# NilanEkanayake/TiTok-Video

Measured on AMD Instinct MI355X. Metric: video clips/sec encode+decode (whole node), higher is better.
Workload: dtype bf16

## Files before the change

include/titok_hip.h:

```cpp
#ifndef TITOK_HIP_H
#define TITOK_HIP_H

#include <stdint.h>

#ifdef __cplusplus
extern "C" {
#endif

#define TTV_OK 0
#define TTV_ERR_INVALID 1
#define TTV_ERR_LAUNCH 2
#define TTV_ERR_UNSUPPORTED 3

#define TTV_BF16 0
#define TTV_F32 1

#define TTV_ENCODER 0
#define TTV_DECODER 1

#define TTV_MAX_FSQ 8
#define TTV_MAX_TOKEN 64
#define TTV_MAX_CLIPS_PER_LAUNCH 64

const char* ttv_error_string(void);
// ... 100 lines not shown
                    int q_heads, int kv_heads, int head_dim, int flags, int dtype, void* stream);

int ttv_patch_gather(const void* const* clips, const int32_t* clip_desc, int clip0, int n_clips, int patch_t, int patch_h,
                     int patch_w, int channels, void* patches, int ld, int dtype, int max_patches_per_clip, void* stream);
int ttv_patch_scatter(const void* patches, int ld, const int32_t* clip_desc, int clip0, int n_clips, int patch_t, int patch_h,
                      int patch_w, int channels, void* const* clips, int dtype, int max_patches_per_clip, void* stream);

typedef struct ttv_tower_dims {
  int32_t kind;
  int32_t dtype;
  int32_t width;
  int32_t layers;
  int32_t q_heads, kv_heads, head_dim;
  int32_t inner;
  int32_t patch_t, patch_h, patch_w;
  int32_t pix_channels;
  int32_t token_size;
  float eps;
  float alpha;
} ttv_tower_dims;

typedef struct ttv_layer_weights {
  const float* pre_ln;
  const void* to_qkv;
  const void* out_proj;
  const float* ffd_norm;
  const void* w12;
  const void* w3;
  const float* attn_post_ln;
  const float* ffd_post_ln;
  const void* to_qkv_pn;
  const void* w12_pn;
  const void* mlp_pack;
  int32_t mlp_pack_qkv_rows;
  int32_t qkv_q_prescaled;
  const void* to_qkv_qs;
  const void* to_qkv_f8; const float* to_qkv_f8_scale;
  const void* w12_f8; const float* w12_f8_scale;
  const void* to_qkv_mx; const void* w12_mx;
  const void* out_proj_f8; const float* out_proj_f8_scale; const void* out_proj_mx;
  const void* w3_f8; const float* w3_f8_scale; const void* w3_mx;
} ttv_layer_weights;

typedef struct ttv_tower_weights {
  const void* proj_in_w;
  const void* proj_in_b;
  const float* mask_token;
  const float* ln_pre_t;
  const float* ln_pre_p;
  const float* ln_post;
  const void* proj_out_w;
  const void* proj_out_b;
  const ttv_layer_weights* layers;
  const void* proj_out_pn;
  int32_t f32_split3;
} ttv_tower_weights;

typedef struct ttv_batch {
  int32_t n_clips;
  int32_t total_rows;
  int32_t sum_tokens;
  int32_t sum_patches;
  int32_t max_patches_per_clip;
  int32_t n_qblocks;
  const int32_t* cu_seqlens;
  const int32_t* latent_rows;
  const int32_t* patch_rows;
  const int32_t* clip_desc;
  const int32_t* qblocks;
  const float* rope_cs;
  const int32_t* blocks64;
  const int32_t* row_seq;
  int32_t n_blocks64;
  int32_t qblocks_paired;
  int32_t qblocks_all_full;
  const int32_t* items64;
  int32_t n_items64;
  const int32_t* rope_ids;
  const float* rope_base;
  const int32_t* qblocks_latent;
  int32_t n_qblocks_latent;
  const int32_t* qblocks_patch;
  int32_t n_qblocks_patch;
} ttv_batch;

int ttv_rope_table_build(const float* base_cos, const float* base_sin, int n_ids, int n_freqs, const int32_t* clip_desc,
                         const int32_t* cu_seqlens, const int32_t* row_seq, float* rope_cs, int total_rows, void* stream);

typedef struct ttv_plan_sizes {
  int32_t n_clips, total_rows, sum_tokens, sum_patches, max_patches_per_clip, max_seqlen, n_rope_ids, n_blocks64;
  int64_t host_words;
  int64_t off_cu_seqlens, off_clip_desc, off_blocks64;
  int64_t dev_words;
  int64_t off_latent_rows, off_patch_rows, off_row_seq, off_rope_ids;
} ttv_plan_sizes;

int ttv_plan_rows_sizes(const int32_t* pixel_dims, const int32_t* token_counts, int n_clips, const int32_t* patch, ttv_plan_sizes* sizes);
int ttv_plan_rows_fill(const int32_t* pixel_dims, const int32_t* token_counts, int n_clips, const int32_t* patch, int bwd_xcd,
                       int32_t* host_segment, int64_t host_words);

int ttv_plan_rows_build(const ttv_plan_sizes* sizes, const int32_t* host_segment, int32_t* dev_segment, const float* base_cos,
                        const float* base_sin, int n_freqs, float* rope_cs, const float* rope_base, ttv_batch* batch, void* stream);

typedef struct ttv_plan_attn {
  int32_t n_qblocks, qblocks_all_full, n_qblocks_latent, n_qblocks_patch, n_qblocks_l0, reserved;
  int64_t words;
  int64_t off_qblocks, off_qblocks_latent, off_qblocks_patch, off_qblocks_l0;
} ttv_plan_attn;

int ttv_plan_attn_sizes(const int32_t* cu_seqlens, const int32_t* token_counts, int n_clips, int q_heads, int kv_heads, int split,
                        int tail_div, ttv_plan_attn* sizes);
int ttv_plan_attn_fill(const int32_t* cu_seqlens, const int32_t* token_counts, int n_clips, int q_heads, int kv_heads, int split,
                       int tail_div, int32_t* host_tables, int64_t host_words);
int ttv_plan_attn_set(const ttv_plan_attn* sizes, const int32_t* host_tables, int32_t* dev_tables, ttv_batch* batch, void* stream);

int ttv_rope_base_table(int head_dim, int nd, int n_ids, double theta, float* base_cos, float* base_sin);

int64_t ttv_tower_workspace_bytes(const ttv_tower_dims* dims, const ttv_batch* batch);

int ttv_encoder_forward(const ttv_tower_dims* dims, const ttv_tower_weights* w, const ttv_batch* batch,
                        const void* const* clips, const ttv_fsq_params* fsq, float* z, void* codes, int32_t* indices,
                        float* bounded, void* workspace, int64_t workspace_bytes, void* stream);

int ttv_decoder_forward(const ttv_tower_dims* dims, const ttv_tower_weights* w, const ttv_batch* batch, const void* codes,
                        void* const* clips_out, void* workspace, int64_t workspace_bytes, void* stream);

typedef struct ttv_dec_l0_const {
  const void* rows;
  int32_t latent_rows;
  int32_t patch_rows;
  const float* state;
  const int32_t* qblocks;
  int32_t n_qblocks;
} ttv_dec_l0_const;
int64_t ttv_dec_l0_const_bytes(const ttv_tower_dims* dims, int patch_rows);
int ttv_dec_l0_const_build(const ttv_tower_dims* dims, const ttv_tower_weights* w, const int32_t* iota, const float* rope_cs,
                           const int32_t* rope_ids, const float* rope_base, int patch_rows, void* block, int64_t block_bytes,
                           int64_t* state_offset, int64_t* flag_offset, void* stream);
int ttv_decoder_forward_const(const ttv_tower_dims* dims, const ttv_tower_weights* w, const ttv_batch* batch, const void* codes,
                              void* const* clips_out, void* workspace, int64_t workspace_bytes, const ttv_dec_l0_const* l0, void* stream);

typedef struct ttv_layer_weights_t {
  const void* to_qkv_t;
  const void* out_proj_t;
  const void* w12_t;
  const void* w3_t;
} ttv_layer_weights_t;
typedef struct ttv_tower_weights_t {
  const void* proj_in_t;
  const void* proj_out_t;
  const ttv_layer_weights_t* layers;
} ttv_tower_weights_t;
typedef struct ttv_layer_grads {
  float* pre_ln; float* to_qkv; float* out_proj; float* ffd_norm; float* w12; float* w3; float* attn_post_ln; float* ffd_post_ln;
} ttv_layer_grads;
typedef struct ttv_tower_grads {
  float* proj_in_w; float* proj_in_b; float* mask_token; float* ln_pre_t; float* ln_pre_p; float* ln_post; float* proj_out_w;
  float* proj_out_b;
  const ttv_layer_grads* layers;
  void** layer_done_events;
} ttv_tower_grads;

int64_t ttv_tower_tape_bytes(const ttv_tower_dims* dims, const ttv_batch* batch);
int64_t ttv_tower_bwd_workspace_bytes(const ttv_tower_dims* dims, const ttv_batch* batch);
#define TTV_TAPE_STORED 0
#define TTV_TAPE_RECOMPUTE 1
// ... 144 lines not shown
int ttv_fvd_preprocess(void* const* clips, const int32_t* dims, int n_clips, int dtype, int clamp, float* out, void* stream);

int ttv_i3d_features(const ttv_i3d_weights* w, const float* x, int n, float* feats, void* workspace, int64_t workspace_bytes,
                     void* stream);

int ttv_i3d_conv3d(const float* x, int N, int T, int H, int W, int Cin, int k, int stride, const float* w, const float* scale,
                   const float* shift, int Cout, int relu, float* y, int ldc, int c_off, void* stream);
int ttv_i3d_maxpool3d(const float* x, int N, int T, int H, int W, int C, int kt, int kh, int kw, int st, int sh, int sw, float* y,
                      void* stream);

#define TTV_VJEPA_WIDTH 1024
#define TTV_VJEPA_TOKENS 1568
#define TTV_VJEPA_PATCH_K 1536
typedef struct ttv_vjepa_layer {
  const float* norm1_w; const float* norm1_b;
  const void* qkv_w; const void* qkv_b;
  const void* proj_w; const void* proj_b;
  const float* norm2_w; const float* norm2_b;
  const void* fc1_w; const void* fc1_b;
  const void* fc2_w; const void* fc2_b;
} ttv_vjepa_layer;
typedef struct ttv_vjepa_weights {
  int32_t width, heads, depth;
  const void* patch_w; const void* patch_b; const float* pos_embed;
  const ttv_vjepa_layer* layers;
  const float* norm_w; const float* norm_b;
  const float* query_tokens; const void* pool_q;
  const float* pool_norm1_w; const float* pool_norm1_b;
  const void* pool_kv_w; const void* pool_kv_b;
  const void* pool_proj_w; const void* pool_proj_b;
  const float* pool_norm2_w; const float* pool_norm2_b;
  const void* pool_fc1_w; const void* pool_fc1_b;
  const void* pool_fc2_w; const void* pool_fc2_b;
} ttv_vjepa_weights;

int ttv_jedi_preprocess(void* const* clips, const int32_t* dims, int n_clips, int dtype, void* out, void* stream);
int64_t ttv_vjepa_workspace_bytes(int n);
int ttv_vjepa_features(const ttv_vjepa_weights* w, const void* x, int n, float* feats, int finetuned, void* workspace,
                       int64_t workspace_bytes, void* stream);

#define TTV_VJEPA_EPI_STORE 0
#define TTV_VJEPA_EPI_GELU 1
#define TTV_VJEPA_EPI_RESID 2
int ttv_vjepa_layernorm(const float* x, int ldx, int rows, int width, const float* w1, const float* b1, float eps1, const float* w2,
                        const float* b2, float eps2, float* y32, int ld32, void* y16, int ld16, void* stream);
int ttv_vjepa_linear(const void* x, int ldx, const void* w, int ldw, const void* bias, int M, int N, int K, int epilogue,
                     const float* resid, int ldr, int resid_rows, void* y, int ldy, void* stream);
int ttv_vjepa_pool_attention(const void* q, const void* kv, int n, int rows, void* out, void* stream);

#define TTV_KC_ATTENTION 1
#define TTV_KC_GEMM_QKV 2
#define TTV_KC_GEMM_GEGLU 3
#define TTV_KC_GEMM_RESID 4
#define TTV_KC_GEMM_STORE 5
#define TTV_KC_RMSNORM 6
#define TTV_KC_PATCH 7
#define TTV_KC_ROWS 8
int ttv_prof_begin(int kernel_class, int max_records);
enum {
  TTV_DBG_NO_STORES = 1,
  TTV_DBG_K256_NO_PANEL_DMA = 2,
  TTV_DBG_MLP_NO_WEIGHT_DMA = 2,
  TTV_DBG_K256_NO_TILE_RELOAD = 4,
  TTV_DBG_MLP_NO_GEGLU = 4,
  TTV_DBG_K256_NO_EPILOGUE_MATH = 8,
  TTV_DBG_MLP_TILES8 = 8,
  TTV_DBG_MLP_NO_P2 = 16,
  TTV_DBG_MLP_PAIRS_ONLY = 32,
  TTV_DBG_MLP_TILES4 = 64,
  TTV_DBG_GEMM_TILE160 = 128,
  TTV_DBG_GEMM_TILE128 = 256,
  TTV_DBG_GEMM_T256 = 512,
  TTV_DBG_MLP_TILES9 = 512,
  TTV_DBG_GEMM_NO_T256 = 1024,
  TTV_DBG_MX_UNFUSED_QUANT = 2048,
  TTV_DBG_SPLIT3_NO_IMAGES = 4096,
  TTV_DBG_SPLIT3_NO_DMA = 8192,
  TTV_DBG_K256_GENERAL = 16384,
  TTV_DBG_QKV256_OFF = 32768,
  TTV_DBG_QKV256_WS = 131072,
  TTV_DBG_ENC_ALL_ROWS = 524288,
  TTV_DBG_ATTN_NO_SWP = 1048576,
  TTV_DBG_DEC_ALL_BLOCKS = 2097152,
  TTV_DBG_DEC_L0_NO_CONST = 4194304
};
int ttv_debug_set(int flags);
int ttv_debug_stamps(void* device_buffer);
int ttv_prof_end(double* total_ms, int* count);

#ifdef __cplusplus
}
#endif
#endif
```

titok_video_amd/_lib.py:

```python
from __future__ import annotations

import ctypes as C
import os
import threading

import torch

from . import switches

TTV_BF16, TTV_F32 = 0, 1
TTV_ENCODER, TTV_DECODER = 0, 1
TTV_MAX_FSQ = 8
TTV_MAX_TOKEN = 64
TTV_MAX_CLIPS_PER_LAUNCH = 64
TTV_DISC_HEAD_GENERATOR, TTV_DISC_HEAD_DISCRIMINATOR = 0, 1
TTV_TAPE_STORED, TTV_TAPE_RECOMPUTE = 0, 1

DBG_NO_STORES = 1
DBG_K256_NO_PANEL_DMA = 2
DBG_MLP_NO_WEIGHT_DMA = 2
DBG_K256_NO_TILE_RELOAD = 4
DBG_MLP_NO_GEGLU = 4
DBG_K256_NO_EPILOGUE_MATH = 8
DBG_MLP_TILES8 = 8
DBG_MLP_NO_P2 = 16
DBG_MLP_PAIRS_ONLY = 32
DBG_MLP_TILES4 = 64
DBG_GEMM_TILE160 = 128
DBG_GEMM_TILE128 = 256
DBG_GEMM_T256 = 512
DBG_MLP_TILES9 = 512
DBG_GEMM_NO_T256 = 1024
DBG_MX_UNFUSED_QUANT = 2048
DBG_SPLIT3_NO_IMAGES = 4096
DBG_SPLIT3_NO_DMA = 8192
DBG_K256_GENERAL = 16384
DBG_QKV256_OFF = 32768
DBG_QKV256_WS = 131072
DBG_ENC_ALL_ROWS = 524288
DBG_ATTN_NO_SWP = 1048576
DBG_DEC_ALL_BLOCKS = 2097152
DBG_DEC_L0_NO_CONST = 4194304

_HERE = os.path.dirname(os.path.abspath(__file__))
LIB_PATH = switches.text("TTV_LIB_PATH") or os.path.join(_HERE, "libtitok_hip.so")

i32, i64, f32, vp = C.c_int32, C.c_int64, C.c_float, C.c_void_p


class FsqParams(C.Structure):
    _fields_ = [("n", i32), ("levels", i32 * TTV_MAX_FSQ), ("basis", i32 * TTV_MAX_FSQ),
                ("half_l", f32 * TTV_MAX_FSQ), ("offset", f32 * TTV_MAX_FSQ), ("shift", f32 * TTV_MAX_FSQ),
                ("half_width", f32 * TTV_MAX_FSQ)]


class TowerDims(C.Structure):
    _fields_ = [("kind", i32), ("dtype", i32), ("width", i32), ("layers", i32), ("q_heads", i32), ("kv_heads", i32),
                ("head_dim", i32), ("inner", i32), ("patch_t", i32), ("patch_h", i32), ("patch_w", i32),
                ("pix_channels", i32), ("token_size", i32), ("eps", f32), ("alpha", f32)]


class NextQkv(C.Structure):
    _fields_ = [("qkv", vp), ("ld", i32), ("rope_cs", vp), ("rows", i32), ("rope_q_end", i32), ("rope_k_begin", i32), ("rope_k_end", i32)]


class LayerWeights(C.Structure):
    _fields_ = [("pre_ln", vp), ("to_qkv", vp), ("out_proj", vp), ("ffd_norm", vp), ("w12", vp), ("w3", vp),
                ("attn_post_ln", vp), ("ffd_post_ln", vp), ("to_qkv_pn", vp), ("w12_pn", vp), ("mlp_pack", vp), ("mlp_pack_qkv_rows", i32), ("qkv_q_prescaled", i32),
                ("to_qkv_qs", vp), ("to_qkv_f8", vp), ("to_qkv_f8_scale", vp), ("w12_f8", vp), ("w12_f8_scale", vp),
                ("to_qkv_mx", vp), ("w12_mx", vp), ("out_proj_f8", vp), ("out_proj_f8_scale", vp), ("out_proj_mx", vp),
                ("w3_f8", vp), ("w3_f8_scale", vp), ("w3_mx", vp)]


class TowerWeights(C.Structure):
    _fields_ = [("proj_in_w", vp), ("proj_in_b", vp), ("mask_token", vp), ("ln_pre_t", vp), ("ln_pre_p", vp),
                ("ln_post", vp), ("proj_out_w", vp), ("proj_out_b", vp), ("layers", C.POINTER(LayerWeights)), ("proj_out_pn", vp),
                ("f32_split3", i32)]


class Batch(C.Structure):
    _fields_ = [("n_clips", i32), ("total_rows", i32), ("sum_tokens", i32), ("sum_patches", i32),
                ("max_patches_per_clip", i32), ("n_qblocks", i32), ("cu_seqlens", vp), ("latent_rows", vp),
                ("patch_rows", vp), ("clip_desc", vp), ("qblocks", vp), ("rope_cs", vp), ("blocks64", vp), ("row_seq", vp),
                ("n_blocks64", i32), ("qblocks_paired", i32), ("qblocks_all_full", i32), ("items64", vp), ("n_items64", i32),
                ("rope_ids", vp), ("rope_base", vp), ("qblocks_latent", vp), ("n_qblocks_latent", i32), ("qblocks_patch", vp),
                ("n_qblocks_patch", i32)]


class PlanSizes(C.Structure):
    _fields_ = [("n_clips", i32), ("total_rows", i32), ("sum_tokens", i32), ("sum_patches", i32), ("max_patches_per_clip", i32),
                ("max_seqlen", i32), ("n_rope_ids", i32), ("n_blocks64", i32), ("host_words", i64), ("off_cu_seqlens", i64),
                ("off_clip_desc", i64), ("off_blocks64", i64), ("dev_words", i64), ("off_latent_rows", i64), ("off_patch_rows", i64),
                ("off_row_seq", i64), ("off_rope_ids", i64)]


class PlanAttn(C.Structure):
    _fields_ = [("n_qblocks", i32), ("qblocks_all_full", i32), ("n_qblocks_latent", i32), ("n_qblocks_patch", i32), ("n_qblocks_l0", i32),
                ("reserved", i32), ("words", i64), ("off_qblocks", i64), ("off_qblocks_latent", i64), ("off_qblocks_patch", i64),
                ("off_qblocks_l0", i64)]


class DecL0Const(C.Structure):
    _fields_ = [("rows", vp), ("latent_rows", i32), ("patch_rows", i32), ("state", vp), ("qblocks", vp), ("n_qblocks", i32)]


class LayerWeightsT(C.Structure):
    _fields_ = [("to_qkv_t", vp), ("out_proj_t", vp), ("w12_t", vp), ("w3_t", vp)]


class TowerWeightsT(C.Structure):
    _fields_ = [("proj_in_t", vp), ("proj_out_t", vp), ("layers", C.POINTER(LayerWeightsT))]


class LayerGrads(C.Structure):
    _fields_ = [("pre_ln", vp), ("to_qkv", vp), ("out_proj", vp), ("ffd_norm", vp), ("w12", vp), ("w3", vp),
                ("attn_post_ln", vp), ("ffd_post_ln", vp)]


class TowerGrads(C.Structure):
    _fields_ = [("proj_in_w", vp), ("proj_in_b", vp), ("mask_token", vp), ("ln_pre_t", vp), ("ln_pre_p", vp), ("ln_post", vp),
                ("proj_out_w", vp), ("proj_out_b", vp), ("layers", C.POINTER(LayerGrads)), ("layer_done_events", C.POINTER(vp))]


TTV_OPT_SCHEDULE_NONE, TTV_OPT_SCHEDULE_COSINE = 0, 1
TTV_OPT_SKIP_NONFINITE = 1


class OptState(C.Structure):
    _fields_ = [("updates", i64), ("skipped", i64), ("schedule_index", i64), ("skip_now", i32), ("lr", f32), ("bc1", f32),
                ("bc2_sqrt", f32), ("clip_coef", f32), ("norm", f32)]


class OptSchedule(C.Structure):
    _fields_ = [("kind", i32), ("reserved", i32), ("warmup_steps", i64), ("training_steps", i64), ("base_lr", C.c_double),
                ("end_lr", C.c_double), ("num_cycles", C.c_double), ("initial_lr", C.c_double), ("first", i64), ("stride", i64)]


class LpipsWeights(C.Structure):
    _fields_ = [("w", vp * 13), ("wd", vp * 13), ("b", vp * 13), ("lin", vp * 5)]


TTV_I3D_CONVS = 58
TTV_I3D_FEATURES = 400


class I3dWeights(C.Structure):
    _fields_ = [("w", vp * TTV_I3D_CONVS), ("scale", vp * TTV_I3D_CONVS), ("shift", vp * TTV_I3D_CONVS)]


TTV_VJEPA_WIDTH = 1024
TTV_VJEPA_TOKENS = 1568
TTV_VJEPA_PATCH_K = 1536
TTV_VJEPA_EPI_STORE, TTV_VJEPA_EPI_GELU, TTV_VJEPA_EPI_RESID = 0, 1, 2


class VjepaLayer(C.Structure):
    _fields_ = [("norm1_w", vp), ("norm1_b", vp), ("qkv_w", vp), ("qkv_b", vp), ("proj_w", vp), ("proj_b", vp), ("norm2_w", vp),
                ("norm2_b", vp), ("fc1_w", vp), ("fc1_b", vp), ("fc2_w", vp), ("fc2_b", vp)]


class VjepaWeights(C.Structure):
    _fields_ = [("width", i32), ("heads", i32), ("depth", i32), ("patch_w", vp), ("patch_b", vp), ("pos_embed", vp),
                ("layers", C.POINTER(VjepaLayer)), ("norm_w", vp), ("norm_b", vp), ("query_tokens", vp), ("pool_q", vp),
                ("pool_norm1_w", vp), ("pool_norm1_b", vp), ("pool_kv_w", vp), ("pool_kv_b", vp), ("pool_proj_w", vp),
                ("pool_proj_b", vp), ("pool_norm2_w", vp), ("pool_norm2_b", vp), ("pool_fc1_w", vp), ("pool_fc1_b", vp),
                ("pool_fc2_w", vp), ("pool_fc2_b", vp)]


_lib = None
# ... 194 lines not shown
```

titok_video_amd/csrc/ttv_api.hip:

```cpp
#include <stdarg.h>
#include <stdio.h>
#include <stdlib.h>
#include <string.h>

#include "ttv_common.h"
#include "ttv_kernels.h"

static thread_local char g_err[512] = "";

void ttv_set_error(const char* fmt, ...) {
  va_list ap;
  va_start(ap, fmt);
  vsnprintf(g_err, sizeof(g_err), fmt, ap);
  va_end(ap);
}

int g_ttv_prof_class = 0;
bool ttv_sw_enc_latent_last() { static const bool v = ttv_env_flag("TTV_ENC_LATENT_LAST", true); return v; }
bool ttv_enc_latent_rows_only(const ttv_tower_dims* d, const ttv_batch* b) {
  return ttv_sw_enc_latent_last() && !(g_ttv_debug & TTV_DBG_ENC_ALL_ROWS) && d->kind == TTV_ENCODER && b->latent_rows && b->sum_tokens > 0 &&
         b->sum_tokens < b->total_rows;
}
bool ttv_sw_keel_f32sum() { static const bool v = ttv_env_flag("TTV_KEEL_F32SUM", false); return v; }
bool ttv_sw_fused_patch() { static const bool v = ttv_env_flag("TTV_FUSED_PATCH", true); return v; }
bool ttv_sw_attn_pipe() { static const bool v = ttv_env_flag("TTV_ATTN_PIPE", false); return v; }
static bool sw_dec_l0_const() { static const bool v = ttv_env_flag("TTV_DEC_L0_CONST", true); return v; }
float ttv_sw_attn_thr() { static const float v = ttv_env_float("TTV_ATTN_THR", 8.0f); return v; }
thread_local int g_ttv_debug = 0;
long long* g_ttv_stamps = nullptr;
static hipEvent_t* g_prof_start = nullptr;
static hipEvent_t* g_prof_stop = nullptr;
static int g_prof_cap = 0, g_prof_n = 0;

TtvProfScope::TtvProfScope(int cls, hipStream_t stream) : slot(-1), s(stream) {
  if (g_ttv_prof_class != 0 && cls == g_ttv_prof_class && g_prof_n < g_prof_cap) {
    slot = g_prof_n++;
    (void)hipEventRecord(g_prof_start[slot], s);
  }
}
TtvProfScope::~TtvProfScope() {
  if (slot >= 0) (void)hipEventRecord(g_prof_stop[slot], s);
}

struct TowerWs {
  char *x, *xn, *qkv, *ao, *h, *pa, *pb;
  char *xl, *aol;
  char *f8, *f8mx;
  float* y32;
  float* rstd;
  int64_t total;
};

static TowerWs carve(const ttv_tower_dims* d, const ttv_batch* b, char* base) {
  const int64_t e = dtype_bytes(d->dtype);
  const int64_t L = b->total_rows, P = b->sum_patches;
  const int64_t g = (int64_t)d->kv_heads * d->head_dim;
  const int64_t pd = patch_dim(d);
  int64_t off = 0;
  TowerWs w;
  auto take = [&](int64_t bytes) { char* p = base ? base + off : nullptr; off += align256(bytes); return p; };
  w.x = take(L * d->width * e);
  w.xn = take(L * d->width * e);
  w.qkv = take(L * (2 * d->width + 2 * g) * e);
  w.ao = take(L * d->width * e);
  w.y32 = (float*)take(L * d->width * 4);
  w.h = take(L * d->inner * e);
  w.pa = take(P * pd * e);
  w.pb = take(P * d->width * e);
  w.rstd = (float*)take(L * 4);
  w.xl = take((int64_t)b->sum_tokens * d->width * e);
  w.aol = take((int64_t)b->sum_tokens * d->width * e);
  w.f8 = w.f8mx = nullptr;
  if (d->dtype == TTV_BF16 && d->width != 256 && d->width % 128 == 0) {
    const int64_t wide = d->width > d->inner ? d->width : d->inner;
    w.f8 = take(L * wide);
    w.f8mx = take(L * (wide / 128 + 4) * 4);
  }
  w.total = off;
  return w;
}

static int check_dims(const ttv_tower_dims* d, const ttv_batch* b) {
  TTV_CHECK_ARG(d && b, "null dims/batch");
  TTV_CHECK_ARG(d->dtype == TTV_BF16 || d->dtype == TTV_F32, "bad dtype %d", d->dtype);
  TTV_CHECK_ARG(d->head_dim == 64 && d->width == d->q_heads * 64, "width must be q_heads*64");
  TTV_CHECK_ARG(d->width % 64 == 0 && d->width <= 1024, "width %d unsupported", d->width);
  TTV_CHECK_ARG(d->inner % 32 == 0, "GEGLU inner dim must be a multiple of 32");
  TTV_CHECK_ARG(d->token_size >= 1 && d->token_size <= TTV_MAX_TOKEN, "token_size out of range");
  TTV_CHECK_ARG(((int64_t)d->pix_channels * d->patch_t * d->patch_h * d->patch_w) % 8 == 0, "patch vector length must be a multiple of 8");
  TTV_CHECK_ARG(b->n_clips > 0 && b->total_rows == b->sum_tokens + b->sum_patches, "inconsistent batch");
  return TTV_OK;
}

struct LayerCtx {
  const ttv_tower_dims* d; const ttv_batch* b; const TowerWs& ws; hipStream_t s;
  int split3, s3img;
  bool gen_ok;
  int pair, all_full, pipe;
};

static int tower_attention(const LayerCtx& c, bool q_scaled, const int32_t* table, int n_table, int site) {
  const ttv_tower_dims* d = c.d;
  const int flags = TTV_ATTN_GATE | (q_scaled ? TTV_ATTN_QSCALED : 0) | (c.split3 ? TTV_ATTN_SPLIT3 : 0) |
                    (c.s3img ? (TTV_ATTN_SPLIT_OUT | TTV_ATTN_SPLIT_IN) : 0) | site;
  return ttvk_attention(c.ws.qkv, 2 * d->width + 2 * d->kv_heads * d->head_dim, c.ws.ao, d->width, c.b->cu_seqlens, table, n_table, d->q_heads,
                        d->kv_heads, d->head_dim, flags, d->dtype, c.s);
}

static int run_layer_mx(const LayerCtx& c, const ttv_layer_weights& lw, int i, bool& rstd_valid, bool& xq_valid) {
  const ttv_tower_dims* d = c.d;
  const ttv_batch* b = c.b;
  const TowerWs& ws = c.ws;
  hipStream_t s = c.s;
  const int L = b->total_rows, dm = d->width, g = d->kv_heads * d->head_dim, dt = d->dtype, nq = 2 * dm + 2 * g, I = d->inner;
  const float alpha = keel_alpha(d, i);
  static const bool fused_env = ttv_env_flag("TTV_MX_FUSED_QUANT", true);
  const bool fused_q = fused_env && !(g_ttv_debug & TTV_DBG_MX_UNFUSED_QUANT);
  if (!rstd_valid) TTV_TRY(ttvk_row_rstd(ws.x, dt, dm, ws.rstd, L, dm, d->eps, s));
  if (!xq_valid) TTV_TRY(ttvk_quant_mx_fp8(ws.x, dt, dm, ws.f8, dm, ws.f8mx, nullptr, L, dm, s));
  xq_valid = false;
  const GemmArgs a = gemm_rope_qk(gemm_args(dt, ws.f8, dm, lw.to_qkv_f8, dm, L, nq, dm, ws.qkv, nq), b->rope_cs, dm, g);
  TTV_TRY(ttvk_gemm_fp8(EPI_QKV_ROPE, a, ws.rstd, lw.to_qkv_f8_scale, s, ws.f8mx, lw.to_qkv_mx));
  const bool q_scaled = lw.qkv_q_prescaled != 0;
  if (fused_q && q_scaled && !c.pair && !c.pipe && d->head_dim == 64) {
    TTV_TRY(ttvk_attention_mxout(ws.qkv, nq, ws.f8, ws.f8mx, (int)ttvk_mx_scale_ld(dm), b->cu_seqlens, b->qblocks, b->n_qblocks, d->q_heads,
                                 d->kv_heads, s));
  } else {
    TTV_TRY(tower_attention(c, q_scaled, b->qblocks, b->n_qblocks, c.pair | (c.pipe ? c.all_full | c.pipe : 0)));
    TTV_TRY(ttvk_quant_mx_fp8(ws.ao, dt, dm, ws.f8, dm, ws.f8mx, nullptr, L, dm, s));
  }
  const GemmArgs o = gemm_resid(gemm_args(dt, ws.f8, dm, lw.out_proj_f8, dm, L, dm, dm, ws.x, dm), ws.x, dm, alpha);
  TTV_TRY(ttvk_gemm_fp8(EPI_RESID_T, o, nullptr, lw.out_proj_f8_scale, s, ws.f8mx, lw.out_proj_mx));
  if (i > 0) {
    TTV_TRY(ttvk_rmsnorm(ws.x, dt, dm, nullptr, ws.x, dt, dm, nullptr, lw.attn_post_ln, L, dm, d->eps, s, ws.rstd, fused_q ? ws.f8 : nullptr,
                         fused_q ? ws.f8mx : nullptr));
    if (!fused_q) TTV_TRY(ttvk_quant_mx_fp8(ws.x, dt, dm, ws.f8, dm, ws.f8mx, nullptr, L, dm, s));
  } else {
    TTV_TRY(ttvk_row_rstd(ws.x, dt, dm, ws.rstd, L, dm, d->eps, s));
    TTV_TRY(ttvk_quant_mx_fp8(ws.x, dt, dm, ws.f8, dm, ws.f8mx, nullptr, L, dm, s));
  }
  GemmArgs f = gemm_args(dt, ws.f8, dm, lw.w12_f8, dm, L, I, dm, ws.h, I);
  char* const hq = ws.h;
  char* const hq_mx = ws.xn;
  const bool h_fused = fused_q && (int64_t)ttvk_mx_scale_ld(I) <= (int64_t)dm * 2;
  if (h_fused) { f.yq = hq; f.yq_mx = hq_mx; }
  TTV_TRY(ttvk_gemm_fp8(EPI_GEGLU, f, ws.rstd, lw.w12_f8_scale, s, ws.f8mx, lw.w12_mx));
  if (!h_fused) TTV_TRY(ttvk_quant_mx_fp8(ws.h, dt, I, ws.f8, I, ws.f8mx, nullptr, L, I, s));
  const GemmArgs f3 = gemm_resid(gemm_args(dt, h_fused ? hq : ws.f8, I, lw.w3_f8, I, L, dm, I, ws.x, dm), ws.x, dm, alpha);
  TTV_TRY(ttvk_gemm_fp8(EPI_RESID_T, f3, nullptr, lw.w3_f8_scale, s, h_fused ? hq_mx : ws.f8mx, lw.w3_mx));
  rstd_valid = false;
  if (i > 0) {
    TTV_TRY(ttvk_rmsnorm(ws.x, dt, dm, nullptr, ws.x, dt, dm, nullptr, lw.ffd_post_ln, L, dm, d->eps, s, ws.rstd, fused_q ? ws.f8 : nullptr,
                         fused_q ? ws.f8mx : nullptr));
    rstd_valid = true;
    xq_valid = fused_q;
  }
  return TTV_OK;
}

static bool rows_f8(int dt, int dm, const void* img, const void* row_scale, const void* mx, const void* folded) {
  return dt == TTV_BF16 && img && row_scale && !mx && dm % 128 == 0 && !(dm == 256 && folded);
}

struct PreNormW { const float* gain; const void *w, *w_pn, *w_f8; const float* w_f8_scale; bool f8; };

static int prenorm_proj(const LayerCtx& c, GemmEpilogue epi, const char* x, int rows, const PreNormW& p, int N, char* y, int y_image,
                        bool rstd_valid, int tile_run = 0, int tile_period = 0) {
  const ttv_tower_dims* d = c.d;
  const TowerWs& ws = c.ws;
  const int dm = d->width, dt = d->dtype;
  GemmArgs a = gemm_args(dt, nullptr, dm, nullptr, dm, rows, N, dm, y, N);
  if (epi == EPI_QKV_ROPE) a = gemm_rope_qk(a, c.b->rope_cs, dm, d->kv_heads * d->head_dim);
  if (p.f8) {
    float* const f8_scales = reinterpret_cast<float*>(ws.xn + align256((int64_t)c.b->total_rows * dm));
    TTV_TRY(ttvk_quant_rows_fp8(x, dt, dm, p.gain, d->eps, ws.xn, dm, f8_scales, rows, dm, c.s));
    a.x = ws.xn; a.w = p.w_f8;
    return ttvk_gemm_fp8(epi, a, f8_scales, p.w_f8_scale, c.s);
  }
  const bool fold256 = dt == TTV_BF16 && dm == 256 && p.w_pn;
  const bool fold_gen = c.gen_ok && p.w_pn;
  const bool fold = fold256 || fold_gen;
  if (fold_gen && !rstd_valid) TTV_TRY(ttvk_row_rstd(x, dt, dm, ws.rstd, rows, dm, d->eps, c.s));
  if (!fold) TTV_TRY(ttvk_rmsnorm(x, dt, dm, nullptr, ws.xn, dt, dm, nullptr, p.gain, rows, dm, d->eps, c.s, nullptr, nullptr, nullptr, c.s3img));
  a.split3 = c.split3; a.x_image = c.s3img && !fold; a.y_image = y_image;
  a.prenorm = fold256; a.eps = d->eps;
  a.row_scale = fold_gen ? ws.rstd : nullptr;
  a.x = fold ? x : ws.xn; a.w = fold ? p.w_pn : p.w;
  if (epi == EPI_QKV_ROPE) { a.rope_ids = c.b->rope_ids; a.rope_base = c.b->rope_ids ? c.b->rope_base : nullptr; }
  a.tile_run = tile_run; a.tile_period = tile_period;
  return ttvk_gemm(epi, a, c.s);
}

static int keel_tail(const LayerCtx& c, GemmArgs o, int layer, const float* post_gain, bool want_rstd, bool& rstd_valid) {
  const ttv_tower_dims* d = c.d;
  const int dm = d->width, dt = d->dtype;
  char* const cx = (char*)o.y;
  o = gemm_resid(o, cx, dm, keel_alpha(d, layer));
  o.split3 = c.split3; o.x_image = c.s3img;
  if (layer == 0) return ttvk_gemm(EPI_RESID_T, o, c.s);
  if (ttvk_gemm_supports_resid_norm(dt, dm, o.K)) {
    o.norm_gain = post_gain; o.eps = d->eps;
    return ttvk_gemm(EPI_RESID_NORM, o, c.s);
  }
  float* const next_rstd = want_rstd ? c.ws.rstd : nullptr;
  if (dt == TTV_BF16 && !ttv_sw_keel_f32sum()) {
    TTV_TRY(ttvk_gemm(EPI_RESID_T, o, c.s));
    TTV_TRY(ttvk_rmsnorm(cx, dt, dm, nullptr, cx, dt, dm, nullptr, post_gain, o.M, dm, d->eps, c.s, next_rstd));
  } else {
    o.y = c.ws.y32;
    TTV_TRY(ttvk_gemm(EPI_RESID_F32, o, c.s));
    TTV_TRY(ttvk_rmsnorm(c.ws.y32, TTV_F32, dm, nullptr, cx, dt, dm, nullptr, post_gain, o.M, dm, d->eps, c.s, next_rstd));
  }
  rstd_valid = want_rstd;
  return TTV_OK;
}

static bool dec_l0_const_ok(const LayerCtx& c, const ttv_tower_weights* w, const ttv_dec_l0_const* l0) {
  const ttv_tower_dims* d = c.d;
  const ttv_batch* b = c.b;
  if (!l0 || !l0->rows || !sw_dec_l0_const() || (g_ttv_debug & TTV_DBG_DEC_L0_NO_CONST)) return false;
  if (d->kind != TTV_DECODER || d->dtype != TTV_BF16 || d->width != 256 || d->head_dim != 64 || c.split3) return false;
  const int K = l0->latent_rows, P = l0->patch_rows;
  if (K <= 0 || P <= 0 || K % 128 || P % 128 || (int64_t)b->n_clips * K != b->sum_tokens || (int64_t)b->n_clips * P != b->sum_patches) return false;
  const ttv_layer_weights& lw = w->layers[0];
  if (!lw.to_qkv_pn || !lw.qkv_q_prescaled) return false;
  if (c.pair || c.pipe || !c.all_full || (b->items64 && b->n_items64 > 0)) return false;
  return ttvk_gemm_qkv_tiles_supported(d->width, d->kv_heads * d->head_dim, d->width) &&
         ttvk_attention_takes_swp(TTV_ATTN_GATE | TTV_ATTN_QSCALED | TTV_ATTN_ALLFULL);
}

static int run_layers(const ttv_tower_dims* d, const ttv_tower_weights* w, const ttv_batch* b, const TowerWs& ws, hipStream_t s,
                      const ttv_dec_l0_const* l0 = nullptr) {
  const int L = b->total_rows, dm = d->width, g = d->kv_heads * d->head_dim, dt = d->dtype;
  const int split3 = (dt == TTV_F32 && w->f32_split3) ? 1 : 0;
  const bool gen_ok = (dt == TTV_BF16 && dm != 256) || split3;
  static const bool s3img_env = ttv_env_flag("TTV_SPLIT3_IMAGES", true);
  const int s3img = (split3 && s3img_env && !(g_ttv_debug & TTV_DBG_SPLIT3_NO_IMAGES)) ? 1 : 0;
  const int nq = 2 * dm + 2 * g;
  const int64_t row_bytes = (int64_t)dm * dtype_bytes(dt);
  bool qkv_ready = false;
  bool rstd_valid = false;
  bool xq_valid = false;
  const bool lat_last = ttv_enc_latent_rows_only(d, b) && b->qblocks_latent && b->n_qblocks_latent > 0;
  static const bool pat_env = ttv_env_flag("TTV_DEC_PATCH_LAST", true);
  const bool pat_last = pat_env && !(g_ttv_debug & TTV_DBG_DEC_ALL_BLOCKS) && d->kind == TTV_DECODER && d->layers >= 2 && b->qblocks_patch &&
                        b->n_qblocks_patch > 0 && !split3 && !b->qblocks_paired;
  bool compacted = false;
  const LayerCtx ctx = {d, b, ws, s, split3, s3img, gen_ok, b->qblocks_paired ? TTV_ATTN_PAIRED : 0, b->qblocks_all_full ? TTV_ATTN_ALLFULL : 0,
                        ttv_sw_attn_pipe() ? TTV_ATTN_PIPE : 0};
  const bool l0_const = dec_l0_const_ok(ctx, w, l0);
  for (int i = 0; i < d->layers; ++i) {
    const ttv_layer_weights& lw = w->layers[i];
    const bool last = i == d->layers - 1;
    const bool l0c = l0_const && i == 0;
    if (dt == TTV_BF16 && dm != 256 && dm % 128 == 0 && d->inner % 128 == 0 && !ttv_sw_keel_f32sum() && lw.to_qkv_f8 && lw.to_qkv_mx && lw.w12_f8 &&
        lw.w12_mx && lw.out_proj_f8 && lw.out_proj_mx && lw.w3_f8 && lw.w3_mx &&
        !(lat_last && last)) {
      TTV_TRY(run_layer_mx(ctx, lw, i, rstd_valid, xq_valid));
      qkv_ready = false;
      continue;
    }
    xq_valid = false;
    const bool f8_qkv = rows_f8(dt, dm, lw.to_qkv_f8, lw.to_qkv_f8_scale, lw.to_qkv_mx, lw.to_qkv_pn);
    const bool f8_w12 = rows_f8(dt, dm, lw.w12_f8, lw.w12_f8_scale, lw.w12_mx, lw.w12_pn);
    if (!qkv_ready) {
      const void* w_plain = (dt == TTV_BF16 && lw.to_qkv_qs) ? lw.to_qkv_qs : lw.to_qkv;
      const PreNormW qw = {lw.pre_ln, w_plain, lw.to_qkv_pn, lw.to_qkv_f8, lw.to_qkv_f8_scale, f8_qkv};
      if (l0c) TTV_TRY(prenorm_proj(ctx, EPI_QKV_ROPE, ws.x, L, qw, nq, ws.qkv, 0, rstd_valid, l0->latent_rows / 128, (l0->latent_rows + l0->patch_rows) / 128));
      else TTV_TRY(prenorm_proj(ctx, EPI_QKV_ROPE, ws.x, L, qw, nq, ws.qkv, s3img ? 2 : 0, rstd_valid));
    }
    const bool q_scaled = dt == TTV_BF16 && (lw.to_qkv_pn ? lw.qkv_q_prescaled != 0 : lw.to_qkv_qs != nullptr);
    rstd_valid = false;
    qkv_ready = false;
    const bool lat_now = lat_last && last;
    if (lat_now)
      TTV_TRY(tower_attention(ctx, q_scaled, b->qblocks_latent, b->n_qblocks_latent, ctx.all_full));
    else if (l0c) {
      TtvProfScope prof(TTV_KC_ATTENTION, s);
      const bool own = l0->qblocks && l0->n_qblocks > 0;
      TTV_TRY(ttvk_attention_swp(ws.qkv, nq, ws.ao, dm, b->cu_seqlens, own ? l0->qblocks : b->qblocks, own ? l0->n_qblocks : b->n_qblocks, d->q_heads,
                                 d->kv_heads, 1, s, l0->rows, l0->latent_rows, l0->state));
    } else if (pat_last && last && dt == TTV_BF16 && !ctx.pipe)
      TTV_TRY(tower_attention(ctx, q_scaled, b->qblocks_patch, b->n_qblocks_patch, ctx.all_full));
    else if (q_scaled && b->items64 && b->n_items64 > 0 && d->head_dim == 64)
      TTV_TRY(ttvk_attention64(ws.qkv, nq, ws.ao, dm, b->cu_seqlens, b->items64, b->n_items64, d->q_heads, d->kv_heads,
                               TTV_ATTN_GATE | TTV_ATTN_QSCALED, s));
    else
      TTV_TRY(tower_attention(ctx, q_scaled, b->qblocks, b->n_qblocks, ctx.pair | ctx.all_full | ctx.pipe));
    char* cx = ws.x;
    char* cao = ws.ao;
    int Lc = L;
    if (lat_now) {
      TTV_TRY(gather_rows(ws.x, ws.xl, b->latent_rows, b->sum_tokens, row_bytes, s));
      TTV_TRY(gather_rows(ws.ao, ws.aol, b->latent_rows, b->sum_tokens, row_bytes, s));
      cx = ws.xl; cao = ws.aol; Lc = b->sum_tokens;
      compacted = true;
    }
    static const bool use_fused_mlp = ttv_env_flag("TTV_FUSED_MLP", true);
    static const bool use_fused_qkv = ttv_env_flag("TTV_FUSED_QKV", false);
    const float alpha = keel_alpha(d, i);
    if (use_fused_mlp && ttvk_mlp_fused_supported(dt, dm, d->inner) && lw.mlp_pack) {
      MlpNextQkv nx = {};
      const bool back = use_fused_qkv && !last && lw.mlp_pack_qkv_rows == nq && nq % 64 == 0 && dm % 64 == 0 && g % 64 == 0;
      if (back) { nx.qkv = ws.qkv; nx.ld = nq; nx.rope_cs = b->rope_cs; nx.rows = nq; nx.rope_q_end = dm; nx.rope_k_begin = 2 * dm; nx.rope_k_end = 2 * dm + g; }
      TTV_TRY(ttvk_mlp_fused(cao, dm, i == 0 ? nullptr : lw.attn_post_ln, alpha, cx, dm, lw.mlp_pack, d->inner, cx, dm, i == 0 ? nullptr : lw.ffd_post_ln,
                             alpha, d->eps, Lc, back ? &nx : nullptr, s));
      qkv_ready = back;
      continue;
    }
    TTV_TRY(keel_tail(ctx, gemm_args(dt, cao, dm, lw.out_proj, dm, Lc, dm, dm, cx, dm), i, lw.attn_post_ln, gen_ok && lw.w12_pn && !f8_w12, rstd_valid));
    const PreNormW fw = {lw.ffd_norm, lw.w12, lw.w12_pn, lw.w12_f8, lw.w12_f8_scale, f8_w12};
    TTV_TRY(prenorm_proj(ctx, EPI_GEGLU, cx, Lc, fw, d->inner, ws.h, s3img, rstd_valid));
    rstd_valid = false;
    const ttv_layer_weights* nl = last ? nullptr : &w->layers[i + 1];
    const bool next_rstd = gen_ok && nl && nl->to_qkv_pn && !rows_f8(dt, dm, nl->to_qkv_f8, nl->to_qkv_f8_scale, nl->to_qkv_mx, nl->to_qkv_pn);
    TTV_TRY(keel_tail(ctx, gemm_args(dt, ws.h, d->inner, lw.w3, d->inner, Lc, dm, d->inner, cx, dm), i, lw.ffd_post_ln, next_rstd, rstd_valid));
  }
  if (compacted)
    TTV_TRY(scatter_rows(ws.xl, ws.x, b->latent_rows, b->sum_tokens, row_bytes, s));
  return TTV_OK;
}

static bool fused_patch_ok(const ttv_tower_dims* d, const ttv_batch* b, int dt) {
  auto pow2 = [](int v) { return v > 0 && (v & (v - 1)) == 0; };
  return ttv_sw_fused_patch() && dt == TTV_BF16 && d->patch_w == 8 && pow2(d->patch_t) && pow2(d->patch_h) &&
         b->n_clips <= TTV_MAX_CLIPS_PER_LAUNCH && b->row_seq && patch_dim(d) % 64 == 0;
}

extern "C" {

const char* ttv_error_string(void) { return g_err; }
int ttv_version(void) { return 100; }

int ttv_fsq_forward(const ttv_fsq_params* p, const void* z, int z_dtype, int rows, void* codes, int codes_dtype, int32_t* indices,
                    float* bounded, void* stream) {
  TTV_CHECK_ARG(rows >= 0 && (rows == 0 || (z && codes && indices)), "fsq_forward: null buffer");
  return ttvk_fsq_forward(p, z, z_dtype, rows, codes, codes_dtype, indices, bounded, (hipStream_t)stream);
}

int ttv_fsq_indices_to_codes(const ttv_fsq_params* p, const int32_t* indices, int rows, void* codes, int codes_dtype, void* stream) {
  TTV_CHECK_ARG(rows >= 0 && (rows == 0 || (indices && codes)), "fsq_indices_to_codes: null buffer");
  return ttvk_fsq_indices_to_codes(p, indices, rows, codes, codes_dtype, (hipStream_t)stream);
}

int ttv_vq_codebook_norms(const void* codebook, int dtype, int ld, int N, int C, float* cnorm, void* stream) {
  TTV_CHECK_ARG(N == 0 || (codebook && cnorm), "vq_codebook_norms: null buffer");
  return ttvk_vq_norms(codebook, dtype, ld, N, C, cnorm, (hipStream_t)stream);
}

int64_t ttv_vq_workspace_bytes(int rows) { return ttvk_vq_workspace_bytes(rows); }

int ttv_vq_l2_argmin(const void* z, int dtype, int ldz, const void* codebook, int ldc, const float* cnorm, int rows, int N, int C,
                     int32_t* indices, float* best_dist, void* workspace, int64_t workspace_bytes, void* stream) {
  TTV_CHECK_ARG(rows == 0 || (z && codebook && cnorm && indices), "vq_l2_argmin: null buffer");
  TTV_CHECK_ARG(ldz >= C && ldc >= C, "vq_l2_argmin: leading dims smaller than the codebook dim");
  return ttvk_vq_l2_argmin(z, dtype, ldz, codebook, ldc, cnorm, rows, N, C, indices, best_dist, workspace, workspace_bytes, (hipStream_t)stream);
}

int ttv_vq_lookup(const void* codebook, int dtype, int ldc, const int32_t* indices, int rows, int C, void* codes, int ldo, void* stream) {
  TTV_CHECK_ARG(rows == 0 || (codebook && indices && codes), "vq_lookup: null buffer");
  return ttvk_vq_lookup(codebook, dtype, ldc, indices, rows, C, codes, ldo, (hipStream_t)stream);
}

int ttv_vq_lookup_backward(const void* dcodes, int dtype, int ld, const int32_t* indices, int rows, int C, float* dcodebook, int ldc, void* stream) {
  TTV_CHECK_ARG(rows == 0 || (dcodes && indices && dcodebook), "vq_lookup_backward: null buffer");
  TTV_CHECK_ARG(ld >= C && ldc >= C, "vq_lookup_backward: leading dims smaller than the codebook dim");
  return ttvk_vq_lookup_bwd(dcodes, dtype, ld, indices, rows, C, dcodebook, ldc, (hipStream_t)stream);
}

int64_t ttv_vq_train_workspace_bytes(int rows, int N) {
  if (rows < 1 || N < 1) { ttv_set_error("vq_train_workspace_bytes: %d rows, %d entries", rows, N); return -1; }
  return ttvk_vq_train_workspace_bytes(rows, N);
}

int ttv_vq_commit_forward(const void* z, int dtype, int ldz, const void* codebook, int ldc, const int32_t* indices, int rows, int N, int C,
                          float* loss, void* workspace, int64_t workspace_bytes, void* stream) {
  TTV_CHECK_ARG(z && codebook && indices && loss && workspace, "vq_commit_forward: null buffer");
  return ttvk_vq_commit_forward(z, dtype, ldz, codebook, ldc, indices, rows, N, C, loss, workspace, workspace_bytes, (hipStream_t)stream);
}

int ttv_vq_commit_backward(const void* grad, int ldg, const void* z, int ldz, const void* e, int lde, int dtype, int rows, int C, double scale,
// ... 505 lines not shown
```

titok_video_amd/csrc/ttv_gemm.hip:

```cpp
#include <stdlib.h>

#include "ttv_common.h"
#include "ttv_kernels.h"

struct GemmDev {
  const void* x; const void* w; void* y;
  const void* bias; const float* add_scalar; const void* resid; const float* rope_cs;
  int ldx, ldw, ldy, ldr;
  int M, N, K;
  int w_rows;
  float alpha;
  int rope_q_end, rope_k_begin, rope_k_end;
  float eps;
  int debug;
  const float* norm_gain;
  ClipPtrs clips;
  const int* clip_desc; const int* patch_rows; const int* row_seq;
  const int* x_rows;
  const float* row_scale;
  const int* rope_ids; const float* rope_base;
  const float* x_scale; const float* w_scale;
  float* sum_f32; int ld_sum;
  void* y2; int ldy2; const float* norm_gain2;
  int split3;
  int x_image, y_image;
  const uint8_t* x_mx; const uint8_t* w_mx;
  int ld_mx;
  uint8_t* yq; uint8_t* yq_mx; int ld_yq_mx, yq_nkp;
  int clip0, pt_shift, ph_shift;
  long long* stamps;
  int resid_rows;
  int tile_run, tile_period;
};

struct PatchDst {
  bf16_t* base;
  int thw, hw, w;
};

__device__ __forceinline__ float gelu_erf(float v) { return 0.5f * v * (1.0f + erff(v * 0.70710678118654752440f)); }
__device__ __forceinline__ float gelu_erf_as(float v) {
  const float x = fabsf(v) * 0.70710678118654752440f;
  const float t = __builtin_amdgcn_rcpf(fmaf(0.3275911f, x, 1.0f));
  const float poly = t * fmaf(t, fmaf(t, fmaf(t, fmaf(t, 1.061405429f, -1.453152027f), 1.421413741f), -0.284496736f), 0.254829592f);
  const float e = __builtin_amdgcn_exp2f(x * x * -1.44269504088896340736f);
  const float erf_abs = fmaf(-poly, e, 1.0f);
  return 0.5f * v * (1.0f + __builtin_copysignf(erf_abs, v));
}

__device__ __forceinline__ uint2 pack_bf16x4(f32x4 v) {
  bf16x4 b = {(bf16_t)v[0], (bf16_t)v[1], (bf16_t)v[2], (bf16_t)v[3]};
  return __builtin_bit_cast(uint2, b);
}

__device__ __forceinline__ uint4 split4_bf16(uint4 v) {
  const float x0 = __uint_as_float(v.x), x1 = __uint_as_float(v.y), x2 = __uint_as_float(v.z), x3 = __uint_as_float(v.w);
  const bf16_t h0 = (bf16_t)x0, h1 = (bf16_t)x1, h2 = (bf16_t)x2, h3 = (bf16_t)x3;
  const bf16_t l0 = (bf16_t)(x0 - (float)h0), l1 = (bf16_t)(x1 - (float)h1), l2 = (bf16_t)(x2 - (float)h2), l3 = (bf16_t)(x3 - (float)h3);
  const bf16x4 hv = {h0, h1, h2, h3}, lv = {l0, l1, l2, l3};
  const uint2 hp = __builtin_bit_cast(uint2, hv), lp = __builtin_bit_cast(uint2, lv);
  return make_uint4(hp.x, hp.y, lp.x, lp.y);
}

template <int EPI, typename T, int NI, int NJ>
__device__ __forceinline__ void epilogue_tile(const GemmDev& p, const int (&tok)[NJ], const int (&feat)[NI],
                                              f32x4 (&acc)[NI][NJ], f32x4 (&acc2)[NI][NJ], int kq, const PatchDst* pd = nullptr) {
  if (p.debug & TTV_DBG_NO_STORES) {
#pragma unroll
    for (int i = 0; i < NI; ++i)
#pragma unroll
      for (int j = 0; j < NJ; ++j) asm volatile("" ::"v"(acc[i][j][0]), "v"(acc[i][j][3]), "v"(acc2[i][j][1]));
    return;
  }
  int tc[NJ], fc[NI];
  bool tv[NJ], fv[NI];
#pragma unroll
  for (int j = 0; j < NJ; ++j) { tv[j] = tok[j] < p.M; tc[j] = tv[j] ? tok[j] : p.M - 1; }
#pragma unroll
  for (int i = 0; i < NI; ++i) { fv[i] = feat[i] < p.N; fc[i] = fv[i] ? feat[i] : p.N - 4; }

  if (p.row_scale) {
#pragma unroll
    for (int j = 0; j < NJ; ++j) {
      const float rs = p.row_scale[tc[j]];
#pragma unroll
      for (int i = 0; i < NI; ++i) {
        acc[i][j] *= rs;
        if (EPI == EPI_GEGLU) acc2[i][j] *= rs;
      }
    }
  }

  if (EPI == EPI_STORE || EPI == EPI_STORE_PATCH || EPI == EPI_BIAS_PLAIN) {
    if (p.bias) {
      f32x4 b[NI];
#pragma unroll
      for (int i = 0; i < NI; ++i) b[i] = Vec4<T>::load((const T*)p.bias + fc[i]);
#pragma unroll
      for (int i = 0; i < NI; ++i)
#pragma unroll
        for (int j = 0; j < NJ; ++j) acc[i][j] += b[i];
    }
    if (p.add_scalar) {
      const float sc = round_to<T>(p.add_scalar[0]);
#pragma unroll
      for (int i = 0; i < NI; ++i)
#pragma unroll
        for (int j = 0; j < NJ; ++j) {
          if (p.bias) {
#pragma unroll
            for (int e = 0; e < 4; ++e) acc[i][j][e] = round_to<T>(acc[i][j][e]);
          }
          acc[i][j] += sc;
        }
    }
// ... 1650 lines not shown
      const int sw = (arow >> 1) & 7;
      const uint4 c0 = lds[buf][arow * 8 + (kq ^ sw)], c1 = lds[buf][arow * 8 + ((kq + 4) ^ sw)];
      ah[i] = __builtin_bit_cast(bf16x8, make_uint4(c0.x, c0.y, c1.x, c1.y));
      al[i] = __builtin_bit_cast(bf16x8, make_uint4(c0.z, c0.w, c1.z, c1.w));
    }
#pragma unroll
    for (int j = 0; j < NJ; ++j) {
      const int brow = wt * (16 * NJ) + j * 16 + l15;
      const int sw = (brow >> 1) & 7;
      const uint4 c0 = lds[buf][TF * 8 + brow * 8 + (kq ^ sw)], c1 = lds[buf][TF * 8 + brow * 8 + ((kq + 4) ^ sw)];
      bh[j] = __builtin_bit_cast(bf16x8, make_uint4(c0.x, c0.y, c1.x, c1.y));
      bl[j] = __builtin_bit_cast(bf16x8, make_uint4(c0.z, c0.w, c1.z, c1.w));
    }
#pragma unroll
    for (int i = 0; i < 4; ++i)
#pragma unroll
      for (int j = 0; j < NJ; ++j) acc[i][j] = __builtin_amdgcn_mfma_f32_16x16x32_bf16(al[i], bh[j], acc[i][j], 0, 0, 0);
#pragma unroll
    for (int i = 0; i < 4; ++i)
#pragma unroll
      for (int j = 0; j < NJ; ++j) acc[i][j] = __builtin_amdgcn_mfma_f32_16x16x32_bf16(ah[i], bl[j], acc[i][j], 0, 0, 0);
#pragma unroll
    for (int i = 0; i < 4; ++i)
#pragma unroll
      for (int j = 0; j < NJ; ++j) acc[i][j] = __builtin_amdgcn_mfma_f32_16x16x32_bf16(ah[i], bh[j], acc[i][j], 0, 0, 0);
    } else {
#pragma unroll
      for (int kb = 0; kb < 2; ++kb) {
        f32x4 a[4], b[NJ];
        const int kc = kb * 4 + kq;
#pragma unroll
        for (int i = 0; i < 4; ++i) {
          const int arow = (DUAL ? (i < 2 ? wf * 32 + i * 16 : 64 + wf * 32 + (i - 2) * 16) : wf * 64 + i * 16) + l15;
          a[i] = __builtin_bit_cast(f32x4, lds[buf][arow * 8 + (kc ^ ((arow >> 1) & 7))]);
        }
#pragma unroll
        for (int j = 0; j < NJ; ++j) {
          const int brow = wt * (16 * NJ) + j * 16 + l15;
          b[j] = __builtin_bit_cast(f32x4, lds[buf][TF * 8 + brow * 8 + (kc ^ ((brow >> 1) & 7))]);
        }
#pragma unroll
        for (int jj = 0; jj < 4; ++jj)
#pragma unroll
          for (int i = 0; i < 4; ++i)
#pragma unroll
            for (int j = 0; j < NJ; ++j) acc[i][j] = __builtin_amdgcn_mfma_f32_16x16x4f32(a[i][jj], b[j][jj], acc[i][j], 0, 0, 0);
      }
    }
    __builtin_amdgcn_s_waitcnt(0x0F70);
    __syncthreads();
  }
#undef GS_STAGE
#undef GS_DMA

  int tok[NJ];
#pragma unroll
  for (int j = 0; j < NJ; ++j) tok[j] = tbase + wt * (16 * NJ) + j * 16 + l15;
  if (DUAL) {
    int feat[2];
    f32x4 ax[2][NJ], ag[2][NJ];
#pragma unroll
    for (int i = 0; i < 2; ++i) {
      feat[i] = fbase + wf * 32 + i * 16 + kq * 4;
#pragma unroll
      for (int j = 0; j < NJ; ++j) { ax[i][j] = acc[i][j]; ag[i][j] = acc[i + 2][j]; }
    }
    epilogue_tile<EPI, float, 2, NJ>(p, tok, feat, ax, ag, kq);
  } else {
    int feat[4];
#pragma unroll
    for (int i = 0; i < 4; ++i) feat[i] = fbase + wf * 64 + i * 16 + kq * 4;
    epilogue_tile<EPI, float, 4, NJ>(p, tok, feat, acc, acc, kq);
  }
}

static int gemm_token_tile(int M, int nf, int debug) {
  if (debug & TTV_DBG_GEMM_TILE160) return 160;
  if (debug & TTV_DBG_GEMM_TILE128) return 128;
  const long cost128 = (long)ttv_cdiv(nf * ttv_cdiv(M, 128), 512) * 128, cost160 = (long)ttv_cdiv(nf * ttv_cdiv(M, 160), 512) * 160;
  return cost160 < cost128 ? 160 : 128;
}

static int sw_qkv256() { static const int v = ttv_env_int("TTV_QKV256", 1); return v; }
bool ttvk_gemm_qkv_tiles_supported(int d_model, int gqa_dim, int ldw) {
  const int N = 2 * d_model + 2 * gqa_dim;
  return sw_qkv256() == 1 && !(g_ttv_debug & (TTV_DBG_QKV256_OFF | TTV_DBG_QKV256_WS)) && N % 64 == 0 && d_model % 64 == 0 && gqa_dim % 64 == 0 &&
         (uint64_t)N * (uint64_t)ldw * 2u < (1ull << 32);
}

template <int EPI>
static int launch(const GemmDev& d, int dtype, bool prenorm, hipStream_t s) {
  if (dtype == TTV_BF16 && d.K == 256 && d.N % 8 == 0 && !((d.debug & TTV_DBG_K256_GENERAL) && !prenorm && EPI != EPI_STORE_PATCH)) {
    const int fo = (EPI == EPI_GEGLU) ? 32 : 64;
    const int n_panels = ttv_cdiv(d.N, fo), n_tiles = d.tile_period ? d.M / K256_TT / d.tile_period * d.tile_run : ttv_cdiv(d.M, K256_TT);
    const int total = n_panels * n_tiles;
    static const int grid_env = ttv_env_int("TTV_K256_GRID", 0);
    int grid = total < 512 ? total : 512;
    if (grid_env > 0) grid = total < grid_env ? total : grid_env;
    else if (total > 512)
      for (int g = 512; g >= 416; --g)
        if (total % g == 0) { grid = g; break; }
    const int qkv256_env = sw_qkv256();
    if constexpr (EPI == EPI_QKV_ROPE) {
      const int n_groups = (n_panels + 3) / 4;
      if (qkv256_env && !(d.debug & TTV_DBG_QKV256_OFF) && d.N % 64 == 0 && d.rope_q_end % 64 == 0 && d.rope_k_begin % 64 == 0 && d.rope_k_end % 64 == 0 &&
          !d.row_scale && !d.bias && !d.add_scalar && (uint64_t)d.w_rows * (uint64_t)d.ldw * 2u < (1ull << 32)) {
        if ((qkv256_env >= 2 || (d.debug & TTV_DBG_QKV256_WS)) && n_groups <= 32 && !d.tile_period) {
          const int tgs = ttv_cdiv(d.M, 32), per_xcd = ttv_cdiv(tgs, 8);
          int q = n_groups * ttv_cdiv(per_xcd, 8);
          q = q > 32 ? 32 : q;
          if (prenorm) hipLaunchKernelGGL((k_qkv256ws<true>), dim3(8 * q), dim3(512), 0, s, d, n_panels, n_groups);
          else hipLaunchKernelGGL((k_qkv256ws<false>), dim3(8 * q), dim3(512), 0, s, d, n_panels, n_groups);
          TTV_CHECK_LAUNCH("qkv256ws");
          return TTV_OK;
        }
        if (prenorm) hipLaunchKernelGGL((k_qkv256<true>), dim3(grid), dim3(256), 0, s, d, n_panels, total);
        else hipLaunchKernelGGL((k_qkv256<false>), dim3(grid), dim3(256), 0, s, d, n_panels, total);
        TTV_CHECK_LAUNCH("qkv256");
        return TTV_OK;
      }
    }
    if (d.tile_period) {
      ttv_set_error("gemm: a tile list needs k_qkv256 (ttvk_gemm_qkv_tiles_supported)");
      return TTV_ERR_UNSUPPORTED;
    }
    if (prenorm) hipLaunchKernelGGL((k_gemm_k256<EPI, true>), dim3(grid), dim3(256), 0, s, d, n_panels, total);
    else hipLaunchKernelGGL((k_gemm_k256<EPI, false>), dim3(grid), dim3(256), 0, s, d, n_panels, total);
    TTV_CHECK_LAUNCH("gemm_k256");
    return TTV_OK;
  }
  if (prenorm || EPI == EPI_STORE_PATCH) {
    ttv_set_error("gemm: folded pre-norm / patch scatter need the bf16 K=256 kernel");
    return TTV_ERR_UNSUPPORTED;
  }
  if (dtype == TTV_BF16) {
    const int ft = (EPI == EPI_GEGLU) ? 64 : TF;
    const int nf = ttv_cdiv(d.N, ft), nt = ttv_cdiv(d.M, TT), nt160 = ttv_cdiv(d.M, 160);
    const bool t160 = gemm_token_tile(d.M, nf, d.debug) == 160;
    static const bool use_dma = ttv_env_flag("TTV_GEMM_DMA", true);
    const bool dma_ok = use_dma && d.K % BK == 0 && (uint64_t)d.M * (uint64_t)d.ldx * 2u < (1ull << 32) && (uint64_t)d.w_rows * (uint64_t)d.ldw * 2u < (1ull << 32);
    static const int t256_env = ttv_env_int("TTV_GEMM_T256", -1);
    if constexpr (EPI == EPI_STORE || EPI == EPI_QKV_ROPE || EPI == EPI_GEGLU || EPI == EPI_RESID_T || EPI == EPI_RESID_F32) {
      const int fo = (EPI == EPI_GEGLU) ? 128 : T256_F;
      const long tiles256 = (long)ttv_cdiv(d.N, fo) * ttv_cdiv(d.M, T256_T);
      const bool forced = (d.debug & TTV_DBG_GEMM_T256) || t256_env == 1;
      const bool ok256 = dma_ok && d.N % fo == 0 && d.K >= 2 * BK && !(d.debug & TTV_DBG_GEMM_NO_T256) && (forced || tiles256 >= 256);
      if (ok256 && (forced || (t256_env < 0 && T256_DEFAULT))) {
        hipLaunchKernelGGL((k_gemm_bf16_t256<EPI>), dim3((unsigned)tiles256), dim3(512), 0, s, d, ttv_cdiv(d.N, fo));
        TTV_CHECK_LAUNCH("gemm_t256");
        return TTV_OK;
      }
    }
    if (t160) {
      if (dma_ok) hipLaunchKernelGGL((k_gemm_bf16_dma<EPI, 5>), dim3(nf * nt160), dim3(256), 0, s, d, nf);
      else hipLaunchKernelGGL((k_gemm_bf16<EPI, false, 5>), dim3(nf * nt160), dim3(256), 0, s, d, nf);
    } else {
      if (dma_ok) hipLaunchKernelGGL((k_gemm_bf16_dma<EPI, 4>), dim3(nf * nt), dim3(256), 0, s, d, nf);
      else hipLaunchKernelGGL((k_gemm_bf16<EPI>), dim3(nf * nt), dim3(256), 0, s, d, nf);
    }
  } else {
    if ((uint64_t)d.M * (uint64_t)d.ldx >= (1ull << 31) || (uint64_t)d.w_rows * (uint64_t)d.ldw >= (1ull << 31)) {
      ttv_set_error("gemm (fp32): operand too large for 32-bit element offsets");
      return TTV_ERR_UNSUPPORTED;
    }
    const int nf = ttv_cdiv(d.N, (EPI == EPI_GEGLU) ? 64 : F_TF), nt = ttv_cdiv(d.M, F_TT), nt160 = ttv_cdiv(d.M, 160);
    const bool t160 = gemm_token_tile(d.M, nf, d.debug) == 160;
    static const bool s3dma_env = ttv_env_flag("TTV_SPLIT3_DMA", true);
    const bool s3dma = d.split3 && d.x_image && s3dma_env && !(d.debug & TTV_DBG_SPLIT3_NO_DMA) && d.K % 32 == 0 && d.ldx % 4 == 0 && d.ldw % 4 == 0 &&
                       (uint64_t)d.M * (uint64_t)d.ldx * 4u < (1ull << 32) && (uint64_t)d.w_rows * (uint64_t)d.ldw * 4u < (1ull << 32);
    if (s3dma) {
      if (t160) hipLaunchKernelGGL((k_gemm_split_dma<EPI, 5>), dim3(nf * nt160), dim3(256), 0, s, d, nf);
      else hipLaunchKernelGGL((k_gemm_split_dma<EPI, 4>), dim3(nf * nt), dim3(256), 0, s, d, nf);
    } else if (d.split3) {
      if (t160) hipLaunchKernelGGL((k_gemm_f32<EPI, true, 5>), dim3(nf * nt160), dim3(256), 0, s, d, nf);
      else hipLaunchKernelGGL((k_gemm_f32<EPI, true, 4>), dim3(nf * nt), dim3(256), 0, s, d, nf);
    } else if (s3dma_env && !(d.debug & TTV_DBG_SPLIT3_NO_DMA) && d.K % 32 == 0 && d.ldx % 4 == 0 && d.ldw % 4 == 0 &&
               (uint64_t)d.M * (uint64_t)d.ldx * 4u < (1ull << 32) && (uint64_t)d.w_rows * (uint64_t)d.ldw * 4u < (1ull << 32)) {
      if (t160) hipLaunchKernelGGL((k_gemm_split_dma<EPI, 5, false>), dim3(nf * nt160), dim3(256), 0, s, d, nf);
      else hipLaunchKernelGGL((k_gemm_split_dma<EPI, 4, false>), dim3(nf * nt), dim3(256), 0, s, d, nf);
    } else {
      if (t160) hipLaunchKernelGGL((k_gemm_f32<EPI, false, 5>), dim3(nf * nt160), dim3(256), 0, s, d, nf);
      else hipLaunchKernelGGL((k_gemm_f32<EPI, false, 4>), dim3(nf * nt), dim3(256), 0, s, d, nf);
    }
  }
  TTV_CHECK_LAUNCH("gemm");
  return TTV_OK;
}

int ttvk_gemm_fp8(GemmEpilogue epi, const GemmArgs& a, const float* x_scale, const float* w_scale, hipStream_t s, const void* x_mx, const void* w_mx) {
  if (a.M == 0 || a.N == 0) return TTV_OK;
  const bool mx = x_mx || w_mx;
  TTV_CHECK_ARG(epi == EPI_STORE || epi == EPI_QKV_ROPE || epi == EPI_GEGLU || (mx && epi == EPI_RESID_T),
                "gemm_fp8: epilogue must be STORE, QKV_ROPE or GEGLU (block-scaled operands: RESID_T as well)");
  TTV_CHECK_ARG(a.K > 0 && a.K % 128 == 0 && a.N % 8 == 0, "gemm_fp8: K %% 128, N %% 8");
  TTV_CHECK_ARG(a.ldx % 16 == 0 && a.ldw % 16 == 0 && a.ldy % 8 == 0 && ((uintptr_t)a.x % 16 == 0) && ((uintptr_t)a.w % 16 == 0) && ((uintptr_t)a.y % 16 == 0),
                "gemm_fp8: 16-byte row alignment");
  if (mx) TTV_CHECK_ARG(x_mx && w_mx && (uintptr_t)x_mx % 4 == 0 && (uintptr_t)w_mx % 4 == 0 && (!w_scale || (uintptr_t)w_scale % 16 == 0),
                        "gemm_fp8: block scales of both operands needed (4-byte aligned)");
  else TTV_CHECK_ARG(x_scale && w_scale && (uintptr_t)w_scale % 16 == 0, "gemm_fp8: scales missing / unaligned");
  if (epi == EPI_RESID_T) TTV_CHECK_ARG(a.resid && a.ldr % 4 == 0, "gemm_fp8: residual missing");
  TTV_CHECK_ARG((uint64_t)a.M * (uint64_t)a.ldx < (1ull << 32), "gemm_fp8: operand too large for 32-bit offsets");
  GemmDev d = {};
  d.x = a.x; d.w = a.w; d.y = a.y; d.bias = a.bias; d.add_scalar = a.add_scalar; d.resid = a.resid; d.rope_cs = a.rope_cs; d.rope_ids = a.rope_ids; d.rope_base = a.rope_base;
  d.ldx = a.ldx; d.ldw = a.ldw; d.ldy = a.ldy; d.ldr = a.ldr; d.M = a.M; d.N = a.N; d.K = a.K; d.alpha = a.alpha;
  d.w_rows = (epi == EPI_GEGLU) ? 2 * a.N : a.N;
  d.rope_q_end = a.rope_q_end; d.rope_k_begin = a.rope_k_begin; d.rope_k_end = a.rope_k_end; d.eps = a.eps; d.debug = g_ttv_debug;
  d.x_scale = x_scale; d.w_scale = w_scale;
  d.x_mx = (const uint8_t*)x_mx; d.w_mx = (const uint8_t*)w_mx; d.ld_mx = 4 * ((a.K / 128 + 3) / 4 * 4);
  if (a.yq) {
    TTV_CHECK_ARG(mx && epi == EPI_GEGLU && a.yq_mx && a.N % 128 == 0 && (uintptr_t)a.yq % 4 == 0, "gemm_fp8: the fp8 GEGLU output needs block-scaled operands, its scale buffer and N %% 128 == 0");
    d.yq = (uint8_t*)a.yq; d.yq_mx = (uint8_t*)a.yq_mx; d.yq_nkp = (a.N / 128 + 3) / 4 * 4; d.ld_yq_mx = 4 * d.yq_nkp;
  }
  if (epi == EPI_QKV_ROPE) TTV_CHECK_ARG(a.rope_cs && a.rope_q_end % 128 == 0 && a.rope_k_begin % 128 == 0 && a.rope_k_end % 128 == 0, "gemm_fp8: rotary ranges must be multiples of 128 columns");
  const int ft = (epi == EPI_GEGLU) ? 64 : TF;
  const int nf = ttv_cdiv(d.N, ft), nt = ttv_cdiv(d.M, TT), nt160 = ttv_cdiv(d.M, 160);
  const bool t160 = gemm_token_tile(d.M, nf, 0) == 160;
  const int kc = epi == EPI_STORE ? TTV_KC_GEMM_STORE : epi == EPI_QKV_ROPE ? TTV_KC_GEMM_QKV : epi == EPI_GEGLU ? TTV_KC_GEMM_GEGLU : TTV_KC_GEMM_RESID;
  TtvProfScope prof(kc, s);
#define F8_LAUNCH(E_, MX_)                                                                                         \
  do {                                                                                                              \
    if (t160) hipLaunchKernelGGL((k_gemm_fp8_dma<E_, 5, MX_>), dim3(nf * nt160), dim3(256), 0, s, d, nf);           \
    else hipLaunchKernelGGL((k_gemm_fp8_dma<E_, 4, MX_>), dim3(nf * nt), dim3(256), 0, s, d, nf);                   \
  } while (0)
  if (mx) {
    if (epi == EPI_STORE) F8_LAUNCH(EPI_STORE, true); else if (epi == EPI_QKV_ROPE) F8_LAUNCH(EPI_QKV_ROPE, true);
    else if (epi == EPI_GEGLU) F8_LAUNCH(EPI_GEGLU, true); else F8_LAUNCH(EPI_RESID_T, true);
  } else {
    if (epi == EPI_STORE) F8_LAUNCH(EPI_STORE, false); else if (epi == EPI_QKV_ROPE) F8_LAUNCH(EPI_QKV_ROPE, false); else F8_LAUNCH(EPI_GEGLU, false);
  }
#undef F8_LAUNCH
  TTV_CHECK_LAUNCH("gemm_fp8");
  return TTV_OK;
}

bool ttvk_gemm_supports_resid_norm(int dtype, int N, int K) { return dtype == TTV_BF16 && N == 256 && K % 8 == 0; }

int ttvk_gemm(GemmEpilogue epi, const GemmArgs& a, hipStream_t s) {
  if (a.M == 0 || a.N == 0) return TTV_OK;
  const int esz = dtype_bytes(a.dtype);
  const int vec = 16 / esz;
  TTV_CHECK_ARG(a.dtype == TTV_BF16 || a.dtype == TTV_F32, "gemm: bad dtype %d", a.dtype);
  TTV_CHECK_ARG(a.K > 0 && a.K % vec == 0, "gemm: K=%d must be a multiple of %d", a.K, vec);
  TTV_CHECK_ARG(a.N % 4 == 0, "gemm: N=%d must be a multiple of 4", a.N);
  TTV_CHECK_ARG(a.ldx % vec == 0 && a.ldw % vec == 0 && a.ldy % vec == 0, "gemm: leading dims must keep 16-byte row alignment");
  TTV_CHECK_ARG(((uintptr_t)a.x % 16 == 0) && ((uintptr_t)a.w % 16 == 0) && ((uintptr_t)a.y % 16 == 0), "gemm: pointers must be 16-byte aligned");
  GemmDev d;
  d.x = a.x; d.w = a.w; d.y = a.y; d.bias = a.bias; d.add_scalar = a.add_scalar; d.resid = a.resid; d.rope_cs = a.rope_cs; d.rope_ids = a.rope_ids; d.rope_base = a.rope_base;
  d.ldx = a.ldx; d.ldw = a.ldw; d.ldy = a.ldy; d.ldr = a.ldr;
  d.M = a.M; d.N = a.N; d.K = a.K; d.alpha = a.alpha;
  d.w_rows = (epi == EPI_GEGLU) ? 2 * a.N : a.N;
  d.rope_q_end = a.rope_q_end; d.rope_k_begin = a.rope_k_begin; d.rope_k_end = a.rope_k_end;
  d.eps = a.eps;
  d.debug = g_ttv_debug;
  d.sum_f32 = a.sum_f32; d.ld_sum = a.ld_sum; d.y2 = a.y2; d.ldy2 = a.ldy2; d.norm_gain2 = a.norm_gain2;
  d.split3 = (a.split3 && a.dtype == TTV_F32) ? 1 : 0;
  d.x_image = d.split3 && a.x_image; d.y_image = d.split3 ? a.y_image : 0;
  TTV_CHECK_ARG(!d.y_image || (d.y_image == 1 && (epi == EPI_STORE || epi == EPI_GEGLU)) || (d.y_image == 2 && epi == EPI_QKV_ROPE),
                "gemm: a split-image output is a STORE / GEGLU option (y_image 1) or the to_qkv layout (y_image 2)");
  d.x_mx = d.w_mx = nullptr; d.ld_mx = 0;
  d.norm_gain = a.norm_gain;
  d.clip_desc = a.clip_desc; d.patch_rows = a.patch_rows; d.row_seq = a.row_seq; d.clip0 = 0; d.pt_shift = d.ph_shift = 0;
  d.x_rows = a.x_rows;
  d.x_scale = nullptr; d.w_scale = nullptr;
  d.row_scale = a.row_scale;
  d.stamps = g_ttv_stamps;
  d.resid_rows = a.resid_rows;
  d.tile_run = d.tile_period = 0;
  if (a.tile_period) {
    TTV_CHECK_ARG(epi == EPI_QKV_ROPE && a.dtype == TTV_BF16 && a.K == 256 && a.tile_run > 0 && a.tile_run < a.tile_period &&
                  a.M % (K256_TT * a.tile_period) == 0, "gemm: a tile list is a to_qkv option of the bf16 K=256 kernel, M a whole number of periods");
    d.tile_run = a.tile_run; d.tile_period = a.tile_period;
  }
  TTV_CHECK_ARG(!a.row_scale || ((a.dtype == TTV_BF16 || a.split3) && (epi == EPI_STORE || epi == EPI_QKV_ROPE || epi == EPI_GEGLU)),
                "gemm: row_scale is a STORE / QKV_ROPE / GEGLU option of the bf16 and the split-bf16 kernels");
  TTV_CHECK_ARG(!a.x_rows || (a.dtype == TTV_BF16 && a.K == 256 && a.N % 8 == 0 && epi != EPI_RESID_NORM), "gemm: x_rows needs the bf16 K=256 kernel");
  if (epi == EPI_STORE_PATCH || a.gather) {
    auto lg2 = [](int v) { int s = 0; while ((1 << s) < v) ++s; return (1 << s) == v ? s : -1; };
    TTV_CHECK_ARG(a.dtype == TTV_BF16 && (a.gather || a.K == 256) && a.patch_w == 8 && lg2(a.patch_t) >= 0 && lg2(a.patch_h) >= 0,
                  "gemm: patch gather/scatter needs bf16, patch_w == 8 and power-of-two patch_t / patch_h (scatter: K == 256)");
    TTV_CHECK_ARG(!a.gather || (epi == EPI_STORE && a.K % 64 == 0 && a.K != 256), "gemm: patch gather is an EPI_STORE option of the general-K kernel");
    TTV_CHECK_ARG(a.clips && a.n_clips > 0 && a.n_clips <= TTV_MAX_CLIPS_PER_LAUNCH && a.clip_desc && a.patch_rows && a.row_seq,
                  "gemm: patch scatter needs clips (<= %d), clip_desc, patch_rows and row_seq", TTV_MAX_CLIPS_PER_LAUNCH);
    for (int i = 0; i < a.n_clips; ++i) d.clips.p[i] = a.clips[i];
    d.pt_shift = lg2(a.patch_t); d.ph_shift = lg2(a.patch_h);
  }
  const bool pn = a.prenorm != 0;
  const int kc = (epi == EPI_STORE || epi == EPI_STORE_PATCH) ? TTV_KC_GEMM_STORE : epi == EPI_QKV_ROPE ? TTV_KC_GEMM_QKV : epi == EPI_GEGLU ? TTV_KC_GEMM_GEGLU : TTV_KC_GEMM_RESID;
  TtvProfScope prof(kc, s);
  switch (epi) {
    case EPI_STORE:
      if (a.gather) {
        const int nf = ttv_cdiv(d.N, TF), nt = ttv_cdiv(d.M, TT), nt160 = ttv_cdiv(d.M, 160);
        if (gemm_token_tile(d.M, nf, d.debug) == 160)
          hipLaunchKernelGGL((k_gemm_bf16<EPI_STORE, true, 5>), dim3(nf * nt160), dim3(256), 0, s, d, nf);
        else
          hipLaunchKernelGGL((k_gemm_bf16<EPI_STORE, true>), dim3(nf * nt), dim3(256), 0, s, d, nf);
        TTV_CHECK_LAUNCH("gemm_gather");
        return TTV_OK;
      }
      return launch<EPI_STORE>(d, a.dtype, pn, s);
    case EPI_STORE_PATCH: return launch<EPI_STORE_PATCH>(d, a.dtype, pn, s);
    case EPI_QKV_ROPE:
      TTV_CHECK_ARG(a.rope_cs && a.rope_q_end % 128 == 0 && a.rope_k_begin % 128 == 0 && a.rope_k_end % 128 == 0, "gemm: rotary ranges must be multiples of 128 columns");
      return launch<EPI_QKV_ROPE>(d, a.dtype, pn, s);
    case EPI_GEGLU: return launch<EPI_GEGLU>(d, a.dtype, pn, s);
    case EPI_RESID_T:
      TTV_CHECK_ARG(a.resid && a.ldr % 4 == 0, "gemm: residual missing");
      return launch<EPI_RESID_T>(d, a.dtype, pn, s);
    case EPI_RESID_F32:
      TTV_CHECK_ARG(a.resid && a.ldr % 4 == 0, "gemm: residual missing");
      return launch<EPI_RESID_F32>(d, a.dtype, pn, s);
    case EPI_BIAS_PLAIN:
    case EPI_BIAS_GELU:
    case EPI_BIAS_RESID_F32R: {
      TTV_CHECK_ARG(a.dtype == TTV_BF16 && a.K % BK == 0 && a.bias && (uintptr_t)a.bias % 8 == 0, "gemm: V-JEPA epilogues need bf16, K %% 64 == 0 and a bias");
      TTV_CHECK_ARG(!a.add_scalar && !a.row_scale, "gemm: V-JEPA epilogues take no scalar / row scale");
      TTV_CHECK_ARG(epi != EPI_BIAS_RESID_F32R || (a.resid && a.ldr % 4 == 0 && (uintptr_t)a.resid % 16 == 0 && a.resid_rows >= 0),
                    "gemm: fp32 residual missing or unaligned");
      TTV_CHECK_ARG((uint64_t)a.M * (uint64_t)a.ldx * 2u < (1ull << 32) && (uint64_t)a.N * (uint64_t)a.ldw * 2u < (1ull << 32),
                    "gemm: operand too large for 32-bit byte offsets");
      if (d.N % T256_F == 0 && d.K >= 2 * BK) {
        const int nf = d.N / T256_F, nt = ttv_cdiv(d.M, T256_T);
        if (epi == EPI_BIAS_PLAIN) hipLaunchKernelGGL((k_gemm_bf16_t256<EPI_BIAS_PLAIN>), dim3(nf * nt), dim3(512), 0, s, d, nf);
        else if (epi == EPI_BIAS_GELU) hipLaunchKernelGGL((k_gemm_bf16_t256<EPI_BIAS_GELU>), dim3(nf * nt), dim3(512), 0, s, d, nf);
        else hipLaunchKernelGGL((k_gemm_bf16_t256<EPI_BIAS_RESID_F32R>), dim3(nf * nt), dim3(512), 0, s, d, nf);
        TTV_CHECK_LAUNCH("gemm_vjepa_t256");
        return TTV_OK;
      }
      const int nf = ttv_cdiv(d.N, TF), nt = ttv_cdiv(d.M, TT);
      if (epi == EPI_BIAS_PLAIN) hipLaunchKernelGGL((k_gemm_bf16_dma<EPI_BIAS_PLAIN, 4>), dim3(nf * nt), dim3(256), 0, s, d, nf);
      else if (epi == EPI_BIAS_GELU) hipLaunchKernelGGL((k_gemm_bf16_dma<EPI_BIAS_GELU, 4>), dim3(nf * nt), dim3(256), 0, s, d, nf);
      else hipLaunchKernelGGL((k_gemm_bf16_dma<EPI_BIAS_RESID_F32R, 4>), dim3(nf * nt), dim3(256), 0, s, d, nf);
      TTV_CHECK_LAUNCH("gemm_vjepa");
      return TTV_OK;
    }
    case EPI_RESID_NORM: {
      TTV_CHECK_ARG(ttvk_gemm_supports_resid_norm(a.dtype, a.N, a.K), "gemm: fused residual+norm needs bf16 and N == 256");
      TTV_CHECK_ARG(a.resid && a.norm_gain && a.ldr % 4 == 0 && a.ldw >= 256, "gemm: residual / gain missing");
      TTV_CHECK_ARG(a.y != a.x, "gemm: fused residual+norm output must not alias the GEMM input");
      TTV_CHECK_ARG(!a.y2 || (a.norm_gain2 && a.ldy2 % 8 == 0 && (uintptr_t)a.y2 % 16 == 0 && a.y2 != a.x), "gemm: second norm output needs its gain, 16-byte rows");
      TTV_CHECK_ARG(!a.sum_f32 || (a.ld_sum % 4 == 0 && (uintptr_t)a.sum_f32 % 16 == 0), "gemm: fp32 sum output needs 16-byte rows");
      if (a.K == 256) {
        const int n_tiles = ttv_cdiv(a.M, ROW_TT);
        hipLaunchKernelGGL(k_gemm_k256_rownorm, dim3(n_tiles < 512 ? n_tiles : 512), dim3(256), 0, s, d, n_tiles);
        TTV_CHECK_LAUNCH("gemm_k256_rownorm");
      } else {
        hipLaunchKernelGGL(k_gemm_rowtile_norm, dim3(ttv_cdiv(a.M, 64)), dim3(256), 0, s, d);
        TTV_CHECK_LAUNCH("gemm_rowtile_norm");
      }
      return TTV_OK;
    }
  }
  ttv_set_error("gemm: unknown epilogue");
  return TTV_ERR_INVALID;
// ... 2 lines not shown
```

titok_video_amd/csrc/ttv_kernels.h:

```cpp
#pragma once
#include <hip/hip_runtime.h>
#include <stdint.h>

#include "../../include/titok_hip.h"

int ttvk_rmsnorm(const void* in, int in_dtype, int ld_in, const int* src_rows, void* out, int out_dtype, int ld_out,
                 const int* dst_rows, const float* gain, int rows, int d, float eps, hipStream_t s, float* next_rstd = nullptr,
                 void* mx_q = nullptr, void* mx_s = nullptr,
                 int split_image = 0);
int ttvk_row_rstd(const void* in, int dtype, int ld_in, float* rstd, int rows, int d, float eps, hipStream_t s);
int ttvk_copy_rows(const void* src, int64_t ld_src_bytes, const int* src_rows, void* dst, int64_t ld_dst_bytes, const int* dst_rows, int rows,
                   int row_bytes, hipStream_t s);
int ttvk_fill_const_rows(void* x, int dtype, int ld, const int* rows_map, int rows, int d, const float* mask_token,
                         const float* gain, float eps, hipStream_t s);
int ttvk_dec_embed(const void* codes, int C, const void* w, const void* bias, const float* mask_token, const float* gain,
                   void* x, int dtype, int ld, const int* rows_map, int rows, int d, float eps, hipStream_t s);
int ttvk_fsq_forward(const ttv_fsq_params* p, const void* z, int z_dtype, int rows, void* codes, int codes_dtype, int* indices,
                     float* bounded, hipStream_t s);
int ttvk_fsq_indices_to_codes(const ttv_fsq_params* p, const int* indices, int rows, void* codes, int codes_dtype, hipStream_t s);
int ttvk_enc_tail(const void* x, int dtype, int ld, const int* rows_map, int rows, int d, const float* gain, float eps,
                  const void* w, const void* bias, int C, const ttv_fsq_params* fsq, float* z_out, void* codes, int* indices,
                  float* bounded, hipStream_t s);
int ttvk_patch_copy(bool scatter, void* const* clips, const int* clip_desc, int clip0, int n_clips, int pt, int ph, int pw,
                    int C, void* patches, int ld, int dtype, int max_patches, hipStream_t s);
int ttvk_rope_apply(void* x, int dtype, int ld, int rows, int heads, const float* cs, hipStream_t s);
int ttvk_histogram(const int* idx, int n, int64_t* counts, int size, hipStream_t s);
int ttvk_quant_rows_fp8(const void* in, int in_dtype, int ld_in, const float* gain, float eps, void* out, int ld_out, float* scales, int rows,
                        int d, hipStream_t s);

int ttvk_split3_pack(const float* w, int ldw, void* out, int ldo, int rows, int K, hipStream_t s);
int64_t ttvk_mx_scale_ld(int d);
int ttvk_quant_mx_fp8(const void* in, int in_dtype, int ld_in, void* out, int ld_out, void* mx, float* row_scales, int rows, int d, hipStream_t s);

int ttvk_clip_from_u8(const void* frames, long long n_pix, void* clip, int dtype, hipStream_t s);

int ttvk_clip_resample_u8(void* const* src, void* const* dst, const int32_t* geom, int n_clips, int dtype, hipStream_t s);

enum GemmEpilogue {
  EPI_STORE = 0,
  EPI_QKV_ROPE,
  EPI_GEGLU,
  EPI_RESID_T,
  EPI_RESID_F32,
  EPI_RESID_NORM,
  EPI_STORE_PATCH,
  EPI_BIAS_PLAIN,
  EPI_BIAS_GELU,
  EPI_BIAS_RESID_F32R,
};

struct GemmArgs {
  const void* x; int ldx;
  const void* w; int ldw;
  int M, N, K;
  void* y; int ldy;
  const void* bias;
  const float* add_scalar;
  const void* resid; int ldr;
  float alpha;
  const float* rope_cs;
  const int* rope_ids; const float* rope_base;
  int rope_q_end, rope_k_begin, rope_k_end;
  int dtype;
  const float* norm_gain;
  float* sum_f32; int ld_sum;
  void* y2; int ldy2; const float* norm_gain2;
  void* yq; void* yq_mx;
  int split3;
  int x_image, y_image;
  int prenorm;
  const float* row_scale;
  const int* x_rows;
  float eps;
  int gather;
  void* const* clips;
  int n_clips;
  const int* clip_desc;
  const int* patch_rows;
  const int* row_seq;
  int patch_t, patch_h, patch_w;
  int resid_rows;
  int tile_run, tile_period;
};
struct ClipPtrs { void* p[TTV_MAX_CLIPS_PER_LAUNCH]; };
int ttvk_gemm(GemmEpilogue epi, const GemmArgs& a, hipStream_t s);
int ttvk_gemm_fp8(GemmEpilogue epi, const GemmArgs& a, const float* x_scale, const float* w_scale, hipStream_t s, const void* x_mx = nullptr,
                  const void* w_mx = nullptr);
bool ttvk_gemm_supports_resid_norm(int dtype, int N, int K);
bool ttvk_gemm_qkv_tiles_supported(int d_model, int gqa_dim, int ldw);

int ttvk_attention(const void* qkvg, int ld, void* out, int ldo, const int* cu_seqlens, const int* qblocks, int n_qblocks,
                   int q_heads, int kv_heads, int head_dim, int flags, int dtype, hipStream_t s, float* lse_out = nullptr,
                   void* out_raw = nullptr);

bool ttvk_attention_takes_swp(int flags);
int ttvk_attention_swp(const void* qkvg, int ld, void* out, int ldo, const int* cu_seqlens, const int* qblocks, int n_qblocks,
                       int q_heads, int kv_heads, int gate_mul, hipStream_t s, const void* rows2 = nullptr, int kwin = 0,
                       const float* state = nullptr);
int64_t ttvk_attention_swp_state_floats(int n_rows, int q_heads);
int ttvk_attention_swp_dump(const void* rows, int ld, int n_rows, int q_heads, int kv_heads, float* state, hipStream_t s);
int ttvk_attention_mxout(const void* qkvg, int ld, void* out_q, void* out_mx, int ld_mx, const int* cu_seqlens, const int* qblocks,
                         int n_qblocks, int q_heads, int kv_heads, hipStream_t s);

int ttvk_attention64(const void* qkvg, int ld, void* out, int ldo, const int* cu_seqlens, const int* items, int n_items, int q_heads,
                     int kv_heads, int flags, hipStream_t s);

int ttvk_vq_norms(const void* cb, int dtype, int ld, int N, int C, float* cnorm, hipStream_t s);
int64_t ttvk_vq_workspace_bytes(int rows);
int ttvk_vq_l2_argmin(const void* z, int dtype, int ldz, const void* cb, int ldc, const float* cnorm, int rows, int N, int C, int* indices,
                      float* best_dist, void* workspace, int64_t workspace_bytes, hipStream_t s);
int ttvk_vq_lookup(const void* cb, int dtype, int ldc, const int* indices, int rows, int C, void* codes, int ldo, hipStream_t s);
int ttvk_vq_lookup_bwd(const void* dcodes, int dtype, int ld, const int* indices, int rows, int C, float* dcb, int ldc, hipStream_t s);

int64_t ttvk_vq_train_workspace_bytes(int rows, int N);
int ttvk_vq_commit_forward(const void* z, int dtype, int ldz, const void* cb, int ldc, const int* idx, int rows, int N, int C, float* loss,
                           void* workspace, int64_t workspace_bytes, hipStream_t s);
int ttvk_vq_commit_backward(const void* g, int ldg, const void* z, int ldz, const void* e, int lde, int dtype, int rows, int C, double scale,
                            void* dz, int ldd, hipStream_t s);
int ttvk_vq_ema_stats(const void* z, int dtype, int ldz, const int* idx, int rows, int N, int C, const float* cluster_size, float dead_threshold,
                      uint64_t seed, const int64_t* ema_step, int rank, int world_size, float* stats, void* workspace, int64_t workspace_bytes,
                      hipStream_t s);
int ttvk_vq_ema_update(const float* stats, float* cluster_size, float* embed_avg, float* codebook, void* copy, int copy_dtype, float* cnorm,
                       int64_t* ema_step, int N, int C, float decay, float one_minus_decay, float eps, float dead_threshold, void* workspace,
                       int64_t workspace_bytes, hipStream_t s);

bool ttvk_mlp_fused_supported(int dtype, int width, int inner);
struct MlpNextQkv {
  void* qkv; int ld;
  const float* rope_cs;
  int rows;
  int rope_q_end, rope_k_begin, rope_k_end;
};
int64_t ttvk_mlp_pack_bytes(int inner, int next_qkv_rows);
int ttvk_mlp_pack(const void* w12_folded, const void* w3, const void* wo, const void* next_qkv_folded, int next_qkv_rows, int inner,
                  void* packed, hipStream_t s);
int ttvk_mlp_fused(const void* ao, int ldao, const float* front_gain, float front_alpha, const void* x, int ldx, const void* packed,
                   int inner, void* y, int ldy, const float* post_gain, float alpha, float eps, int M, const MlpNextQkv* nq, hipStream_t s);

int ttvk_l1_loss(void* const* recon, void* const* target, void* const* grad, const int* sizes, int n_clips, int total_clips, int dtype,
                 float* loss, hipStream_t s);
int ttvk_sq_err(void* const* recon, void* const* target, const int* sizes, int n_clips, int dtype, int clamp, double* acc2, hipStream_t s);
int ttvk_rmsnorm_bwd_chain(const void* x, int ldx, const void* dy, int lddy, const float* gain1, float* dgain1, float* dx, int lddx,
                           const void* y, int y_dt, int ldy, const float* gain2, float* dgain2, float out_scale, void* cast_out, int ldc, int rows,
                           int d, float eps, int dt, hipStream_t s);
int ttvk_rmsnorm_bwd(const void* x, int x_dt, int ldx, const int* xr, const void* dy, int dy_dt, int lddy, const int* dyr,
                     const float* gain, void* dx, int dx_dt, int lddx, const int* dxr, int acc, float* dgain, int rows, int d, float eps,
                     hipStream_t s);
int ttvk_colsum(const void* a, int dt, int lda, const int* rows_map, int rows, int n, float* out, hipStream_t s);
int ttvk_sumall(const void* a, int dt, int lda, const int* rows_map, int rows, int n, const float* colw, float scale, float* out, hipStream_t s);
int ttvk_gate_fwd(const void* a, int lda, const void* gate, int ldg, void* ag, int ldo, int rows, int d, int dt, hipStream_t s);
int ttvk_gate_bwd(const void* dag, int ldd, const void* a, int lda, const void* gate, int ldg, void* da, int ldda, void* dgate, int lddg,
                  int rows, int d, int dt, float* delta, hipStream_t s);
int ttvk_geglu_fwd(const void* u, int ldu, void* h, int ldh, int rows, int I, int dt, hipStream_t s);
int ttvk_geglu_bwd(const void* u, int ldu, const void* dh, int lddh, void* du, int lddu, int rows, int I, int dt, hipStream_t s);
int ttvk_scale_cast(const float* a, float alpha, float* b, void* c, int dt, long n, hipStream_t s);
int ttvk_to_f32(const void* a, int dt, float* b, long n, int accumulate, hipStream_t s);
int ttvk_fsq_bwd(const ttv_fsq_params* fp, const float* z, const void* dcodes, int dt, float* dz, int rows, hipStream_t s);
#define TTV_WGRAD_BATCH 6
struct WgradBatch {
  int n = 0;
  int64_t used_bytes = 0;
  struct Entry { const float* part; float* dw; int splits, lddw, N, K, tiles_n, tiles; } e[TTV_WGRAD_BATCH];
};
int ttvk_wgrad(const void* dy, int lddy, const void* x, int ldx, float* dw, int lddw, int L, int N, int K, int dt, float* part,
               int64_t part_bytes, hipStream_t s, WgradBatch* batch = nullptr);
int ttvk_wgrad_flush(WgradBatch* batch, hipStream_t s);
int64_t ttvk_wgrad_ws_bytes(int L, int N, int K);
int ttvk_outer_small(const void* a, int a_dt, int lda, int C, const void* b, int b_dt, int ldb, const int* b_rows, float* dw, int lddw,
                     int transpose_out, int rows, int d, hipStream_t s);
int ttvk_expand_small(const void* a, int a_dt, int lda, int C, const void* w, int w_dt, int ldw, int w_cf, void* out, int o_dt, int ldo,
                      int rows, int d, hipStream_t s);
int ttvk_reduce_small(const void* a, int a_dt, int lda, const int* a_rows, const void* w, int w_dt, int ldw, int C, float* out, int ldo,
                      int rows, int d, hipStream_t s);
int ttvk_attention_bwd(const void* qkvg, int ld, const void* o, int ldo, const void* dout, int ldd, const float* lse, float* delta,
                       const int* cu, const int* blocks64, int n_blocks64, const int* row_seq, void* dqkvg, int ldg, float* dkv_scratch,
                       int total_rows, int hq, int hkv, int dt, const float* rope_cs, hipStream_t s, int delta_ready = 0, const int* qlim_desc = nullptr);
int ttvk_rope_apply_dir(void* x, int dtype, int ld, int rows, int heads, const float* cs, int conj, hipStream_t s);
int ttvk_dec_embed_ex(const void* codes, int C, const void* w, const void* bias, const float* mask_token, const float* gain, void* x,
                      int dtype, int ld, const int* rows_map, int rows, int d, float eps, void* hpre, hipStream_t s);
int ttvk_const_rows_bwd(const float* colsum, const float* mask_token, const float* gain, int dt, float eps, float* dgain, float* dmask,
                        int d, hipStream_t s);
int ttvk_rope_build(const float* base_cos, const float* base_sin, int n_ids, int F, const int* clip_desc, const int* cu, const int* row_seq,
                    float* out, int total_rows, hipStream_t s);

int64_t ttvk_ssim_workspace_bytes(const int32_t* dims, int n_clips);
int ttvk_ssim(void* const* recon, void* const* target, const int32_t* dims, int n_clips, int dtype, int clamp, double* acc2, void* workspace,
              int64_t workspace_bytes, hipStream_t s);

int ttvk_lpips_crops_forward(void* const* recon, void* const* target, const int32_t* clip_dims, int n_clips, const int32_t* crops, int n_crops,
                             int size, void* recon_crops, void* target_crops, int dtype, hipStream_t s);
int ttvk_lpips_crops_backward(void* const* recon, void* const* grad, const int32_t* clip_dims, int n_clips, const int32_t* crops, int n_crops,
                              int size, const void* g, int dtype, hipStream_t s);

int64_t ttvk_lpips_tape_bytes(int n, int H, int W, int dtype);
int64_t ttvk_lpips_workspace_bytes(int n, int H, int W, int dtype);
int ttvk_lpips_forward(const ttv_lpips_weights* w, const void* recon, const void* target, int n, int H, int W, int dtype, float* lpips,
                       float* gram, void* tape, void* ws, int64_t ws_bytes, hipStream_t s);
int ttvk_lpips_backward(const ttv_lpips_weights* w, const void* tape, int n, int H, int W, int dtype, const float* glpips, const float* ggram,
                        void* drecon, void* ws, int64_t ws_bytes, hipStream_t s);
int64_t ttvk_lpips_eval_workspace_bytes(int frames, int H, int W, int dtype);
int ttvk_lpips_eval_accumulate(const ttv_lpips_weights* w, void* const* recon, void* const* target, const int32_t* frames, int n_clips, int H,
                               int W, int dtype, int clamp_recon, float* per_frame, double* acc, void* ws, int64_t ws_bytes, hipStream_t s);
int64_t ttvk_lpips_conv_workspace_bytes(int N, int H, int W, int Cin, int Cout, int dtype);
int ttvk_lpips_conv3x3(const void* x, int N, int H, int W, int Cin, int Cout, const void* w, const float* bias, int mode, const void* h,
                       void* y, int dtype, void* ws, int64_t ws_bytes, hipStream_t s);
int ttvk_lpips_maxpool(const void* x, int N, int H, int W, int C, void* y, int dtype, hipStream_t s);
int ttvk_lpips_maxpool_backward(const void* dy, const float* add, const void* h, int N, int H, int W, int C, void* dx, int dtype, hipStream_t s);

int64_t ttvk_i3d_workspace_bytes(int n);
int ttvk_fvd_preprocess(void* const* clips, const int32_t* dims, int n_clips, int dtype, int clamp, float* out, hipStream_t s);
int ttvk_i3d_features(const ttv_i3d_weights* w, const float* x, int n, float* feats, void* ws, int64_t ws_bytes, hipStream_t s);
int ttvk_i3d_conv3d(const float* x, int N, int T, int H, int W, int Cin, int k, int stride, const float* w, const float* scale,
                    const float* shift, int Cout, int relu, float* y, int ldc, int c_off, hipStream_t s);
int ttvk_i3d_maxpool3d(const float* x, int N, int T, int H, int W, int C, int kt, int kh, int kw, int st, int sh, int sw, float* y,
                       hipStream_t s);

int ttvk_jedi_preprocess(void* const* clips, const int32_t* dims, int n_clips, int dtype, void* out, hipStream_t s);
int64_t ttvk_vjepa_workspace_bytes(int n);
int ttvk_vjepa_features(const ttv_vjepa_weights* w, const void* x, int n, float* feats, int finetuned, void* ws, int64_t ws_bytes,
                        hipStream_t s);
// ... 52 lines not shown
```

titok_video_amd/csrc/ttv_mlp.hip:

```cpp
#include "ttv_common.h"
#include "ttv_kernels.h"

#define MLP_W12_CHUNKS 2048
#define MLP_W3_CHUNKS 1024
#define MLP_PANEL_CHUNKS (MLP_W12_CHUNKS + MLP_W3_CHUNKS)
#define MLP_WO_CHUNKS (4 * MLP_W12_CHUNKS)

struct MlpDev {
  const bf16_t* x; int ldx;
  const uint4* pack;
  const bf16_t* ao; int ldao;
  const float* front_gain;
  float front_alpha;
  bf16_t* qkv; int ldq;
  const float* rope_cs;
  int nqp, rope_q_end, rope_k_begin, rope_k_end;
  int I;
  bf16_t* y; int ldy;
  const float* post_gain;
  float alpha, eps;
  int M, n_tiles, debug;
  long long* stamps;
};

__global__ void k_mlp_pack(const bf16_t* __restrict__ w12f, const bf16_t* __restrict__ w3, const bf16_t* __restrict__ wo,
                           const bf16_t* __restrict__ wq, int nq_rows, int I, uint4* __restrict__ out) {
  const int np = I / 32;
  const int nqp = (nq_rows + 63) / 64;
  const int o = blockIdx.x * blockDim.x + threadIdx.x;
  if (o >= np * MLP_PANEL_CHUNKS + MLP_WO_CHUNKS + nqp * MLP_W12_CHUNKS) return;
  if (o >= np * MLP_PANEL_CHUNKS + MLP_WO_CHUNKS) {
    const int c = o - np * MLP_PANEL_CHUNKS - MLP_WO_CHUNKS, qp = c / MLP_W12_CHUNKS, cc = c - qp * MLP_W12_CHUNKS;
    const int r = cc >> 5, cp = cc & 31;
    const int ch = (cp & 16) | ((cp & 15) ^ (r & 15));
    int srow = qp * 64 + r;
    srow = srow < nq_rows ? srow : nq_rows - 1;
    const bf16_t* src = wq + (size_t)srow * 256 + (ch >> 2) * 32 + (ch & 3) * 4;
    const uint2 lo = *reinterpret_cast<const uint2*>(src), hi = *reinterpret_cast<const uint2*>(src + 16);
    out[o] = make_uint4(lo.x, lo.y, hi.x, hi.y);
    return;
  }
  if (o >= np * MLP_PANEL_CHUNKS) {
    const int c = o - np * MLP_PANEL_CHUNKS, wp = c / MLP_W12_CHUNKS, cc = c - wp * MLP_W12_CHUNKS;
    const int r = cc >> 5, cp = cc & 31;
    const int ch = (cp & 16) | ((cp & 15) ^ (r & 15));
    out[o] = wo ? *reinterpret_cast<const uint4*>(wo + (size_t)(wp * 64 + r) * 256 + ch * 8) : make_uint4(0, 0, 0, 0);
    return;
  }
  const int pn = o / MLP_PANEL_CHUNKS, c = o - pn * MLP_PANEL_CHUNKS;
  if (c < MLP_W12_CHUNKS) {
    const int r = c >> 5, cp = c & 31;
    const int ch = (cp & 16) | ((cp & 15) ^ (r & 15));
    const int srow = r < 32 ? pn * 32 + r : I + pn * 32 + (r - 32);
    const bf16_t* src = w12f + (size_t)srow * 256 + (ch >> 2) * 32 + (ch & 3) * 4;
    const uint2 lo = *reinterpret_cast<const uint2*>(src), hi = *reinterpret_cast<const uint2*>(src + 16);
    out[o] = make_uint4(lo.x, lo.y, hi.x, hi.y);
  } else {
    const int c3 = c - MLP_W12_CHUNKS, kq = c3 >> 8, row = c3 & 255;
    bf16x8 v;
#pragma unroll
    for (int j = 0; j < 8; ++j) v[j] = w3[(size_t)row * I + pn * 32 + (j < 4 ? 4 * kq + j : 16 + 4 * kq + (j - 4))];
    out[o] = __builtin_bit_cast(uint4, v);
  }
}

typedef uint32_t u32x2_t __attribute__((ext_vector_type(2)));
typedef uint32_t u32x4_t __attribute__((ext_vector_type(4)));
__device__ __forceinline__ f32x4 cvt4(bf16x4 b) { return (f32x4){(float)b[0], (float)b[1], (float)b[2], (float)b[3]}; }
#define MLP_LD12(img_, t_, s8_)                                                                                    \
  __builtin_bit_cast(bf16x8, (img_)[((t_) * 16 + l15) * 32 + ((((s8_) * 4 + kq) & 16) | ((((s8_) * 4 + kq) & 15) ^ l15))])
#define MLP_GLDS_4(src_, dst_)                                                                                     \
  do {                                                                                                             \
    unsigned keep__;                                                                                               \
    asm volatile("s_mov_b32 %0, m0\n\t"                                                                            \
                 "s_mov_b32 m0, %6\n\ts_nop 0\n\tglobal_load_lds_dwordx4 %1, %5\n\t"                               \
                 "s_add_u32 m0, %6, 0x2000\n\ts_nop 0\n\tglobal_load_lds_dwordx4 %2, %5\n\t"                       \
                 "s_add_u32 m0, %6, 0x4000\n\ts_nop 0\n\tglobal_load_lds_dwordx4 %3, %5\n\t"                       \
                 "s_add_u32 m0, %6, 0x6000\n\ts_nop 0\n\tglobal_load_lds_dwordx4 %4, %5\n\t"                       \
                 "s_mov_b32 m0, %0"                                                                                \
                 : "=&s"(keep__)                                                                                   \
                 : "v"(lane16), "v"(lane16 + 8192u), "v"(lane16 + 16384u), "v"(lane16 + 24576u), "s"(src_), "s"(dst_) \
                 : "memory", "scc");                                                                               \
  } while (0)
#define MLP_GLDS_2(src_, dst_)                                                                                     \
  do {                                                                                                             \
    unsigned keep__;                                                                                               \
    asm volatile("s_mov_b32 %0, m0\n\t"                                                                            \
                 "s_mov_b32 m0, %4\n\ts_nop 0\n\tglobal_load_lds_dwordx4 %1, %3\n\t"                               \
                 "s_add_u32 m0, %4, 0x2000\n\ts_nop 0\n\tglobal_load_lds_dwordx4 %2, %3\n\t"                       \
                 "s_mov_b32 m0, %0"                                                                                \
                 : "=&s"(keep__)                                                                                   \
                 : "v"(lane16), "v"(lane16 + 8192u), "s"(src_), "s"(dst_)                                          \
                 : "memory", "scc");                                                                               \
  } while (0)
#ifdef MLP_STAMPS
#define MLP_STAMP()                                                                                                \
  do {                                                                                                             \
    if (p.stamps && blockIdx.x == 0 && (wave & 3) == 0 && lane == 0 && n_stamp < 64)                               \
      p.stamps[(wave >> 2) * 64 + n_stamp++] = (long long)__builtin_readcyclecounter();                            \
  } while (0)
#else
#define MLP_STAMP() do { (void)n_stamp; } while (0)
#endif

template <int TPB, int T1, int T2, bool GELU_FIRST, bool KEEL, bool FRONT, bool BACK>
__device__ __forceinline__ void mlp_wave(const MlpDev& p, uint4* l12, uint4* l3, uint4* hb, const float* gl, int tile, int wave, int lane,
                                         int P1F, int P2F, int& n_stamp) {
  constexpr int T1A = T1 > 0 ? T1 : 1, T2A = T2 > 0 ? T2 : 1;
  const int l15 = lane & 15, kq = lane >> 4;
  const int np = p.I / 32;
  const uint32_t lane16 = lane * 16;
  const uint32_t lds_l12 = (uint32_t)(uintptr_t)(__attribute__((address_space(3))) void*)l12;
  const uint32_t lds_l3 = (uint32_t)(uintptr_t)(__attribute__((address_space(3))) void*)l3;
#define GLDS_W12(pn_, buf_)                                                                                        \
  do {                                                                                                             \
    const uint4* src__ = p.pack + ((size_t)(pn_) * MLP_PANEL_CHUNKS + wave * 64);                                  \
    const uint32_t dst__ = lds_l12 + ((buf_) * MLP_W12_CHUNKS + wave * 64) * 16;                                   \
    MLP_GLDS_4(src__, dst__);                                                                                      \
  } while (0)
#define GLDS_W3(pn_, buf_)                                                                                         \
  do {                                                                                                             \
    const uint4* src__ = p.pack + ((size_t)(pn_) * MLP_PANEL_CHUNKS + MLP_W12_CHUNKS + wave * 64);                 \
    const uint32_t dst__ = lds_l3 + ((buf_) * MLP_W3_CHUNKS + wave * 64) * 16;                                     \
    MLP_GLDS_2(src__, dst__);                                                                                      \
  } while (0)

  const int tok0 = tile * (16 * TPB) + l15;
  typedef __attribute__((address_space(1))) char gchar;
  typedef __attribute__((address_space(1))) const char gcchar;
  gcchar* const gx = (gcchar*)p.x;
  gcchar* const gao = (gcchar*)p.ao;
  gchar* const gy = (gchar*)p.y;

  MLP_STAMP();
  __syncthreads();

  bf16x8 bfr[T1A][8];
  float rstd[T1A];
  if (FRONT) {
#define GLDS_WO(wp_, buf_)                                                                                         \
  do {                                                                                                             \
    const uint4* src__ = p.pack + ((size_t)np * MLP_PANEL_CHUNKS + (wp_) * MLP_W12_CHUNKS + wave * 64);            \
    const uint32_t dst__ = lds_l12 + ((buf_) * MLP_W12_CHUNKS + wave * 64) * 16;                                   \
    MLP_GLDS_4(src__, dst__);                                                                                      \
  } while (0)
    GLDS_WO(0, 0);
    bf16x8 abf[T1A][8];
#pragma unroll
    for (int j = 0; j < T1; ++j) {
      const int t = tok0 + 16 * (P1F + j);
      const int tc = t < p.M ? t : p.M - 1;
      const uint32_t aoff = ((uint32_t)tc * (uint32_t)p.ldao + kq * 8) * 2u;
#pragma unroll
      for (int s8 = 0; s8 < 8; ++s8) abf[j][s8] = *(const __attribute__((address_space(1))) bf16x8*)(gao + aoff + s8 * 64);
    }
    f32x4 facc[16][T1A];
    __builtin_amdgcn_s_waitcnt(0x0F70);
    __syncthreads();
#pragma unroll
    for (int wp = 0; wp < 4; ++wp) {
      if (wp + 1 < 4) GLDS_WO(wp + 1, (wp + 1) & 1);
      const uint4* img = l12 + (wp & 1) * MLP_W12_CHUNKS;
      bf16x8 a[2][4];
      if constexpr (T1 > 0) {
#pragma unroll
      for (int i = 0; i < 4; ++i) a[0][i] = MLP_LD12(img, i, 0);
#pragma unroll
      for (int s8 = 0; s8 < 8; ++s8) {
        if (s8 + 1 < 8) {
#pragma unroll
          for (int i = 0; i < 4; ++i) a[(s8 + 1) & 1][i] = MLP_LD12(img, i, s8 + 1);
        }
#pragma unroll
        for (int i = 0; i < 4; ++i)
#pragma unroll
          for (int j = 0; j < T1; ++j)
            facc[4 * wp + i][j] = __builtin_amdgcn_mfma_f32_16x16x32_bf16(a[s8 & 1][i], abf[j][s8],
                                                                           s8 ? facc[4 * wp + i][j] : (f32x4){0.f, 0.f, 0.f, 0.f}, 0, 0, 0);
        if (s8 + 1 < 8) __builtin_amdgcn_sched_group_barrier(0x100, 4, 0);
        __builtin_amdgcn_sched_group_barrier(0x008, 4 * T1A, 0);
        __builtin_amdgcn_sched_barrier(0);
      }
      }
      __builtin_amdgcn_s_waitcnt(0x0F70);
      __syncthreads();
    }
#undef GLDS_WO
    GLDS_W12(0, 0);
#pragma unroll
    for (int j = 0; j < T1; ++j) {
      const int t = tok0 + 16 * (P1F + j);
      const int tc = t < p.M ? t : p.M - 1;
      const uint32_t roff = ((uint32_t)tc * (uint32_t)p.ldx + kq * 4) * 2u;
      float ss = 0.f;
#pragma unroll
      for (int m = 0; m < 16; ++m) {
        facc[m][j] += p.front_alpha * cvt4(*(const __attribute__((address_space(1))) bf16x4*)(gx + roff + m * 32));
#pragma unroll
        for (int e = 0; e < 4; ++e) ss = fmaf(facc[m][j][e], facc[m][j][e], ss);
      }
      float scale = 1.0f;
      if (p.front_gain) {
        ss = quad16_sum(ss);
        scale = 1.0f / sqrtf(ss * (1.0f / 256.0f) + p.eps);
      }
      float ss2 = 0.f;
#pragma unroll
      for (int s8 = 0; s8 < 8; ++s8) {
        bf16x4 q[2];
#pragma unroll
// ... 257 lines not shown
      const int t = tok0 + 16 * (P2F + j);
      qv[j] = t < p.M;
      const int tc = qv[j] ? t : p.M - 1;
      qoff[j] = ((uint32_t)tc * (uint32_t)p.ldq + kq * 4) * 2u;
      gcchar* cs = grope + ((uint32_t)tc * 64u + kq * 2) * 4u;
#pragma unroll
      for (int i = 0; i < 4; ++i) {
        rc[i][j] = *(const __attribute__((address_space(1))) f32x2*)(cs + i * 32);
        rs[i][j] = *(const __attribute__((address_space(1))) f32x2*)(cs + 128 + i * 32);
      }
    }
    __builtin_amdgcn_s_waitcnt(0x0F70);
    __syncthreads();
    for (int qp = 0; qp < p.nqp; ++qp) {
      if (qp + 1 < p.nqp) GLDS_WQ(qp + 1, (qp + 1) & 1);
      const uint4* img = l12 + (qp & 1) * MLP_W12_CHUNKS;
      f32x4 qa[4][T2A];
      bf16x8 a[2][4];
#pragma unroll
      for (int i = 0; i < 4; ++i) a[0][i] = MLP_LD12(img, i, 0);
#pragma unroll
      for (int s8 = 0; s8 < 8; ++s8) {
        if (s8 + 1 < 8) {
#pragma unroll
          for (int i = 0; i < 4; ++i) a[(s8 + 1) & 1][i] = MLP_LD12(img, i, s8 + 1);
        }
#pragma unroll
        for (int i = 0; i < 4; ++i)
#pragma unroll
          for (int j = 0; j < T2; ++j)
            qa[i][j] = __builtin_amdgcn_mfma_f32_16x16x32_bf16(a[s8 & 1][i], xq[j][s8], s8 ? qa[i][j] : (f32x4){0.f, 0.f, 0.f, 0.f}, 0, 0, 0);
        if (s8 + 1 < 8) __builtin_amdgcn_sched_group_barrier(0x100, 4, 0);
        __builtin_amdgcn_sched_group_barrier(0x008, 4 * T2A, 0);
        __builtin_amdgcn_sched_barrier(0);
      }
      __builtin_amdgcn_s_waitcnt(0x0F70);
      __syncthreads();
      const int f_first = qp * 64;
      const bool rot = f_first < p.rope_q_end || (f_first >= p.rope_k_begin && f_first < p.rope_k_end);
#pragma unroll
      for (int j = 0; j < T2; ++j) {
        const bool odd = kq & 1;
        gchar* const qrow = gq + (qoff[j] - (uint32_t)(kq * 4) * 2u) + (uint32_t)(f_first + (odd ? 16 + kq * 4 - 4 : kq * 4)) * 2u;
#pragma unroll
        for (int ip = 0; ip < 2; ++ip) {
          uint2 pk[2];
#pragma unroll
          for (int u = 0; u < 2; ++u) {
            const int i = 2 * ip + u;
            f32x4 v = qa[i][j] * rstdq[j];
            if (rot)
              v = (f32x4){v[0] * rc[i][j].x - v[1] * rs[i][j].x, v[0] * rs[i][j].x + v[1] * rc[i][j].x,
                          v[2] * rc[i][j].y - v[3] * rs[i][j].y, v[2] * rs[i][j].y + v[3] * rc[i][j].y};
            const bf16x4 q = {(bf16_t)v[0], (bf16_t)v[1], (bf16_t)v[2], (bf16_t)v[3]};
            pk[u] = __builtin_bit_cast(uint2, q);
          }
          const uint4 ox = xchg16_pair(pk[0], pk[1]);
          const u32x4_t ov = {ox.x, ox.y, ox.z, ox.w};
          if (qv[j]) *(__attribute__((address_space(1))) u32x4_t*)(qrow + ip * 64) = ov;
        }
      }
    }
#undef GLDS_WQ
    MLP_STAMP();
  }
#undef GLDS_W12
#undef GLDS_W3
}

template <int TILES, bool KEEL, bool FRONT, bool BACK>
__global__ __launch_bounds__(512, 1) void k_mlp256(MlpDev p) {
  extern __shared__ __attribute__((aligned(16))) uint4 smem[];
  uint4* const l12 = smem;
  uint4* const l3 = smem + 2 * MLP_W12_CHUNKS;
  uint4* const hb = l3 + 2 * MLP_W3_CHUNKS;
  float* const gl = reinterpret_cast<float*>(hb + 2 * TILES * 64);
  if (threadIdx.x < 256) {
    gl[threadIdx.x] = p.post_gain ? p.post_gain[threadIdx.x] : 1.0f;
    gl[256 + threadIdx.x] = (FRONT && p.front_gain) ? p.front_gain[threadIdx.x] : 1.0f;
  }
  const int lane = threadIdx.x & 63;
  const int wave = __builtin_amdgcn_readfirstlane(threadIdx.x >> 6);
  int n_stamp = 0;
  const int tile = blockIdx.x;
  if constexpr (TILES == 9) {
    if (wave < 4) mlp_wave<9, 2, 0, false, KEEL, FRONT, BACK>(p, l12, l3, hb, gl, tile, wave, lane, 2 * wave, 0, n_stamp);
    else if (wave < 6) mlp_wave<9, 0, 3, false, KEEL, FRONT, BACK>(p, l12, l3, hb, gl, tile, wave, lane, 0, 3 * (wave - 4), n_stamp);
    else if (wave == 6) mlp_wave<9, 1, 1, false, KEEL, FRONT, BACK>(p, l12, l3, hb, gl, tile, wave, lane, 8, 6, n_stamp);
    else mlp_wave<9, 0, 2, false, KEEL, FRONT, BACK>(p, l12, l3, hb, gl, tile, wave, lane, 0, 7, n_stamp);
  } else {
    constexpr int NT = TILES / 4;
    constexpr int TA = NT - NT / 2;
    const int g0 = (wave & 3) * NT;
    if (wave < 4) mlp_wave<TILES, TA, NT - TA, false, KEEL, FRONT, BACK>(p, l12, l3, hb, gl, tile, wave, lane, g0, g0 + TA, n_stamp);
    else mlp_wave<TILES, NT - TA, TA, false, KEEL, FRONT, BACK>(p, l12, l3, hb, gl, tile, wave, lane, g0 + TA, g0, n_stamp);
  }
}
#undef MLP_LD12
#undef MLP_GLDS_4
#undef MLP_GLDS_2
#undef MLP_STAMP

bool ttvk_mlp_fused_supported(int dtype, int width, int inner) { return dtype == TTV_BF16 && width == 256 && inner % 32 == 0 && inner > 0; }

int64_t ttvk_mlp_pack_bytes(int inner, int next_qkv_rows) {
  if (inner <= 0 || inner % 32 != 0 || next_qkv_rows < 0) return 0;
  return ((int64_t)(inner / 32) * MLP_PANEL_CHUNKS + MLP_WO_CHUNKS + (int64_t)((next_qkv_rows + 63) / 64) * MLP_W12_CHUNKS) * 16;
}

int ttvk_mlp_pack(const void* w12_folded, const void* w3, const void* wo, const void* next_qkv_folded, int next_qkv_rows, int inner,
                  void* packed, hipStream_t s) {
  TTV_CHECK_ARG(w12_folded && w3 && packed, "mlp_pack: null buffer");
  TTV_CHECK_ARG(inner > 0 && inner % 32 == 0, "mlp_pack: inner %% 32");
  TTV_CHECK_ARG((next_qkv_folded != nullptr) == (next_qkv_rows > 0), "mlp_pack: next_qkv weight and row count must come together");
  TTV_CHECK_ARG(((uintptr_t)w12_folded % 16 == 0) && ((uintptr_t)packed % 16 == 0) && ((uintptr_t)wo % 16 == 0) &&
                    ((uintptr_t)next_qkv_folded % 16 == 0), "mlp_pack: 16-byte alignment");
  const int total = inner / 32 * MLP_PANEL_CHUNKS + MLP_WO_CHUNKS + (next_qkv_rows + 63) / 64 * MLP_W12_CHUNKS;
  hipLaunchKernelGGL(k_mlp_pack, dim3(ttv_cdiv(total, 256)), dim3(256), 0, s, (const bf16_t*)w12_folded, (const bf16_t*)w3,
                     (const bf16_t*)wo, (const bf16_t*)next_qkv_folded, next_qkv_rows, inner, (uint4*)packed);
  TTV_CHECK_LAUNCH("mlp_pack");
  return TTV_OK;
}

int ttvk_mlp_fused(const void* ao, int ldao, const float* front_gain, float front_alpha, const void* x, int ldx, const void* packed,
                   int inner, void* y, int ldy, const float* post_gain, float alpha, float eps, int M, const MlpNextQkv* nq, hipStream_t s) {
  if (M == 0) return TTV_OK;
  TTV_CHECK_ARG(x && packed && y, "mlp_fused: null buffer");
  TTV_CHECK_ARG(inner % 32 == 0 && ldx % 8 == 0 && ldy % 8 == 0 && (!ao || ldao % 8 == 0), "mlp_fused: inner %% 32, leading dims %% 8");
  TTV_CHECK_ARG(((uintptr_t)x % 16 == 0) && ((uintptr_t)packed % 16 == 0) && ((uintptr_t)y % 16 == 0) && ((uintptr_t)ao % 16 == 0),
                "mlp_fused: 16-byte alignment");
  MlpDev d;
  d.x = (const bf16_t*)x; d.ldx = ldx; d.pack = (const uint4*)packed; d.I = inner;
  d.ao = (const bf16_t*)ao; d.ldao = ldao; d.front_gain = front_gain; d.front_alpha = front_alpha;
  d.y = (bf16_t*)y; d.ldy = ldy; d.post_gain = post_gain; d.alpha = alpha; d.eps = eps; d.M = M; d.debug = g_ttv_debug; d.stamps = g_ttv_stamps;
  d.qkv = nullptr; d.ldq = 0; d.rope_cs = nullptr; d.nqp = 0; d.rope_q_end = d.rope_k_begin = d.rope_k_end = 0;
  if (nq) {
    TTV_CHECK_ARG(nq->qkv && nq->rope_cs && nq->rows > 0 && nq->rows % 64 == 0 && nq->ld >= nq->rows && nq->ld % 4 == 0 &&
                      (uintptr_t)nq->qkv % 8 == 0, "mlp_fused: bad next-qkv arguments (rows %% 64, ld %% 4, 8-byte aligned)");
    TTV_CHECK_ARG(nq->rope_q_end % 64 == 0 && nq->rope_k_begin % 64 == 0 && nq->rope_k_end % 64 == 0, "mlp_fused: rotary ranges must be whole heads");
    d.qkv = (bf16_t*)nq->qkv; d.ldq = nq->ld; d.rope_cs = nq->rope_cs; d.nqp = nq->rows / 64;
    d.rope_q_end = nq->rope_q_end; d.rope_k_begin = nq->rope_k_begin; d.rope_k_end = nq->rope_k_end;
  }
  const int cus = 256;
  int tiles = 4;
  long best = -1;
  for (int c = 1; c <= 3; ++c) {
    const long cost = (long)ttv_cdiv(ttv_cdiv(M, 64 * c), cus) * (16 + 19 * c);
    if (best < 0 || cost < best) { best = cost; tiles = 4 * c; }
  }
  if (!nq && !(g_ttv_debug & TTV_DBG_MLP_PAIRS_ONLY)) {
    const long cost9 = (long)ttv_cdiv(ttv_cdiv(M, 144), cus) * (16 + 14 * 3);
    if (cost9 < best) { best = cost9; tiles = 9; }
  }
  if ((g_ttv_debug & TTV_DBG_MLP_TILES9) && !nq) tiles = 9;
  if (g_ttv_debug & TTV_DBG_MLP_TILES8) tiles = 8;
  if (g_ttv_debug & TTV_DBG_MLP_TILES4) tiles = 4;
  d.n_tiles = ttv_cdiv(M, 16 * tiles);
  const int grid = d.n_tiles;
  const size_t smem = (size_t)(2 * MLP_W12_CHUNKS + 2 * MLP_W3_CHUNKS + 2 * tiles * 64) * sizeof(uint4) + 2048;
  TtvProfScope prof(TTV_KC_GEMM_GEGLU, s);
#define LAUNCH_MLP(TILES_, KEEL_, FRONT_, BACK_)                                                                    \
  do {                                                                                                              \
    (void)hipFuncSetAttribute((const void*)k_mlp256<TILES_, KEEL_, FRONT_, BACK_>, hipFuncAttributeMaxDynamicSharedMemorySize, (int)smem); \
    hipLaunchKernelGGL((k_mlp256<TILES_, KEEL_, FRONT_, BACK_>), dim3(grid), dim3(512), smem, s, d);                \
  } while (0)
#define LAUNCH_MLP_F(TILES_, KEEL_)                                                                                 \
  do {                                                                                                              \
    if (ao && nq) LAUNCH_MLP(TILES_, KEEL_, true, true);                                                            \
    else if (ao) LAUNCH_MLP(TILES_, KEEL_, true, false);                                                            \
    else LAUNCH_MLP(TILES_, KEEL_, false, false);                                                                   \
  } while (0)
#define LAUNCH_MLP_9(KEEL_)                                                                                         \
  do {                                                                                                              \
    if (ao) LAUNCH_MLP(9, KEEL_, true, false);                                                                      \
    else LAUNCH_MLP(9, KEEL_, false, false);                                                                        \
  } while (0)
  TTV_CHECK_ARG(!nq || ao, "mlp_fused: the next-qkv part needs the out_proj front (ttv_layer_tail_fused)");
  if (post_gain) {
    if (tiles == 9) LAUNCH_MLP_9(true); else if (tiles == 12) LAUNCH_MLP_F(12, true); else if (tiles == 8) LAUNCH_MLP_F(8, true); else LAUNCH_MLP_F(4, true);
  } else {
    if (tiles == 9) LAUNCH_MLP_9(false); else if (tiles == 12) LAUNCH_MLP_F(12, false); else if (tiles == 8) LAUNCH_MLP_F(8, false); else LAUNCH_MLP_F(4, false);
  }
#undef LAUNCH_MLP_9
#undef LAUNCH_MLP_F
#undef LAUNCH_MLP
  TTV_CHECK_LAUNCH("mlp_fused");
  return TTV_OK;
}
```

titok_video_amd/csrc/ttv_plan.hip:

```cpp
#include <string.h>

#include "ttv_common.h"
#include "ttv_kernels.h"

struct PlanRowsArgs {
  const int* cu;
  const int* desc;
  int* latent_rows;
  int* patch_rows;
  int* row_seq;
  int* rope_ids;
  int n, L, sum_tokens, sum_patches, n_ids;
};

template <typename End>
__device__ __forceinline__ int plan_find(int n, int v, End end) {
  int lo = 0, hi = n - 1;
  while (lo < hi) {
    const int mid = (lo + hi) >> 1;
    if (end(mid) > v) hi = mid;
    else lo = mid + 1;
  }
  return lo;
}
// ... 48 lines not shown
          a.rope_ids[(size_t)(r0 + e) * 2] = w0[e];
          a.rope_ids[(size_t)(r0 + e) * 2 + 1] = w1[e];
        }
    }
    return;
  }
  g -= gA;
  const bool lat = g < gB;
  if (!lat) g -= gB;
  if (g >= (lat ? gB : gC)) return;
  const int total = lat ? a.sum_tokens : a.sum_patches;
  int* out = lat ? a.latent_rows : a.patch_rows;
  auto pbase = [&](int i) { return i < n ? a.desc[i * 8 + 6] : a.sum_patches; };
  auto first = [&](int i) { return lat ? a.cu[i] - pbase(i) : pbase(i); };
  const int m0 = g * 4, cnt = min(4, total - m0);
  int b = plan_find(n, m0, [&](int i) { return first(i + 1); });
  int v[4];
  int end = first(b + 1);
  int shift = lat ? a.cu[b] - first(b) : a.cu[b + 1] - end;
#pragma unroll
  for (int e = 0; e < 4; ++e) {
    const int m = m0 + e;
    if (e < cnt) {
      while (m >= end && b + 1 < n) {
        ++b;
        end = first(b + 1);
        shift = lat ? a.cu[b] - first(b) : a.cu[b + 1] - end;
      }
      v[e] = m + shift;
    } else v[e] = 0;
  }
  if (cnt == 4) *reinterpret_cast<int4*>(out + m0) = make_int4(v[0], v[1], v[2], v[3]);
  else {
#pragma unroll
    for (int e = 0; e < 3; ++e)
      if (e < cnt) out[m0 + e] = v[e];
  }
}

extern "C" int ttv_plan_rows_build(const ttv_plan_sizes* sz, const int32_t* host_segment, int32_t* dev_segment, const float* base_cos,
                                   const float* base_sin, int n_freqs, float* rope_cs, const float* rope_base, ttv_batch* batch, void* stream) {
  TTV_CHECK_ARG(sz && host_segment && dev_segment && base_cos && base_sin && rope_cs && batch, "plan_rows_build: null argument");
  TTV_CHECK_ARG(sz->n_clips >= 1 && sz->total_rows >= 1 && sz->sum_tokens >= 0 && sz->sum_patches >= 1 &&
                    (int64_t)sz->sum_tokens + sz->sum_patches == sz->total_rows && sz->total_rows <= INT32_MAX / 2,
                "plan_rows_build: sizes are not those of ttv_plan_rows_sizes");
  TTV_CHECK_ARG(sz->n_rope_ids >= 1 && sz->n_rope_ids <= 65535, "plan_rows_build: %d rotary position ids", sz->n_rope_ids);
  TTV_CHECK_ARG(n_freqs >= 1 && 3 * n_freqs <= 32, "plan_rows_build: bad rotary table shape");
  TTV_CHECK_ARG(sz->host_words >= 4 && sz->dev_words >= sz->host_words && ((uintptr_t)dev_segment & 15) == 0,
                "plan_rows_build: the device segment must be 16-byte aligned and hold dev_words words");
  hipStream_t s = (hipStream_t)stream;
  if (hipMemcpyAsync(dev_segment, host_segment, (size_t)sz->host_words * 4, hipMemcpyHostToDevice, s) != hipSuccess) {
    (void)hipGetLastError();
    ttv_set_error("plan_rows_build: hipMemcpyAsync failed");
    return TTV_ERR_LAUNCH;
  }
  PlanRowsArgs a;
  a.cu = dev_segment + sz->off_cu_seqlens;
  a.desc = dev_segment + sz->off_clip_desc;
  a.latent_rows = dev_segment + sz->off_latent_rows;
  a.patch_rows = dev_segment + sz->off_patch_rows;
  a.row_seq = dev_segment + sz->off_row_seq;
  a.rope_ids = dev_segment + sz->off_rope_ids;
  a.n = sz->n_clips; a.L = sz->total_rows; a.sum_tokens = sz->sum_tokens; a.sum_patches = sz->sum_patches; a.n_ids = sz->n_rope_ids;
  const int groups = (a.L + 3) / 4 + (a.sum_tokens + 3) / 4 + (a.sum_patches + 3) / 4;
  hipLaunchKernelGGL(k_plan_rows, dim3(ttv_cdiv(groups, 256)), dim3(256), 0, s, a);
  TTV_CHECK_LAUNCH("plan_rows");
  const int rc = ttvk_rope_build(base_cos, base_sin, sz->n_rope_ids, n_freqs, a.desc, a.cu, a.row_seq, rope_cs, a.L, s);
  if (rc != TTV_OK) return rc;

  memset(batch, 0, sizeof(*batch));
  batch->n_clips = sz->n_clips;
  batch->total_rows = sz->total_rows;
  batch->sum_tokens = sz->sum_tokens;
  batch->sum_patches = sz->sum_patches;
  batch->max_patches_per_clip = sz->max_patches_per_clip;
  batch->cu_seqlens = a.cu;
  batch->latent_rows = a.latent_rows;
  batch->patch_rows = a.patch_rows;
  batch->clip_desc = a.desc;
  batch->rope_cs = rope_cs;
  batch->blocks64 = dev_segment + sz->off_blocks64;
  batch->row_seq = a.row_seq;
  batch->n_blocks64 = sz->n_blocks64;
  if (rope_base) {
    batch->rope_ids = a.rope_ids;
    batch->rope_base = rope_base;
  }
  return TTV_OK;
}

extern "C" int ttv_plan_attn_set(const ttv_plan_attn* sz, const int32_t* host_tables, int32_t* dev_tables, ttv_batch* batch, void* stream) {
  TTV_CHECK_ARG(sz && host_tables && dev_tables && batch, "plan_attn_set: null argument");
  TTV_CHECK_ARG(sz->n_qblocks >= 1 && sz->words >= 4 * (int64_t)sz->n_qblocks && ((uintptr_t)dev_tables & 15) == 0,
                "plan_attn_set: sizes are not those of ttv_plan_attn_sizes, or the device buffer is not 16-byte aligned");
  if (hipMemcpyAsync(dev_tables, host_tables, (size_t)sz->words * 4, hipMemcpyHostToDevice, (hipStream_t)stream) != hipSuccess) {
    (void)hipGetLastError();
    ttv_set_error("plan_attn_set: hipMemcpyAsync failed");
    return TTV_ERR_LAUNCH;
  }
  batch->qblocks = dev_tables + sz->off_qblocks;
  batch->n_qblocks = sz->n_qblocks;
  batch->qblocks_paired = 0;
  batch->qblocks_all_full = sz->qblocks_all_full;
  batch->items64 = nullptr;
  batch->n_items64 = 0;
  batch->qblocks_latent = sz->n_qblocks_latent ? dev_tables + sz->off_qblocks_latent : nullptr;
  batch->n_qblocks_latent = sz->n_qblocks_latent;
  batch->qblocks_patch = sz->n_qblocks_patch ? dev_tables + sz->off_qblocks_patch : nullptr;
  batch->n_qblocks_patch = sz->n_qblocks_patch;
  return TTV_OK;
}
```

titok_video_amd/csrc/ttv_qkv256.inc:

```
#ifdef QKV_STAMPS
#define QK_STAMP_DECL unsigned long long qst_prev__ = 0, qst_acc__[8] = {0, 0, 0, 0, 0, 0, 0, 0}
#define QK_STAMP_START()                                                                                     \
  do {                                                                                                       \
    __builtin_amdgcn_sched_barrier(0);                                                                       \
    asm volatile("s_memtime %0\n\ts_waitcnt lgkmcnt(0)" : "=s"(qst_prev__)::"memory");                       \
    __builtin_amdgcn_sched_barrier(0);                                                                       \
  } while (0)
#define QK_STAMP(seg_)                                                                                       \
  do {                                                                                                       \
    unsigned long long t__;                                                                                  \
    __builtin_amdgcn_sched_barrier(0);                                                                       \
    asm volatile("s_memtime %0\n\ts_waitcnt lgkmcnt(0)" : "=s"(t__)::"memory");                              \
    __builtin_amdgcn_sched_barrier(0);                                                                       \
    qst_acc__[seg_] += t__ - qst_prev__;                                                                     \
    qst_prev__ = t__;                                                                                        \
  } while (0)
#else
#define QK_STAMP_DECL
#define QK_STAMP_START()
#define QK_STAMP(seg_)
#endif
typedef unsigned qk_u32x4 __attribute__((ext_vector_type(4)));
typedef unsigned qk_u32x2 __attribute__((ext_vector_type(2)));
template <bool PRENORM>
__global__ __launch_bounds__(256, 2) void k_qkv256(GemmDev p, int n_panels, int total_items) {
  __shared__ uint4 wl[2][K256_ROWS * 32];

  const int tid = threadIdx.x, lane = tid & 63;
  const int wave = __builtin_amdgcn_readfirstlane(tid >> 6);
  const int r = lane & 31, h = lane >> 5;
  const int lb = xcd_remap(blockIdx.x, gridDim.x);
  const int it0 = (int)((long)total_items * lb / gridDim.x);
  const int it1 = (int)((long)total_items * (lb + 1) / gridDim.x);
  if (it0 >= it1) return;
  const bf16_t* X = (const bf16_t*)p.x;

  const uint32_t wl_lds = (uint32_t)(uintptr_t)(__attribute__((address_space(3))) void*)&wl[0][0];
  const uint32_t dchunk0 = (uint32_t)(((lane & 16) | ((lane & 15) ^ h)) * 16);
  const uint32_t drow0 = (uint32_t)h * (uint32_t)p.ldw * 2u;
  const uint32_t dstride = (uint32_t)p.ldw * 4u;
#define QK_DMA_PIECE(dc_, i_, src_, dst_)                                                                       \
  do {                                                                                                       \
    unsigned keep__;                                                                                         \
    const uint32_t voff__ = ((dc_) ^ (uint32_t)((i_) << 5)) + drow0;                                            \
    asm volatile("s_mov_b32 %0, m0\n\ts_mov_b32 m0, %3\n\ts_nop 0\n\tglobal_load_lds_dwordx4 %1, %2\n\ts_mov_b32 m0, %0" \
                 : "=&s"(keep__) : "v"(voff__), "s"((src_) + (size_t)(i_) * dstride), "s"((dst_) + (i_) * 1024) : "memory"); \
  } while (0)
#define QK_PANEL_SRC(panel_) (reinterpret_cast<const char*>(p.w) + ((size_t)(panel_) * 64 + wave * 16) * (size_t)p.ldw * 2)
#define QK_PANEL_DST(buf_) (wl_lds + (buf_) * (K256_ROWS * 512) + wave * (16 * 512))

  const int r15 = r & 15;
  const char* const wl_base = reinterpret_cast<const char*>(&wl[0][0]);
  const uint32_t aoff0 = (uint32_t)(r * 32 + (h ^ r15)) * 16u;
#define QK_AFRAG(buf_, t_, ks_) \
  (*reinterpret_cast<const bf16x8*>(wl_base + (a0__ ^ (uint32_t)(((ks_) & 7) << 5)) + (buf_) * (K256_ROWS * 512) + (t_) * (32 * 512) + (((ks_) >> 3) & 1) * 256))

  bf16x8 bfr[16];
  float rstd = 1.f;
  float2 rcs[2][4][2];
  char* ytok = nullptr;
  uint2 idp = make_uint2(0u, 0u);
  int tk = 0;
  bool tok_ok = true, wave_full = true;
  int cur_tile = -1;
  int pend = 0;
  int pend_panel = 0;
  const f32x16 zero16 = {0.f, 0.f, 0.f, 0.f, 0.f, 0.f, 0.f, 0.f, 0.f, 0.f, 0.f, 0.f, 0.f, 0.f, 0.f, 0.f};

#define QK_ROT(acc_, ROT_, G_)                                                                               \
  do {                                                                                                       \
    const int t__ = (G_) >> 2, g__ = (G_) & 3;                                                               \
    const float a0__ = acc_[t__][4 * g__], a1__ = acc_[t__][4 * g__ + 1], a2__ = acc_[t__][4 * g__ + 2], a3__ = acc_[t__][4 * g__ + 3]; \
    if (ROT_) {                                                                                              \
      const float2 k0__ = rcs[t__][g__][0], k1__ = rcs[t__][g__][1];                                         \
      o_[0] = a0__ * k0__.x - a1__ * k0__.y; o_[1] = a0__ * k0__.y + a1__ * k0__.x;                          \
      o_[2] = a2__ * k1__.x - a3__ * k1__.y; o_[3] = a2__ * k1__.y + a3__ * k1__.x;                          \
    } else {                                                                                                 \
      o_[0] = a0__ * rstd; o_[1] = a1__ * rstd; o_[2] = a2__ * rstd; o_[3] = a3__ * rstd;                    \
    }                                                                                                        \
    asm volatile("" : "+v"(o_[0]), "+v"(o_[1]), "+v"(o_[2]), "+v"(o_[3]));                                   \
  } while (0)
#define QK_PACK(G_)                                                                                          \
  do {                                                                                                       \
    const int g__ = (G_) & 3;                                                                                \
    const bf16x4 b__ = {(bf16_t)o_[0], (bf16_t)o_[1], (bf16_t)o_[2], (bf16_t)o_[3]};                         \
    pk_[g__ & 1] = __builtin_bit_cast(qk_u32x2, b__);                                                        \
    if (g__ & 1) {                                                                                           \
      const auto sx__ = __builtin_amdgcn_permlane32_swap(pk_[0].x, pk_[1].x, false, false);                  \
      const auto sy__ = __builtin_amdgcn_permlane32_swap(pk_[0].y, pk_[1].y, false, false);                  \
      out_ = (qk_u32x4){sx__[0], sy__[0], sx__[1], sy__[1]};                                                 \
      asm volatile("" : "+v"(out_));                                                                         \
    } else {                                                                                                 \
      asm volatile("" : "+v"(pk_[0]));                                                                       \
    }                                                                                                        \
  } while (0)
#define QK_STORE_CHUNK(c_, panel_)                                                                           \
  do {                                                                                                       \
    if (tok_ok && !(p.debug & TTV_DBG_NO_STORES)) *reinterpret_cast<qk_u32x4*>(ytok + (size_t)(panel_) * 128 + (c_) * 32) = out_; \
  } while (0)
#define QK_EPILOGUE(acc_, ROT_, panel_)                                                                      \
  do {                                                                                                       \
    float o_[4]; qk_u32x2 pk_[2]; qk_u32x4 out_;                                                             \
    _Pragma("unroll") for (int G__ = 0; G__ < 8; ++G__) {                                                    \
      QK_ROT(acc_, ROT_, G__);                                                                               \
// ... 10 lines not shown
    uint32_t a0__ = aoff0, dc0__ = dchunk0;                                                                  \
    asm volatile("" : "+v"(a0__), "+v"(dc0__));    \
    af__[0][0] = QK_AFRAG(buf_, 0, 0);                                                                       \
    af__[0][1] = QK_AFRAG(buf_, 1, 0);                                                                       \
    __builtin_amdgcn_sched_barrier(0);                                                                       \
    _Pragma("unroll") for (int ks__ = 0; ks__ < 16; ++ks__) {                                                \
      if (ks__ < 8 && has_next__) {                                                                          \
        if (ks__ == 0) QK_DMA_PIECE(dc0__, 0, nsrc__, ndst__); else if (ks__ == 1) QK_DMA_PIECE(dc0__, 1, nsrc__, ndst__);  \
        else if (ks__ == 2) QK_DMA_PIECE(dc0__, 2, nsrc__, ndst__); else if (ks__ == 3) QK_DMA_PIECE(dc0__, 3, nsrc__, ndst__); \
        else if (ks__ == 4) QK_DMA_PIECE(dc0__, 4, nsrc__, ndst__); else if (ks__ == 5) QK_DMA_PIECE(dc0__, 5, nsrc__, ndst__); \
        else if (ks__ == 6) QK_DMA_PIECE(dc0__, 6, nsrc__, ndst__); else QK_DMA_PIECE(dc0__, 7, nsrc__, ndst__);            \
      }                                                                                                      \
      if (MODE_ == 0 && ks__ == 8) {                                                                         \
        int hq__ = h;                                                                                        \
        asm volatile("" : "+v"(hq__));       \
        if (p.rope_ids) {                                                                                    \
          _Pragma("unroll") for (int t__ = 0; t__ < 2; ++t__)                                                \
            _Pragma("unroll") for (int g__ = 0; g__ < 4; ++g__)                                              \
              _Pragma("unroll") for (int e__ = 0; e__ < 2; ++e__) {                                          \
                const int pp__ = 16 * t__ + 4 * g__ + 2 * hq__ + e__;                                        \
                const int f__ = pp__ < 30 ? pp__ / 3 : 0, ax__ = pp__ < 30 ? pp__ - 3 * (pp__ / 3) : 3;      \
                const uint32_t wd__ = (ax__ & 2) ? idp.y : idp.x;                                            \
                const uint32_t id__ = (ax__ & 1) ? (wd__ >> 16) : (wd__ & 0xffffu);                          \
                rcs[t__][g__][e__] = *reinterpret_cast<const float2*>(reinterpret_cast<const char*>(p.rope_base) + id__ * 80u + (uint32_t)f__ * 8u); \
              }                                                                                              \
        } else {                                                                                             \
          const float* c__ = p.rope_cs + (size_t)tk * 64 + 2 * hq__;                                         \
          _Pragma("unroll") for (int t__ = 0; t__ < 2; ++t__)                                                \
            _Pragma("unroll") for (int g__ = 0; g__ < 4; ++g__) {                                            \
              const float2 cc__ = *reinterpret_cast<const float2*>(c__ + 16 * t__ + 4 * g__);                \
              const float2 sn__ = *reinterpret_cast<const float2*>(c__ + 32 + 16 * t__ + 4 * g__);           \
              rcs[t__][g__][0] = make_float2(cc__.x, sn__.x);                                                \
              rcs[t__][g__][1] = make_float2(cc__.y, sn__.y);                                                \
            }                                                                                                \
        }                                                                                                    \
      }                                                                                                      \
      __builtin_amdgcn_sched_barrier(0);                                                                     \
      if (ks__ + 1 < 16) {                                                                                   \
        af__[(ks__ + 1) & 1][0] = QK_AFRAG(buf_, 0, ks__ + 1);                                               \
        af__[(ks__ + 1) & 1][1] = QK_AFRAG(buf_, 1, ks__ + 1);                                               \
      }                                                                                                      \
      cur_[0] = __builtin_amdgcn_mfma_f32_32x32x16_bf16(af__[ks__ & 1][0], bfr[ks__], ks__ ? cur_[0] : zero16, 0, 0, 0); \
      cur_[1] = __builtin_amdgcn_mfma_f32_32x32x16_bf16(af__[ks__ & 1][1], bfr[ks__], ks__ ? cur_[1] : zero16, 0, 0, 0); \
      if (MODE_) {                                                                                           \
        if ((ks__ & 1) == 0) QK_ROT(prev_, MODE_ == 2, ks__ >> 1); else QK_PACK(ks__ >> 1);                  \
      } else if (PRENORM) {                                                                                  \
        const bf16x8 v__ = bfr[ks__];                                                                        \
        ss0__ = __builtin_amdgcn_fdot2_f32_bf16((bf16x2){v__[0], v__[1]}, (bf16x2){v__[0], v__[1]}, ss0__, false); \
        ss1__ = __builtin_amdgcn_fdot2_f32_bf16((bf16x2){v__[2], v__[3]}, (bf16x2){v__[2], v__[3]}, ss1__, false); \
        ss0__ = __builtin_amdgcn_fdot2_f32_bf16((bf16x2){v__[4], v__[5]}, (bf16x2){v__[4], v__[5]}, ss0__, false); \
        ss1__ = __builtin_amdgcn_fdot2_f32_bf16((bf16x2){v__[6], v__[7]}, (bf16x2){v__[6], v__[7]}, ss1__, false); \
        asm volatile("" : "+v"(ss0__), "+v"(ss1__));                                                         \
      }                                                                                                      \
      if (ks__ + 1 < 16) __builtin_amdgcn_sched_group_barrier(0x100, 2, 0);                                  \
      __builtin_amdgcn_sched_group_barrier(0x008, 1, 0);                                                     \
      if (MODE_) { if ((ks__ & 1) || MODE_ != 2) __builtin_amdgcn_sched_group_barrier(0x002, 2, 0); else __builtin_amdgcn_sched_group_barrier(0x002, 4, 0); } \
      else if (PRENORM) __builtin_amdgcn_sched_group_barrier(0x002, 2, 0);                                   \
      __builtin_amdgcn_sched_group_barrier(0x008, 1, 0);                                                     \
      if (MODE_) { if ((ks__ & 1) || MODE_ != 2) __builtin_amdgcn_sched_group_barrier(0x002, 2, 0); else __builtin_amdgcn_sched_group_barrier(0x002, 4, 0); } \
      else if (PRENORM) __builtin_amdgcn_sched_group_barrier(0x002, 2, 0);                                   \
      __builtin_amdgcn_sched_barrier(0);                                                                     \
      if (MODE_ && (ks__ & 3) == 3) {                                                                        \
        QK_STORE_CHUNK(ks__ >> 2, pend_panel);                                                               \
        __builtin_amdgcn_sched_barrier(0);                                                                   \
      }                                                                                                      \
    }                                                                                                        \
    if (MODE_ == 0) {                                                                                        \
      if (PRENORM) {                                                                                         \
        float ss__ = ss0__ + ss1__;                                                                          \
        ss__ = pair32_sum(ss__);                                                                    \
        rstd = 1.0f / sqrtf(ss__ * (1.0f / 256.0f) + p.eps);                                                 \
      }                                                                                                      \
      _Pragma("unroll") for (int t__ = 0; t__ < 2; ++t__)                                                    \
        _Pragma("unroll") for (int g__ = 0; g__ < 4; ++g__)                                                  \
          _Pragma("unroll") for (int e__ = 0; e__ < 2; ++e__)                                                \
            rcs[t__][g__][e__] = make_float2(rcs[t__][g__][e__].x * rstd, rcs[t__][g__][e__].y * rstd);      \
    }                                                                                                        \
  } while (0)

#define QK_STEP(cur_, prev_, it_)                                                                            \
  do {                                                                                                       \
    const int it__ = (it_);                                                                                  \
    const int buf__ = (it__ - it0) & 1;                                                                      \
    const int tile__ = it__ / n_panels, panel__ = it__ - tile__ * n_panels;                                  \
    if (tile__ != cur_tile) {                                                                                \
      cur_tile = tile__;                                                                                     \
       \
                                                                               \
        \
      const int ttile__ = p.tile_period ? (tile__ / p.tile_run) * p.tile_period + tile__ % p.tile_run : tile__; \
      const int t0__ = ttile__ * K256_TT + wave * 32;                                                        \
      int ntk__ = t0__ + r;                                                                                  \
      const bool nok__ = ntk__ < p.M;                                                                        \
      ntk__ = nok__ ? ntk__ : p.M - 1;                                                                       \
      const bf16_t* xr__ = X + (size_t)(p.x_rows ? p.x_rows[ntk__] : ntk__) * p.ldx + h * 8;                 \
      _Pragma("unroll") for (int ks__ = 0; ks__ < 16; ++ks__) bfr[ks__] = *reinterpret_cast<const bf16x8*>(xr__ + ks__ * 16); \
      uint2 nidp__ = make_uint2(0u, 0u);                                                                     \
      if (p.rope_ids) nidp__ = *reinterpret_cast<const uint2*>(p.rope_ids + 2 * (size_t)ntk__);              \
      if (pend == 2) QK_EPILOGUE(prev_, true, pend_panel); else if (pend == 1) QK_EPILOGUE(prev_, false, pend_panel); \
      pend = 0;                                                                                              \
       \
       \
       \
      _Pragma("unroll") for (int ks__ = 0; ks__ < 16; ++ks__) asm volatile("" : "+v"(bfr[ks__]));            \
      tk = ntk__; tok_ok = nok__; idp = nidp__;                                                              \
      wave_full = t0__ + 32 <= p.M;                                                                          \
      ytok = reinterpret_cast<char*>((bf16_t*)p.y + (size_t)tk * p.ldy) + h * 16;                            \
      rstd = 1.f;                                                                                            \
    }                                                                                                        \
    QK_STAMP(0);                                                                                             \
    if (it__ == it0) {                                                                                       \
      asm volatile("s_waitcnt vmcnt(0)" ::: "memory");                                                       \
      __syncthreads();                                                                                       \
    }                                                                                                        \
    QK_STAMP(1);                                                                                             \
    const bool has_next__ = it__ + 1 < it1;                                                                  \
    const char* nsrc__ = QK_PANEL_SRC((it__ + 1) % n_panels);                                                \
    const uint32_t ndst__ = QK_PANEL_DST(buf__ ^ 1);                                                         \
    const int f_first__ = panel__ * 64;                                                                      \
    const int rot__ = (f_first__ < p.rope_q_end || (f_first__ >= p.rope_k_begin && f_first__ < p.rope_k_end)) ? 2 : 1; \
    bool counted__ = false;                                                                                  \
    if (pend == 2) {                                                                                         \
      if (buf__) QK_BODY(cur_, prev_, 1, 2); else QK_BODY(cur_, prev_, 0, 2);                                \
      counted__ = wave_full && !(p.debug & TTV_DBG_NO_STORES);                                                               \
      QK_STAMP(2);                                                                                           \
    } else if (pend == 1) {                                                                                  \
      if (buf__) QK_BODY(cur_, prev_, 1, 1); else QK_BODY(cur_, prev_, 0, 1);                                \
      counted__ = wave_full && !(p.debug & TTV_DBG_NO_STORES);                                                               \
      QK_STAMP(2);                                                                                           \
    } else {                                                                                                 \
      if (buf__) QK_BODY(cur_, prev_, 1, 0); else QK_BODY(cur_, prev_, 0, 0);                                \
      QK_STAMP(3);                                                                                           \
    }                                                                                                        \
     \
    if (counted__) asm volatile("s_waitcnt vmcnt(3)" ::: "memory");                                          \
    else asm volatile("s_waitcnt vmcnt(0)" ::: "memory");                                                    \
    QK_STAMP(4);                                                                                             \
    __builtin_amdgcn_s_barrier();                                                                            \
    QK_STAMP(5);                                                                                             \
    pend = rot__;                                                                                            \
    pend_panel = panel__;                                                                                    \
  } while (0)

  f32x16 accA[2], accB[2];
  QK_STAMP_DECL;
  {
    const char* src0 = QK_PANEL_SRC(it0 % n_panels);
    const uint32_t dst0 = QK_PANEL_DST(0);
    QK_DMA_PIECE(dchunk0, 0, src0, dst0); QK_DMA_PIECE(dchunk0, 1, src0, dst0); QK_DMA_PIECE(dchunk0, 2, src0, dst0); QK_DMA_PIECE(dchunk0, 3, src0, dst0);
    QK_DMA_PIECE(dchunk0, 4, src0, dst0); QK_DMA_PIECE(dchunk0, 5, src0, dst0); QK_DMA_PIECE(dchunk0, 6, src0, dst0); QK_DMA_PIECE(dchunk0, 7, src0, dst0);
  }
  QK_STAMP_START();
  int it = it0;
  for (; it + 1 < it1; it += 2) {
    QK_STEP(accA, accB, it);
    QK_STEP(accB, accA, it + 1);
  }
  if (it < it1) {
    QK_STEP(accA, accB, it);
    if (pend == 2) QK_EPILOGUE(accA, true, pend_panel); else QK_EPILOGUE(accA, false, pend_panel);
  } else {
    if (pend == 2) QK_EPILOGUE(accB, true, pend_panel); else QK_EPILOGUE(accB, false, pend_panel);
  }
  QK_STAMP(6);
#ifdef QKV_STAMPS
  if (p.stamps && lb % 16 == 0 && lane == 0) {
    long long* dst = p.stamps + ((size_t)(lb / 16) * 4 + wave) * 8;
    for (int i = 0; i < 7; ++i) dst[i] = (long long)qst_acc__[i];
    dst[7] = it1 - it0;
  }
#endif
#undef QK_DMA_PIECE
#undef QK_PANEL_SRC
#undef QK_PANEL_DST
#undef QK_AFRAG
#undef QK_ROT
#undef QK_PACK
#undef QK_STORE_CHUNK
#undef QK_EPILOGUE
#undef QK_BODY
#undef QK_STEP
}
```

titok_video_amd/plan.py:

```python
from __future__ import annotations

import ctypes as C
import functools
import math
from typing import List, Optional, Sequence, Tuple

import numpy as np
import torch

from . import _lib, switches

QBLOCK = 128
ATTN_SLOTS = 1024


@functools.lru_cache(maxsize=8)
def _rope_base_table(head_dim: int, nd: int, n_ids: int, theta: float = 10000.0):
    f = head_dim // (2 * nd)
    inv = torch.pow(theta, torch.linspace(0.0, 1.0, f, dtype=torch.float64)) * torch.pi / 2.0
    ids = torch.arange(n_ids, dtype=torch.float32).to(torch.float64)
    ang = ids.view(-1, 1) * inv.view(1, -1)
    fc = torch.polar(torch.ones(1, dtype=torch.float64), ang)
    return fc.real.to(torch.float32).numpy(), fc.imag.to(torch.float32).numpy()

# ... 86 lines not shown
    for l in lists:
        out.extend(l[depth:])
    return np.asarray(out, dtype=np.int32).reshape(-1, 2)


class BatchPlan:

    def __init__(self, pixel_grids: Sequence[Sequence[int]], token_counts: Sequence[int], patch: Sequence[int],
                 device: torch.device, head_dim: int = 64):
        if head_dim != 64:
            raise ValueError("head_dim is fixed at 64 (reference model/base/utils.py:8)")
        self.device = torch.device(device)
        self.patch = tuple(int(p) for p in patch)
        self.pixel_grids = [tuple(int(v) for v in g) for g in pixel_grids]
        self.token_counts = [int(k) for k in token_counts]
        if len(self.pixel_grids) != len(self.token_counts) or not self.pixel_grids:
            raise ValueError("need one token count per clip and at least one clip")
        grids, sizes = [], []
        for pg in self.pixel_grids:
            if len(pg) != len(self.patch) or any(v <= 0 or v % p for v, p in zip(pg, self.patch)):
                raise ValueError(f"clip shape {pg} is not a positive multiple of patch size {self.patch}")
            g = tuple(v // p for v, p in zip(pg, self.patch))
            grids.append(g)
            sizes.append(math.prod(g))
        if any(k < 0 for k in self.token_counts):
            raise ValueError("token counts must be >= 0")
        self.grids, self.grid_sizes = grids, sizes
        B = len(grids)
        cu = [0]
        for k, p in zip(self.token_counts, sizes):
            if k + p <= 0:
                raise ValueError("empty sequence")
            cu.append(cu[-1] + k + p)
        self.cu_seqlens = cu
        self.total_rows = cu[-1]
        self.sum_tokens = sum(self.token_counts)
        self.sum_patches = sum(sizes)
        self.max_seqlen = max(k + p for k, p in zip(self.token_counts, sizes))

        latent_rows = np.concatenate([np.arange(cu[b], cu[b] + self.token_counts[b], dtype=np.int32) for b in range(B)])
        patch_rows = np.concatenate([np.arange(cu[b] + self.token_counts[b], cu[b + 1], dtype=np.int32) for b in range(B)])
        desc = np.zeros((B, 8), dtype=np.int32)
        pbase = 0
        for b in range(B):
            T, H, W = self.pixel_grids[b]
            desc[b] = (T, H, W, grids[b][0], grids[b][1], grids[b][2], pbase, 3)
            pbase += sizes[b]
        n_ids = 512
        while n_ids < max(k + max(g) for g, k in zip(grids, self.token_counts)) + 1:
            n_ids *= 2
        self.n_rope_ids = n_ids
        ids = np.concatenate([_clip_rope_ids(grids[b], self.token_counts[b], n_ids) for b in range(B)], axis=0)
        rope_ids = ids.view(np.int32).reshape(-1)
        blocks64 = _xcd_interleave([[(b, r0) for r0 in range(0, cu[b + 1] - cu[b], 64)] for b in range(B)])
        row_seq = np.concatenate([np.full(cu[b + 1] - cu[b], b, dtype=np.int32) for b in range(B)])
        self.n_blocks64 = int(blocks64.shape[0])
        parts = [np.asarray(cu, dtype=np.int32), latent_rows, patch_rows, desc.reshape(-1), blocks64.reshape(-1), row_seq, rope_ids]
        offs, total = [], 0
        for p in parts:
            offs.append(total)
            total += (p.size + 3) // 4 * 4
        host = np.zeros(total, dtype=np.int32)
        for o, p in zip(offs, parts):
            host[o:o + p.size] = p
        self.int_tables = _upload(host, self.device)
        base = self.int_tables.data_ptr()
        if self.device.type == "cuda":
            bc, bs = _rope_base_device(head_dim, len(self.patch), n_ids, str(self.device))
            self.rope_cs = torch.empty((self.total_rows, head_dim), dtype=torch.float32, device=self.device)
            rc = _lib.lib().ttv_rope_table_build(bc.data_ptr(), bs.data_ptr(), n_ids, bc.shape[1], base + 4 * offs[3], base + 4 * offs[0],
                                                 base + 4 * offs[5], self.rope_cs.data_ptr(), self.total_rows,
                                                 _lib.stream_ptr(self.device))
            _lib.check(rc, "ttv_rope_table_build")
            self.build_stream = torch.cuda.current_stream(self.device)
            self.ready = torch.cuda.Event()
            self.ready.record(self.build_stream)
        else:
            rope = np.concatenate([_rope_clip_table(g, k, head_dim) for g, k in zip(grids, self.token_counts)], axis=0)
            self.rope_cs = torch.from_numpy(rope).to(self.device)

        self._base_fields = dict(
            n_clips=B, total_rows=self.total_rows, sum_tokens=self.sum_tokens, sum_patches=self.sum_patches,
            max_patches_per_clip=max(sizes),
            cu_seqlens=base + 4 * offs[0], latent_rows=base + 4 * offs[1], patch_rows=base + 4 * offs[2],
            clip_desc=base + 4 * offs[3], rope_cs=self.rope_cs.data_ptr(),
            blocks64=base + 4 * offs[4], row_seq=base + 4 * offs[5], n_blocks64=self.n_blocks64)
        if self.device.type == "cuda" and len(self.patch) == 3 and switches.flag("TTV_ROPE_IDS", True):
            self._rope_base_cs = _rope_base_interleaved(head_dim, len(self.patch), n_ids, str(self.device))
            self._base_fields.update(rope_ids=base + 4 * offs[6], rope_base=self._rope_base_cs.data_ptr())
        self._offs = offs
        self._attn = {}
        self._attn_all_full = {}
        self._batch_structs = {}
        self.reader_streams = {}

    def use_on_current_stream(self) -> None:
        if self.device.type != "cuda":
            return
        cur = torch.cuda.current_stream(self.device)
        if cur != self.build_stream and cur.cuda_stream not in self.reader_streams:
            cur.wait_event(self.ready)
        self.reader_streams[cur.cuda_stream] = cur

    def retire(self) -> None:
        if self.device.type != "cuda":
            return
        cur = torch.cuda.current_stream(self.device)
        build = getattr(self, "build_stream", None)
        for st in self.reader_streams.values():
            if st != cur:
                cur.wait_stream(st)
            if build is not None and build != cur and st != build:
                build.wait_stream(st)

    def attention_table(self, q_heads: int, kv_heads: int, split: Optional[bool] = None) -> torch.Tensor:
        if split is None and switches.text("TTV_ATTN_SPLIT") in ("0", "1"):
            split = switches.text("TTV_ATTN_SPLIT") == "1"
        key = (int(q_heads), int(kv_heads), split)
        t = self._attn.get(key)
        if t is None:
            rep = q_heads // kv_heads
            n_items = sum(-(-(self.cu_seqlens[b + 1] - self.cu_seqlens[b]) // QBLOCK) for b in range(len(self.grids))) * q_heads
            small_grid = n_items < ATTN_SLOTS
            units_full, units_half = [], []
            for b in range(len(self.grids)):
                s = self.cu_seqlens[b + 1] - self.cu_seqlens[b]
                nq = -(-s // QBLOCK)
                tail_div = 3 if small_grid else switches.integer("TTV_ATTN_TAIL_DIV", 0)
                first_half = 0 if split else (nq if (split is False or tail_div <= 0) else nq - nq // tail_div)
                for kvh in range(kv_heads):
                    heads = [kvh * rep + r for r in range(rep)]
                    units_full.append([(b, qb * QBLOCK, hd, 0) for qb in range(first_half) for hd in heads])
                    units_half.append([(b, q0, hd, 1) for qb in range(first_half, nq) for hd in heads
                                       for q0 in (qb * QBLOCK, qb * QBLOCK + 64) if q0 < s])
            order = sorted(range(len(units_full)), key=lambda i: len(units_full[i]) + len(units_half[i]) / 2, reverse=True)
            lists, weight, halves = [[] for _ in range(8)], [0.0] * 8, [[] for _ in range(8)]
            for i in order:
                x = min(range(8), key=lambda j: weight[j])
                lists[x].extend(units_full[i])
                halves[x].extend(units_half[i])
                weight[x] += len(units_full[i]) + len(units_half[i]) / 2
            for x in range(8):
                lists[x].extend(halves[x])
            depth = max(len(l) for l in lists)
            table = np.full((depth, 8, 4), -1, dtype=np.int32)
            for x, l in enumerate(lists):
                if l:
                    table[: len(l), x, :] = np.asarray(l, dtype=np.int32)
            flat = table.reshape(-1, 4)
            last = int(np.max(np.nonzero(flat[:, 0] >= 0)[0])) + 1
            t = _upload(np.ascontiguousarray(flat[:last]), self.device)
            self._attn[key] = t
            self._attn_all_full[t.data_ptr()] = not bool((flat[:last, 3] > 0).any())
        return t

    def attention_table_latent(self, q_heads: int, kv_heads: int) -> torch.Tensor:
        key = ("latent", int(q_heads), int(kv_heads))
        t = self._attn.get(key)
        if t is None:
            rep = q_heads // kv_heads
            units = []
            for b in range(len(self.grids)):
                nq = -(-int(self.token_counts[b]) // QBLOCK)
                for kvh in range(kv_heads):
                    units.append([(b, qb * QBLOCK, kvh * rep + r, 0) for qb in range(nq) for r in range(rep)])
            order = sorted(range(len(units)), key=lambda i: len(units[i]), reverse=True)
# ... 377 lines not shown
```

Measured before the change: 30780.

## Restrict last-layer QKV panels and run latent MLP in place on uniform batches

On the last layer of a tower, where only the latent or only the patch rows are consumed, the QKV GEMM now computes only the needed column panels for each row class (Q-only panels are skipped where just K/V are read). The latent-only MLP runs in place on the strided full-row buffer through a run/period row map, so the two gather copies are skipped. This adds per-item panel-range indexing and grid sizing in the K=256 QKV kernel. It applies only when batches have uniform clip shapes with 128-aligned latent and patch counts.

```diff
diff --git a/include/titok_hip.h b/include/titok_hip.h
--- a/include/titok_hip.h
+++ b/include/titok_hip.h
@@ -206,6 +206,7 @@
   int32_t n_qblocks_latent;
   const int32_t* qblocks_patch;
   int32_t n_qblocks_patch;
+  int32_t clip_latent_rows;
 } ttv_batch;
 
 int ttv_rope_table_build(const float* base_cos, const float* base_sin, int n_ids, int n_freqs, const int32_t* clip_desc,
@@ -516,7 +517,8 @@
   TTV_DBG_ENC_ALL_ROWS = 524288,
   TTV_DBG_ATTN_NO_SWP = 1048576,
   TTV_DBG_DEC_ALL_BLOCKS = 2097152,
-  TTV_DBG_DEC_L0_NO_CONST = 4194304
+  TTV_DBG_DEC_L0_NO_CONST = 4194304,
+  TTV_DBG_EDGE_NO_PANELS = 8388608
 };
 int ttv_debug_set(int flags);
 int ttv_debug_stamps(void* device_buffer);
diff --git a/titok_video_amd/_lib.py b/titok_video_amd/_lib.py
--- a/titok_video_amd/_lib.py
+++ b/titok_video_amd/_lib.py
@@ -41,6 +41,7 @@
 DBG_ATTN_NO_SWP = 1048576
 DBG_DEC_ALL_BLOCKS = 2097152
 DBG_DEC_L0_NO_CONST = 4194304
+DBG_EDGE_NO_PANELS = 8388608
 
 _HERE = os.path.dirname(os.path.abspath(__file__))
 LIB_PATH = switches.text("TTV_LIB_PATH") or os.path.join(_HERE, "libtitok_hip.so")
@@ -84,7 +85,7 @@
                 ("patch_rows", vp), ("clip_desc", vp), ("qblocks", vp), ("rope_cs", vp), ("blocks64", vp), ("row_seq", vp),
                 ("n_blocks64", i32), ("qblocks_paired", i32), ("qblocks_all_full", i32), ("items64", vp), ("n_items64", i32),
                 ("rope_ids", vp), ("rope_base", vp), ("qblocks_latent", vp), ("n_qblocks_latent", i32), ("qblocks_patch", vp),
-                ("n_qblocks_patch", i32)]
+                ("n_qblocks_patch", i32), ("clip_latent_rows", i32)]
 
 
 class PlanSizes(C.Structure):
diff --git a/titok_video_amd/csrc/ttv_api.hip b/titok_video_amd/csrc/ttv_api.hip
--- a/titok_video_amd/csrc/ttv_api.hip
+++ b/titok_video_amd/csrc/ttv_api.hip
@@ -25,6 +25,7 @@
 bool ttv_sw_fused_patch() { static const bool v = ttv_env_flag("TTV_FUSED_PATCH", true); return v; }
 bool ttv_sw_attn_pipe() { static const bool v = ttv_env_flag("TTV_ATTN_PIPE", false); return v; }
 static bool sw_dec_l0_const() { static const bool v = ttv_env_flag("TTV_DEC_L0_CONST", true); return v; }
+static bool sw_edge_panels() { static const bool v = ttv_env_flag("TTV_EDGE_PANELS", true); return v; }
 float ttv_sw_attn_thr() { static const float v = ttv_env_float("TTV_ATTN_THR", 8.0f); return v; }
 thread_local int g_ttv_debug = 0;
 long long* g_ttv_stamps = nullptr;
@@ -164,8 +165,10 @@
 
 struct PreNormW { const float* gain; const void *w, *w_pn, *w_f8; const float* w_f8_scale; bool f8; };
 
+struct QkvTiles { int run, period, begin_run, begin_rest; };
+
 static int prenorm_proj(const LayerCtx& c, GemmEpilogue epi, const char* x, int rows, const PreNormW& p, int N, char* y, int y_image,
-                        bool rstd_valid, int tile_run = 0, int tile_period = 0) {
+                        bool rstd_valid, QkvTiles tiles = {0, 0, 0, 0}) {
   const ttv_tower_dims* d = c.d;
   const TowerWs& ws = c.ws;
   const int dm = d->width, dt = d->dtype;
@@ -187,7 +190,8 @@
   a.row_scale = fold_gen ? ws.rstd : nullptr;
   a.x = fold ? x : ws.xn; a.w = fold ? p.w_pn : p.w;
   if (epi == EPI_QKV_ROPE) { a.rope_ids = c.b->rope_ids; a.rope_base = c.b->rope_ids ? c.b->rope_base : nullptr; }
-  a.tile_run = tile_run; a.tile_period = tile_period;
+  a.tile_run = tiles.run; a.tile_period = tiles.period;
+  a.panel_begin_run = tiles.begin_run; a.panel_begin_rest = tiles.begin_rest;
   return ttvk_gemm(epi, a, c.s);
 }
 
@@ -227,6 +231,20 @@
   if (c.pair || c.pipe || !c.all_full || (b->items64 && b->n_items64 > 0)) return false;
   return ttvk_gemm_qkv_tiles_supported(d->width, d->kv_heads * d->head_dim, d->width) &&
          ttvk_attention_takes_swp(TTV_ATTN_GATE | TTV_ATTN_QSCALED | TTV_ATTN_ALLFULL);
+}
+
+static bool edge_panels_ok(const LayerCtx& c, const ttv_tower_weights* w) {
+  const ttv_tower_dims* d = c.d;
+  const ttv_batch* b = c.b;
+  if (!sw_edge_panels() || (g_ttv_debug & TTV_DBG_EDGE_NO_PANELS)) return false;
+  if (d->dtype != TTV_BF16 || d->width != 256 || d->head_dim != 64 || c.split3) return false;
+  const int K = b->clip_latent_rows, P = b->max_patches_per_clip;
+  if (K <= 0 || P <= 0 || K % 128 || P % 128 || (int64_t)b->n_clips * K != b->sum_tokens || (int64_t)b->n_clips * P != b->sum_patches) return false;
+  const ttv_layer_weights& lw = w->layers[d->layers - 1];
+  if (!lw.to_qkv_pn || !lw.qkv_q_prescaled) return false;
+  if (rows_f8(d->dtype, d->width, lw.to_qkv_f8, lw.to_qkv_f8_scale, lw.to_qkv_mx, lw.to_qkv_pn)) return false;
+  if (c.pair || c.pipe || !c.all_full || (b->items64 && b->n_items64 > 0)) return false;
+  return ttvk_gemm_qkv_tiles_supported(d->width, d->kv_heads * d->head_dim, d->width, 2 * d->width);
 }
 
 static int run_layers(const ttv_tower_dims* d, const ttv_tower_weights* w, const ttv_batch* b, const TowerWs& ws, hipStream_t s,
@@ -249,6 +267,9 @@
   const LayerCtx ctx = {d, b, ws, s, split3, s3img, gen_ok, b->qblocks_paired ? TTV_ATTN_PAIRED : 0, b->qblocks_all_full ? TTV_ATTN_ALLFULL : 0,
                         ttv_sw_attn_pipe() ? TTV_ATTN_PIPE : 0};
   const bool l0_const = dec_l0_const_ok(ctx, w, l0);
+  const bool edge = edge_panels_ok(ctx, w);
+  const QkvTiles edge_tiles = {b->clip_latent_rows / 128, (b->clip_latent_rows + b->max_patches_per_clip) / 128, 0, 0};
+  const int kv_panel = 2 * dm / 64;
   for (int i = 0; i < d->layers; ++i) {
     const ttv_layer_weights& lw = w->layers[i];
     const bool last = i == d->layers - 1;
@@ -266,7 +287,12 @@
     if (!qkv_ready) {
       const void* w_plain = (dt == TTV_BF16 && lw.to_qkv_qs) ? lw.to_qkv_qs : lw.to_qkv;
       const PreNormW qw = {lw.pre_ln, w_plain, lw.to_qkv_pn, lw.to_qkv_f8, lw.to_qkv_f8_scale, f8_qkv};
-      if (l0c) TTV_TRY(prenorm_proj(ctx, EPI_QKV_ROPE, ws.x, L, qw, nq, ws.qkv, 0, rstd_valid, l0->latent_rows / 128, (l0->latent_rows + l0->patch_rows) / 128));
+      if (l0c) TTV_TRY(prenorm_proj(ctx, EPI_QKV_ROPE, ws.x, L, qw, nq, ws.qkv, 0, rstd_valid,
+                                    {l0->latent_rows / 128, (l0->latent_rows + l0->patch_rows) / 128, 0, nq / 64}));
+      else if (edge && last && lat_last)
+        TTV_TRY(prenorm_proj(ctx, EPI_QKV_ROPE, ws.x, L, qw, nq, ws.qkv, 0, rstd_valid, {edge_tiles.run, edge_tiles.period, 0, kv_panel}));
+      else if (edge && last && pat_last)
+        TTV_TRY(prenorm_proj(ctx, EPI_QKV_ROPE, ws.x, L, qw, nq, ws.qkv, 0, rstd_valid, {edge_tiles.run, edge_tiles.period, kv_panel, 0}));
       else TTV_TRY(prenorm_proj(ctx, EPI_QKV_ROPE, ws.x, L, qw, nq, ws.qkv, s3img ? 2 : 0, rstd_valid));
     }
     const bool q_scaled = dt == TTV_BF16 && (lw.to_qkv_pn ? lw.qkv_q_prescaled != 0 : lw.to_qkv_qs != nullptr);
@@ -290,13 +316,22 @@
     char* cx = ws.x;
     char* cao = ws.ao;
     int Lc = L;
+    static const bool fused_mlp_env = ttv_env_flag("TTV_FUSED_MLP", true);
+    const bool lat_in_place = lat_now && edge && fused_mlp_env && ttvk_mlp_fused_supported(dt, dm, d->inner) && lw.mlp_pack &&
+                              ttvk_mlp_fused_takes_rows(b->sum_tokens, b->clip_latent_rows, b->clip_latent_rows + b->max_patches_per_clip);
+    if (lat_in_place) {
+      TTV_TRY(ttvk_mlp_fused(ws.ao, dm, i == 0 ? nullptr : lw.attn_post_ln, keel_alpha(d, i), ws.x, dm, lw.mlp_pack, d->inner, ws.x, dm,
+                             i == 0 ? nullptr : lw.ffd_post_ln, keel_alpha(d, i), d->eps, b->sum_tokens, nullptr, s, b->clip_latent_rows,
+                             b->clip_latent_rows + b->max_patches_per_clip));
+      continue;
+    }
     if (lat_now) {
       TTV_TRY(gather_rows(ws.x, ws.xl, b->latent_rows, b->sum_tokens, row_bytes, s));
       TTV_TRY(gather_rows(ws.ao, ws.aol, b->latent_rows, b->sum_tokens, row_bytes, s));
       cx = ws.xl; cao = ws.aol; Lc = b->sum_tokens;
       compacted = true;
     }
-    static const bool use_fused_mlp = ttv_env_flag("TTV_FUSED_MLP", true);
+    const bool use_fused_mlp = fused_mlp_env;
     static const bool use_fused_qkv = ttv_env_flag("TTV_FUSED_QKV", false);
     const float alpha = keel_alpha(d, i);
     if (use_fused_mlp && ttvk_mlp_fused_supported(dt, dm, d->inner) && lw.mlp_pack) {
diff --git a/titok_video_amd/csrc/ttv_gemm.hip b/titok_video_amd/csrc/ttv_gemm.hip
--- a/titok_video_amd/csrc/ttv_gemm.hip
+++ b/titok_video_amd/csrc/ttv_gemm.hip
@@ -31,6 +31,7 @@
   long long* stamps;
   int resid_rows;
   int tile_run, tile_period;
+  int panel_begin_run, panel_begin_rest;
 };
 
 struct PatchDst {
@@ -1847,24 +1848,30 @@
 }
 
 static int sw_qkv256() { static const int v = ttv_env_int("TTV_QKV256", 1); return v; }
-bool ttvk_gemm_qkv_tiles_supported(int d_model, int gqa_dim, int ldw) {
+bool ttvk_gemm_qkv_tiles_supported(int d_model, int gqa_dim, int ldw, int range_col) {
   const int N = 2 * d_model + 2 * gqa_dim;
   return sw_qkv256() == 1 && !(g_ttv_debug & (TTV_DBG_QKV256_OFF | TTV_DBG_QKV256_WS)) && N % 64 == 0 && d_model % 64 == 0 && gqa_dim % 64 == 0 &&
-         (uint64_t)N * (uint64_t)ldw * 2u < (1ull << 32);
+         (uint64_t)N * (uint64_t)ldw * 2u < (1ull << 32) && range_col >= 0 && range_col < N && range_col % 64 == 0;
 }
 
 template <int EPI>
 static int launch(const GemmDev& d, int dtype, bool prenorm, hipStream_t s) {
   if (dtype == TTV_BF16 && d.K == 256 && d.N % 8 == 0 && !((d.debug & TTV_DBG_K256_GENERAL) && !prenorm && EPI != EPI_STORE_PATCH)) {
     const int fo = (EPI == EPI_GEGLU) ? 32 : 64;
-    const int n_panels = ttv_cdiv(d.N, fo), n_tiles = d.tile_period ? d.M / K256_TT / d.tile_period * d.tile_run : ttv_cdiv(d.M, K256_TT);
-    const int total = n_panels * n_tiles;
+    const int n_panels = ttv_cdiv(d.N, fo);
+    const int total = d.tile_period ? d.M / K256_TT / d.tile_period * (d.tile_run * (n_panels - d.panel_begin_run) + (d.tile_period - d.tile_run) * (n_panels - d.panel_begin_rest))
+                                    : n_panels * ttv_cdiv(d.M, K256_TT);
     static const int grid_env = ttv_env_int("TTV_K256_GRID", 0);
     int grid = total < 512 ? total : 512;
     if (grid_env > 0) grid = total < grid_env ? total : grid_env;
     else if (total > 512)
       for (int g = 512; g >= 416; --g)
         if (total % g == 0) { grid = g; break; }
+    if (grid_env <= 0 && d.tile_period && d.panel_begin_run < n_panels && d.panel_begin_rest < n_panels && d.panel_begin_run != d.panel_begin_rest) {
+      int q = n_panels - d.panel_begin_run, r = n_panels - d.panel_begin_rest;
+      while (r) { const int t = q % r; q = r; r = t; }
+      if (total / q <= 512) grid = total / q;
+    }
     const int qkv256_env = sw_qkv256();
     if constexpr (EPI == EPI_QKV_ROPE) {
       const int n_groups = (n_panels + 3) / 4;
@@ -2030,11 +2037,16 @@
   d.row_scale = a.row_scale;
   d.stamps = g_ttv_stamps;
   d.resid_rows = a.resid_rows;
-  d.tile_run = d.tile_period = 0;
+  d.tile_run = d.tile_period = d.panel_begin_run = d.panel_begin_rest = 0;
+  TTV_CHECK_ARG(a.tile_period || (!a.panel_begin_run && !a.panel_begin_rest), "gemm: a panel range belongs to a tile list");
   if (a.tile_period) {
     TTV_CHECK_ARG(epi == EPI_QKV_ROPE && a.dtype == TTV_BF16 && a.K == 256 && a.tile_run > 0 && a.tile_run < a.tile_period &&
                   a.M % (K256_TT * a.tile_period) == 0, "gemm: a tile list is a to_qkv option of the bf16 K=256 kernel, M a whole number of periods");
+    const int n_panels = a.N / 64;
+    TTV_CHECK_ARG(a.N % 64 == 0 && a.panel_begin_run >= 0 && a.panel_begin_rest >= 0 && a.panel_begin_run <= n_panels && a.panel_begin_rest <= n_panels &&
+                  a.panel_begin_run + a.panel_begin_rest < 2 * n_panels, "gemm: a tile list's panel ranges begin in [0, N / 64], and one class has panels");
     d.tile_run = a.tile_run; d.tile_period = a.tile_period;
+    d.panel_begin_run = a.panel_begin_run; d.panel_begin_rest = a.panel_begin_rest;
   }
   TTV_CHECK_ARG(!a.row_scale || ((a.dtype == TTV_BF16 || a.split3) && (epi == EPI_STORE || epi == EPI_QKV_ROPE || epi == EPI_GEGLU)),
                 "gemm: row_scale is a STORE / QKV_ROPE / GEGLU option of the bf16 and the split-bf16 kernels");
diff --git a/titok_video_amd/csrc/ttv_kernels.h b/titok_video_amd/csrc/ttv_kernels.h
--- a/titok_video_amd/csrc/ttv_kernels.h
+++ b/titok_video_amd/csrc/ttv_kernels.h
@@ -81,13 +81,14 @@
   int patch_t, patch_h, patch_w;
   int resid_rows;
   int tile_run, tile_period;
+  int panel_begin_run, panel_begin_rest;
 };
 struct ClipPtrs { void* p[TTV_MAX_CLIPS_PER_LAUNCH]; };
 int ttvk_gemm(GemmEpilogue epi, const GemmArgs& a, hipStream_t s);
 int ttvk_gemm_fp8(GemmEpilogue epi, const GemmArgs& a, const float* x_scale, const float* w_scale, hipStream_t s, const void* x_mx = nullptr,
                   const void* w_mx = nullptr);
 bool ttvk_gemm_supports_resid_norm(int dtype, int N, int K);
-bool ttvk_gemm_qkv_tiles_supported(int d_model, int gqa_dim, int ldw);
+bool ttvk_gemm_qkv_tiles_supported(int d_model, int gqa_dim, int ldw, int range_col = 0);
 
 int ttvk_attention(const void* qkvg, int ld, void* out, int ldo, const int* cu_seqlens, const int* qblocks, int n_qblocks,
                    int q_heads, int kv_heads, int head_dim, int flags, int dtype, hipStream_t s, float* lse_out = nullptr,
@@ -135,7 +136,9 @@
 int ttvk_mlp_pack(const void* w12_folded, const void* w3, const void* wo, const void* next_qkv_folded, int next_qkv_rows, int inner,
                   void* packed, hipStream_t s);
 int ttvk_mlp_fused(const void* ao, int ldao, const float* front_gain, float front_alpha, const void* x, int ldx, const void* packed,
-                   int inner, void* y, int ldy, const float* post_gain, float alpha, float eps, int M, const MlpNextQkv* nq, hipStream_t s);
+                   int inner, void* y, int ldy, const float* post_gain, float alpha, float eps, int M, const MlpNextQkv* nq, hipStream_t s,
+                   int run_rows = 0, int period_rows = 0);
+bool ttvk_mlp_fused_takes_rows(int M, int run_rows, int period_rows);
 
 int ttvk_l1_loss(void* const* recon, void* const* target, void* const* grad, const int* sizes, int n_clips, int total_clips, int dtype,
                  float* loss, hipStream_t s);
diff --git a/titok_video_amd/csrc/ttv_mlp.hip b/titok_video_amd/csrc/ttv_mlp.hip
--- a/titok_video_amd/csrc/ttv_mlp.hip
+++ b/titok_video_amd/csrc/ttv_mlp.hip
@@ -20,6 +20,7 @@
   const float* post_gain;
   float alpha, eps;
   int M, n_tiles, debug;
+  int blk_run, blk_period_rows;
   long long* stamps;
 };
 
@@ -104,7 +105,7 @@
 #endif
 
 template <int TPB, int T1, int T2, bool GELU_FIRST, bool KEEL, bool FRONT, bool BACK>
-__device__ __forceinline__ void mlp_wave(const MlpDev& p, uint4* l12, uint4* l3, uint4* hb, const float* gl, int tile, int wave, int lane,
+__device__ __forceinline__ void mlp_wave(const MlpDev& p, uint4* l12, uint4* l3, uint4* hb, const float* gl, int row0, int wave, int lane,
                                          int P1F, int P2F, int& n_stamp) {
   constexpr int T1A = T1 > 0 ? T1 : 1, T2A = T2 > 0 ? T2 : 1;
   const int l15 = lane & 15, kq = lane >> 4;
@@ -125,7 +126,7 @@
     MLP_GLDS_2(src__, dst__);                                                                                      \
   } while (0)
 
-  const int tok0 = tile * (16 * TPB) + l15;
+  const int tok0 = row0 + l15;
   typedef __attribute__((address_space(1))) char gchar;
   typedef __attribute__((address_space(1))) const char gcchar;
   gcchar* const gx = (gcchar*)p.x;
@@ -549,18 +550,19 @@
   const int lane = threadIdx.x & 63;
   const int wave = __builtin_amdgcn_readfirstlane(threadIdx.x >> 6);
   int n_stamp = 0;
-  const int tile = blockIdx.x;
+  const int blk = blockIdx.x;
+  const int row0 = p.blk_run ? (blk / p.blk_run) * p.blk_period_rows + (blk % p.blk_run) * (16 * TILES) : blk * (16 * TILES);
   if constexpr (TILES == 9) {
-    if (wave < 4) mlp_wave<9, 2, 0, false, KEEL, FRONT, BACK>(p, l12, l3, hb, gl, tile, wave, lane, 2 * wave, 0, n_stamp);
-    else if (wave < 6) mlp_wave<9, 0, 3, false, KEEL, FRONT, BACK>(p, l12, l3, hb, gl, tile, wave, lane, 0, 3 * (wave - 4), n_stamp);
-    else if (wave == 6) mlp_wave<9, 1, 1, false, KEEL, FRONT, BACK>(p, l12, l3, hb, gl, tile, wave, lane, 8, 6, n_stamp);
-    else mlp_wave<9, 0, 2, false, KEEL, FRONT, BACK>(p, l12, l3, hb, gl, tile, wave, lane, 0, 7, n_stamp);
+    if (wave < 4) mlp_wave<9, 2, 0, false, KEEL, FRONT, BACK>(p, l12, l3, hb, gl, row0, wave, lane, 2 * wave, 0, n_stamp);
+    else if (wave < 6) mlp_wave<9, 0, 3, false, KEEL, FRONT, BACK>(p, l12, l3, hb, gl, row0, wave, lane, 0, 3 * (wave - 4), n_stamp);
+    else if (wave == 6) mlp_wave<9, 1, 1, false, KEEL, FRONT, BACK>(p, l12, l3, hb, gl, row0, wave, lane, 8, 6, n_stamp);
+    else mlp_wave<9, 0, 2, false, KEEL, FRONT, BACK>(p, l12, l3, hb, gl, row0, wave, lane, 0, 7, n_stamp);
   } else {
     constexpr int NT = TILES / 4;
     constexpr int TA = NT - NT / 2;
     const int g0 = (wave & 3) * NT;
-    if (wave < 4) mlp_wave<TILES, TA, NT - TA, false, KEEL, FRONT, BACK>(p, l12, l3, hb, gl, tile, wave, lane, g0, g0 + TA, n_stamp);
-    else mlp_wave<TILES, NT - TA, TA, false, KEEL, FRONT, BACK>(p, l12, l3, hb, gl, tile, wave, lane, g0 + TA, g0, n_stamp);
+    if (wave < 4) mlp_wave<TILES, TA, NT - TA, false, KEEL, FRONT, BACK>(p, l12, l3, hb, gl, row0, wave, lane, g0, g0 + TA, n_stamp);
+    else mlp_wave<TILES, NT - TA, TA, false, KEEL, FRONT, BACK>(p, l12, l3, hb, gl, row0, wave, lane, g0 + TA, g0, n_stamp);
   }
 }
 #undef MLP_LD12
@@ -589,9 +591,34 @@
   return TTV_OK;
 }
 
+static int mlp_tiles_per_block(int M, bool next_qkv) {
+  const int cus = 256;
+  int tiles = 4;
+  long best = -1;
+  for (int c = 1; c <= 3; ++c) {
+    const long cost = (long)ttv_cdiv(ttv_cdiv(M, 64 * c), cus) * (16 + 19 * c);
+    if (best < 0 || cost < best) { best = cost; tiles = 4 * c; }
+  }
+  if (!next_qkv && !(g_ttv_debug & TTV_DBG_MLP_PAIRS_ONLY)) {
+    const long cost9 = (long)ttv_cdiv(ttv_cdiv(M, 144), cus) * (16 + 14 * 3);
+    if (cost9 < best) { best = cost9; tiles = 9; }
+  }
+  if ((g_ttv_debug & TTV_DBG_MLP_TILES9) && !next_qkv) tiles = 9;
+  if (g_ttv_debug & TTV_DBG_MLP_TILES8) tiles = 8;
+  if (g_ttv_debug & TTV_DBG_MLP_TILES4) tiles = 4;
+  return tiles;
+}
+
+bool ttvk_mlp_fused_takes_rows(int M, int run_rows, int period_rows) {
+  return M > 0 && run_rows > 0 && run_rows < period_rows && M % run_rows == 0 && run_rows % (16 * mlp_tiles_per_block(M, false)) == 0 &&
+         (int64_t)(M / run_rows) * period_rows <= INT32_MAX;
+}
+
 int ttvk_mlp_fused(const void* ao, int ldao, const float* front_gain, float front_alpha, const void* x, int ldx, const void* packed,
-                   int inner, void* y, int ldy, const float* post_gain, float alpha, float eps, int M, const MlpNextQkv* nq, hipStream_t s) {
+                   int inner, void* y, int ldy, const float* post_gain, float alpha, float eps, int M, const MlpNextQkv* nq, hipStream_t s,
+                   int run_rows, int period_rows) {
   if (M == 0) return TTV_OK;
+  TTV_CHECK_ARG(!period_rows || (!nq && ttvk_mlp_fused_takes_rows(M, run_rows, period_rows)), "mlp_fused: a block list needs runs of whole blocks and no next-qkv part");
   TTV_CHECK_ARG(x && packed && y, "mlp_fused: null buffer");
   TTV_CHECK_ARG(inner % 32 == 0 && ldx % 8 == 0 && ldy % 8 == 0 && (!ao || ldao % 8 == 0), "mlp_fused: inner %% 32, leading dims %% 8");
   TTV_CHECK_ARG(((uintptr_t)x % 16 == 0) && ((uintptr_t)packed % 16 == 0) && ((uintptr_t)y % 16 == 0) && ((uintptr_t)ao % 16 == 0),
@@ -608,21 +635,13 @@
     d.qkv = (bf16_t*)nq->qkv; d.ldq = nq->ld; d.rope_cs = nq->rope_cs; d.nqp = nq->rows / 64;
     d.rope_q_end = nq->rope_q_end; d.rope_k_begin = nq->rope_k_begin; d.rope_k_end = nq->rope_k_end;
   }
-  const int cus = 256;
-  int tiles = 4;
-  long best = -1;
-  for (int c = 1; c <= 3; ++c) {
-    const long cost = (long)ttv_cdiv(ttv_cdiv(M, 64 * c), cus) * (16 + 19 * c);
-    if (best < 0 || cost < best) { best = cost; tiles = 4 * c; }
-  }
-  if (!nq && !(g_ttv_debug & TTV_DBG_MLP_PAIRS_ONLY)) {
-    const long cost9 = (long)ttv_cdiv(ttv_cdiv(M, 144), cus) * (16 + 14 * 3);
-    if (cost9 < best) { best = cost9; tiles = 9; }
-  }
-  if ((g_ttv_debug & TTV_DBG_MLP_TILES9) && !nq) tiles = 9;
-  if (g_ttv_debug & TTV_DBG_MLP_TILES8) tiles = 8;
-  if (g_ttv_debug & TTV_DBG_MLP_TILES4) tiles = 4;
+  const int tiles = mlp_tiles_per_block(M, nq != nullptr);
   d.n_tiles = ttv_cdiv(M, 16 * tiles);
+  d.blk_run = d.blk_period_rows = 0;
+  if (period_rows) {
+    d.blk_run = run_rows / (16 * tiles); d.blk_period_rows = period_rows;
+    d.M = M / run_rows * period_rows;
+  }
   const int grid = d.n_tiles;
   const size_t smem = (size_t)(2 * MLP_W12_CHUNKS + 2 * MLP_W3_CHUNKS + 2 * tiles * 64) * sizeof(uint4) + 2048;
   TtvProfScope prof(TTV_KC_GEMM_GEGLU, s);
diff --git a/titok_video_amd/csrc/ttv_plan.hip b/titok_video_amd/csrc/ttv_plan.hip
--- a/titok_video_amd/csrc/ttv_plan.hip
+++ b/titok_video_amd/csrc/ttv_plan.hip
@@ -154,6 +154,10 @@
   batch->blocks64 = dev_segment + sz->off_blocks64;
   batch->row_seq = a.row_seq;
   batch->n_blocks64 = sz->n_blocks64;
+  const int32_t* const cu = host_segment + sz->off_cu_seqlens;
+  bool uniform = (int64_t)sz->max_patches_per_clip * sz->n_clips == sz->sum_patches;
+  for (int b = 1; uniform && b < sz->n_clips; ++b) uniform = cu[b + 1] - cu[b] == cu[1] - cu[0];
+  if (uniform) batch->clip_latent_rows = cu[1] - cu[0] - sz->max_patches_per_clip;
   if (rope_base) {
     batch->rope_ids = a.rope_ids;
     batch->rope_base = rope_base;
diff --git a/titok_video_amd/csrc/ttv_qkv256.inc b/titok_video_amd/csrc/ttv_qkv256.inc
--- a/titok_video_amd/csrc/ttv_qkv256.inc
+++ b/titok_video_amd/csrc/ttv_qkv256.inc
@@ -20,6 +20,38 @@
 #define QK_STAMP_START()
 #define QK_STAMP(seg_)
 #endif
+__device__ __forceinline__ void qk_item(const GemmDev& p, int n_panels, int it, int& ttile, int& panel) {
+  if (!p.tile_period) {
+    ttile = it / n_panels;
+    panel = it - ttile * n_panels;
+    return;
+  }
+  const int w_run = n_panels - p.panel_begin_run, w_rest = n_panels - p.panel_begin_rest;
+  const int run_items = p.tile_run * w_run;
+  const int per_items = run_items + (p.tile_period - p.tile_run) * w_rest;
+  const int per = it / per_items;
+  int rem = it - per * per_items;
+  if (rem < run_items) {
+    const int tl = rem / w_run;
+    ttile = per * p.tile_period + tl;
+    panel = p.panel_begin_run + rem - tl * w_run;
+  } else {
+    rem -= run_items;
+    const int tl = rem / w_rest;
+    ttile = per * p.tile_period + p.tile_run + tl;
+    panel = p.panel_begin_rest + rem - tl * w_rest;
+  }
+}
+__device__ __forceinline__ void qk_next_item(const GemmDev& p, int n_panels, int& ttile, int& panel) {
+  if (++panel < n_panels) return;
+  ++ttile;
+  panel = 0;
+  if (!p.tile_period) return;
+  int pos = ttile % p.tile_period;
+  if (pos >= p.tile_run && p.panel_begin_rest >= n_panels) { ttile += p.tile_period - pos; pos = 0; }
+  if (pos < p.tile_run && p.panel_begin_run >= n_panels) { ttile += p.tile_run - pos; pos = p.tile_run; }
+  panel = pos < p.tile_run ? p.panel_begin_run : p.panel_begin_rest;
+}
 typedef unsigned qk_u32x4 __attribute__((ext_vector_type(4)));
 typedef unsigned qk_u32x2 __attribute__((ext_vector_type(2)));
 template <bool PRENORM>
@@ -196,13 +228,14 @@
   do {                                                                                                       \
     const int it__ = (it_);                                                                                  \
     const int buf__ = (it__ - it0) & 1;                                                                      \
-    const int tile__ = it__ / n_panels, panel__ = it__ - tile__ * n_panels;                                  \
-    if (tile__ != cur_tile) {                                                                                \
-      cur_tile = tile__;                                                                                     \
+    const int ttile__ = it_tile, panel__ = it_panel;                                                         \
+    int ntile__ = ttile__, npanel__ = panel__;                                                               \
+    qk_next_item(p, n_panels, ntile__, npanel__);                                                            \
+    if (ttile__ != cur_tile) {                                                                               \
+      cur_tile = ttile__;                                                                                    \
        \
                                                                                \
-        \
-      const int ttile__ = p.tile_period ? (tile__ / p.tile_run) * p.tile_period + tile__ % p.tile_run : tile__; \
+           \
       const int t0__ = ttile__ * K256_TT + wave * 32;                                                        \
       int ntk__ = t0__ + r;                                                                                  \
       const bool nok__ = ntk__ < p.M;                                                                        \
@@ -229,7 +262,7 @@
     }                                                                                                        \
     QK_STAMP(1);                                                                                             \
     const bool has_next__ = it__ + 1 < it1;                                                                  \
-    const char* nsrc__ = QK_PANEL_SRC((it__ + 1) % n_panels);                                                \
+    const char* nsrc__ = QK_PANEL_SRC(npanel__);                                                             \
     const uint32_t ndst__ = QK_PANEL_DST(buf__ ^ 1);                                                         \
     const int f_first__ = panel__ * 64;                                                                      \
     const int rot__ = (f_first__ < p.rope_q_end || (f_first__ >= p.rope_k_begin && f_first__ < p.rope_k_end)) ? 2 : 1; \
@@ -254,12 +287,15 @@
     QK_STAMP(5);                                                                                             \
     pend = rot__;                                                                                            \
     pend_panel = panel__;                                                                                    \
+    it_tile = ntile__; it_panel = npanel__;                                                                  \
   } while (0)
 
   f32x16 accA[2], accB[2];
   QK_STAMP_DECL;
+  int it_tile, it_panel;
+  qk_item(p, n_panels, it0, it_tile, it_panel);
   {
-    const char* src0 = QK_PANEL_SRC(it0 % n_panels);
+    const char* src0 = QK_PANEL_SRC(it_panel);
     const uint32_t dst0 = QK_PANEL_DST(0);
     QK_DMA_PIECE(dchunk0, 0, src0, dst0); QK_DMA_PIECE(dchunk0, 1, src0, dst0); QK_DMA_PIECE(dchunk0, 2, src0, dst0); QK_DMA_PIECE(dchunk0, 3, src0, dst0);
     QK_DMA_PIECE(dchunk0, 4, src0, dst0); QK_DMA_PIECE(dchunk0, 5, src0, dst0); QK_DMA_PIECE(dchunk0, 6, src0, dst0); QK_DMA_PIECE(dchunk0, 7, src0, dst0);
diff --git a/titok_video_amd/plan.py b/titok_video_amd/plan.py
--- a/titok_video_amd/plan.py
+++ b/titok_video_amd/plan.py
@@ -192,6 +192,7 @@
         self._base_fields = dict(
             n_clips=B, total_rows=self.total_rows, sum_tokens=self.sum_tokens, sum_patches=self.sum_patches,
             max_patches_per_clip=max(sizes),
+            clip_latent_rows=self.token_counts[0] if len(set(self.token_counts)) == 1 and len(set(sizes)) == 1 else 0,
             cu_seqlens=base + 4 * offs[0], latent_rows=base + 4 * offs[1], patch_rows=base + 4 * offs[2],
             clip_desc=base + 4 * offs[3], rope_cs=self.rope_cs.data_ptr(),
             blocks64=base + 4 * offs[4], row_seq=base + 4 * offs[5], n_blocks64=self.n_blocks64)
```

Measured after the change: 31070 (median of 6 runs). About the same (+0.9%).
